# wiedenhoeft/HaMMLET

Hardware: AMD Instinct MI355X
Metric: block-updates/sec (Gibbs sweep) + HBM GB/s, 10^8 pos / 5 states (higher is better)
Workload: dtype f32; 1 GPU; c3_1e8_k5_dynamic; positions=100000000, states=5, block_structure=dynamic, chains=1, parallelism=chain-parallel x1

## Files before the change

hammlet_amd/csrc/hml_capi.hip:

```cpp
#include "hml_capi_shared.hpp"

static thread_local std::string g_err;
int hml_set_err(int code, const std::string& msg) { g_err = msg; return code; }

static const hml_ktab* ktab(int K);
#define HML_KTAB(KV, tab) const hml_ktab* tab = ktab(KV); if (!tab) return set_err(HML_ERR_ARG, "number of states must be in [2,16]")

std::atomic<int> hml_live_ctx[64];
int hml_ctx_bind(hml_ctx* c) { return ctx_bind(c); }
int hml_ctx_fetch_model(hml_ctx* c, hml_model* out) { return fetch_model(c, out); }

HML_KERNEL void hml_k_debug_eval(int fn, const float* __restrict__ a, const float* __restrict__ b, float* __restrict__ out,
                                 uint64_t n, uint64_t seed) {
    if (fn == 24) {
        const uint64_t nw = ((uint64_t)gridDim.x * blockDim.x) >> 6;
        if ((threadIdx.x & 63) != 0) return;
        for (uint64_t i = ((uint64_t)blockIdx.x * blockDim.x + threadIdx.x) >> 6; i < n; i += nw) {
            hml_dev_src src;
            src.s = hml_stream_open(hml_make_key(seed, 0), HML_KIND_THETA, seed, (uint32_t)i);
            out[i] = hml_gamma_f32<hml_devmath>(src, a[i], b[i]);
        }
        return;
    }
    const uint64_t stride = (uint64_t)gridDim.x * blockDim.x;
// ... 615 lines not shown
    layout(c->fwdL_mid, c->lay_mid);
    layout(c->fwdL_many, c->lay_many);
    HIPCHK(hipMalloc(&c->d_em, plane * sizeof(float)));
    HIPCHK(hipMalloc(&c->d_gsc, plane * sizeof(float)));
    HIPCHK(hipMalloc(&c->d_rows, plane * sizeof(float)));
    HIPCHK(hipMalloc(&c->d_entry, maxChunks * K * sizeof(float)));
    HIPCHK(hipMalloc(&c->d_exitA, maxChunks * K * sizeof(float)));
    HIPCHK(hipMalloc(&c->d_fb, maxChunks * sizeof(uint32_t)));
    HIPCHK(hipMalloc(&c->d_smap, (cap + 2) * sizeof(unsigned long long)));
    const uint64_t bchunks = (cap + 15) / 16 + 1;
    HIPCHK(hipMalloc(&c->d_cmap, bchunks * sizeof(unsigned long long)));
    HIPCHK(hipMalloc(&c->d_bentry, bchunks));
    HIPCHK(hipMalloc(&c->d_scmap, bchunks * sizeof(unsigned long long)));
    HIPCHK(hipMalloc(&c->d_super, (bchunks / 64 + 2) * sizeof(unsigned long long)));
    HIPCHK(hipMalloc(&c->d_bentry2, bchunks / 64 + 2));
    HIPCHK(hipMalloc(&c->d_redo, bchunks * sizeof(uint32_t)));
    HIPCHK(hipMemsetAsync(c->d_redo, 0, bchunks * sizeof(uint32_t), c->stream));
    HIPCHK(hipMalloc(&c->d_touched, bchunks * sizeof(uint32_t)));
    HIPCHK(hipMemsetAsync(c->d_touched, 0, bchunks * sizeof(uint32_t), c->stream));
    HIPCHK(hipMalloc(&c->d_redo2, bchunks * sizeof(uint32_t)));
    HIPCHK(hipMalloc(&c->d_tre_bitmap, (bchunks / 32 + 2) * sizeof(uint32_t)));
    HIPCHK(hipMalloc(&c->d_tre_ckpt, (cap / HML_TRE_CKPT_ROWS + 64) * (uint64_t)(K + 1) * sizeof(uint32_t)));
    HIPCHK(hipMalloc(&c->d_q, cap * sizeof(int16_t)));
    const uint64_t n_partial = ((uint64_t)HML_REDUCE_GROUPS + HML_PARAMS_TREE_WGS) * K * 2;
    HIPCHK(hipMalloc(&c->d_partial, n_partial * sizeof(double)));
    HIPCHK(hipMemsetAsync(c->d_partial, 0, n_partial * sizeof(double), c->stream));
    return 0;
}

static int grow_capacity(hml_ctx* c, uint64_t needed) {
    const uint64_t cap = std::min<uint64_t>(c->T, std::max<uint64_t>(needed + needed / 2 + 1024, 2 * c->cap));
    if (c->graph_exec) { hipGraphExecDestroy(c->graph_exec); c->graph_exec = nullptr; }
    void** blocks[] = {(void**)&c->d_starts, (void**)&c->d_bstat};
    for (void** q : blocks) if (*q) { hipFree(*q); *q = nullptr; }
    free_sweep_buffers(c,  true);
    if (c->d_eprobe) { hipFree(c->d_eprobe); c->d_eprobe = nullptr; }
    if (c->d_aprobe) { hipFree(c->d_aprobe); c->d_aprobe = nullptr; }
    c->cap = cap;
    HIPCHK(hipMalloc(&c->d_starts, (cap + 1) * sizeof(uint32_t)));
    HIPCHK(hipMalloc(&c->d_bstat, cap * (uint64_t)c->D * sizeof(float2)));
    if (c->model_set) {
        if (int r = alloc_sweep_buffers(c)) return r;
        if (c->probes) {
            HIPCHK(hipMalloc(&c->d_eprobe, c->cap * c->K * sizeof(float)));
            HIPCHK(hipMalloc(&c->d_aprobe, (c->cap + 1) * c->K * sizeof(float)));
        }
    }
    const uint32_t words[2] = {(uint32_t)cap, 0u};
    static_assert(offsetof(hml_model, halted) == offsetof(hml_model, cap) + sizeof(uint32_t), "cap and halted are written together");
    HIPCHK(hipMemcpyAsync(&c->d_mdl->cap, words, sizeof words, hipMemcpyHostToDevice, c->stream));
    HIPCHK(hipStreamSynchronize(c->stream));
    c->h_B[2] = 0u;
    c->blocks_valid = false;
    c->hint_stale = false;
    c->grown++;
    return 0;
}

static int sweep_dispatch(hml_ctx* c, char method, bool record);

int hml_settle(hml_ctx* c) {
    for (int round = 0; round < 64; ++round) {
        HIPCHK(hipStreamSynchronize(c->stream));
        if (!chain_halted(c)) { c->sweep_log.clear(); c->log_base = c->requested; return 0; }
        const uint64_t needed = c->h_B[2];
        if (c->cap >= c->T) return set_err(HML_ERR_HIP, "internal error: a chain with full block capacity halted");
        std::vector<uint8_t> pending;
        if (c->model_set) {
            hml_model m;
            if (int r = fetch_model(c, &m)) return r;
            const uint64_t ran = m.sweeps >= c->log_base ? m.sweeps - c->log_base : 0;
            if (ran < c->sweep_log.size()) pending.assign(c->sweep_log.begin() + ran, c->sweep_log.end());
            c->log_base = m.sweeps;
        }
        if (int r = grow_capacity(c, needed)) return r;
        c->sweep_log = pending;
        bool halted_again = false;
        for (size_t i = 0; i < pending.size() && !halted_again; ++i) {
            const char method = (pending[i] & 1) ? HML_METHOD_MIXTURE : HML_METHOD_FB;
            const bool record = (pending[i] & 2) != 0;
            if (int r = sweep_dispatch(c, method, record)) return r;
            if (record && c->cb) {
                HIPCHK(hipStreamSynchronize(c->stream));
                halted_again = chain_halted(c);
                if (!halted_again) {
                    if (int r = check_device_error(c)) return r;
                    const unsigned long long ordinal = c->log_base + i;
                    c->cb(c, ordinal >= c->call_base ? (uint64_t)(ordinal - c->call_base) : 0u, c->cb_user);
                }
            }
        }
    }
    return set_err(HML_ERR_HIP, "internal error: the block capacity did not settle");
}

extern "C" {

int hml_set_model(hml_ctx* c, int K, const float nig4[4], float a_off, float a_diag, float pi_alpha, int self_trans) {
    if (!c || !c->loaded) return set_err(HML_ERR_ARG, "no observations loaded");
    if (K < 2) return set_err(HML_ERR_MODEL, "Requested parameters would yield an HMM with less than 2 states!");
    if (K > HML_CAP_K) return set_err(HML_ERR_ARG, "number of states must be in [2,64]");
    if (c->model_set) return set_err(HML_ERR_ARG, "model already set");
    if (c->D > 1 && c->P == 0) {
        for (int pp = 2; pp <= K; ++pp) { long k = 1; for (int d = 0; d < c->D; ++d) k *= pp; if (k == K) { c->P = pp; break; } if (k > K) break; }
        if (c->P == 0) return set_err(HML_ERR_ARG, "number of states must be (number of parameters)^(data dimensions)");
    }
    if (c->P > 0) {
        long k = 1;
        for (int d = 0; d < c->D; ++d) k *= c->P;
        if (k != K) return set_err(HML_ERR_ARG, "number of states must be (number of parameters)^(data dimensions)");
    }
    if (!(nig4[0] > 0)) return set_err(HML_ERR_MODEL, "Alpha (" + std::to_string(nig4[0]) + ") must be positive!");
    if (!(nig4[1] > 0)) return set_err(HML_ERR_MODEL, "Beta (" + std::to_string(nig4[1]) + ") must be positive!");
    if (!(nig4[3] > 0)) return set_err(HML_ERR_MODEL, "Nu (" + std::to_string(nig4[3]) + ")must be positive!");
    const hml_ktab* kt = nullptr;
    c->wide = !c->compat && (K > HML_MAX_K || (getenv("HML_WIDE") && atoi(getenv("HML_WIDE")) != 0));
    if (!c->compat && !c->wide) { kt = ktab(K); if (!kt) return set_err(HML_ERR_ARG, "number of states must be in [2,16]"); }
    if (int r = ctx_bind(c)) return r;
    free_sweep_buffers(c);
    c->K = K;
    if (!getenv("HML_PARAMS_SPREAD")) c->params_spread = K >= 8;
    const uint64_t T = c->T;
    if (int r = alloc_sweep_buffers(c)) return r;

    hml_model m;
    memset(&m, 0, sizeof m);
    m.K = K; m.self_trans = self_trans ? 1 : 0; m.dynamic = 1; m.T = (uint32_t)T;
    m.D = c->D; m.P = c->P > 0 ? c->P : K; m.stat_stride = T;
    m.cap = (uint32_t)c->cap;
    for (int st = 0; st < K; ++st) {
        int nn = st;
        for (int d = 0; d < HML_MAX_D; ++d) { m.map[st][d] = (uint8_t)(d < c->D ? nn % m.P : 0); nn /= m.P; }
    }
    for (int i = 0; i < 4; ++i) m.nig_prior[i] = nig4[i];
    m.a_off = a_off; m.a_diag = a_diag; m.pi_alpha = pi_alpha;
    m.key = hml_make_key(c->seed, c->chain);
    for (int k = 0; k < K; ++k) {
        for (int i = 0; i < 4; ++i) m.nig_post[k][i] = nig4[i];
        m.dirPi[k] = pi_alpha;
        m.pi[k] = 1.0f / K;
        for (int j = 0; j < K; ++j) { m.dirA[k * K + j] = (k == j) ? a_diag : a_off; m.A[k * K + j] = 1.0f / K; }
    }
    m.max_state_recorded = -1;
    m.tre_fused = (c->tre_fused && c->D == 1) ? 1u : 0u;
    m.tre_hi_shift = 17u; m.tre_lo_shift = 20u;
    if (const char* e = getenv("HML_TRE_REFIT_SHIFTS")) { unsigned a = 17, b = 20; if (sscanf(e, "%u,%u", &a, &b) == 2 && a < 32 && b < 32) { m.tre_hi_shift = a; m.tre_lo_shift = b; } }
    m.fwd_W0 = (uint32_t)c->fwdW;
    m.fwd_W = m.fwd_W_burnin = (uint32_t)std::max(c->fwdW, c->fwdW_init);
    if (c->compat || c->wide) { m.fwd_W = 64u; m.fwd_W0 = c->wide ? (uint32_t)c->wide_w0 : 32u; }
    m.wl_bwd_W = 64u; m.wl_bwd_quiet = 0u; m.wl_retry = 0u; m.wl_W_need = 0u; m.wl_need_age = 0u;
    m.fwd_burnin_sweeps = c->fwd_burnin_sweeps;
    m.fwd_quiet_need = c->fwd_quiet_need;
    m.n_spans = c->n_spans;
    HIPCHK(hipMemcpyAsync(c->d_mdl, &m, sizeof m, hipMemcpyHostToDevice, c->stream));
    HIPCHK(hipStreamSynchronize(c->stream));
    c->dynamic = true;
    c->hint_stale = true;
    if (c->compat) {
        hml_mt_state h;
        hml_mt_seed(&h, c->seed + (uint64_t)c->chain);
        HIPCHK(hipMalloc(&c->d_mt, sizeof(hml_mt_state)));
        HIPCHK(hipMemcpyAsync(c->d_mt, &h, sizeof h, hipMemcpyHostToDevice, c->stream));
        HIPCHK(hipStreamSynchronize(c->stream));
        hipLaunchKernelGGL(hml_k_compat_draw, dim3(1), dim3(64), 0, c->stream, c->d_mdl, (hml_mt_state*)c->d_mt, 2);
        KLAUNCH_CHECK();
        c->model_set = true;
        return 0;
    }
    if (c->wide) hipLaunchKernelGGL(hml_k_wide_params, dim3(1), dim3(1024), 0, c->stream, c->d_mdl, c->d_partial, (hml_wide_acc*)c->d_wacc, 2);
    else kt->params(c, 2);
    KLAUNCH_CHECK();
    c->model_set = true;
    return 0;
}

int hml_sample_prior(hml_ctx* c) {
    if (!c || !c->model_set) return set_err(HML_ERR_ARG, "model not set");
    if (int r = ctx_bind(c)) return r;
    if (int r = settle_if_limited(c)) return r;
    if (c->compat) {
        hipLaunchKernelGGL(hml_k_compat_draw, dim3(1), dim3(64), 0, c->stream, c->d_mdl, (hml_mt_state*)c->d_mt, 1);
    } else if (c->wide) {
        hipLaunchKernelGGL(hml_k_wide_params, dim3(1), dim3(1024), 0, c->stream, c->d_mdl, c->d_partial, (hml_wide_acc*)c->d_wacc, 1);
    } else { HML_KTAB(c->K, kt); kt->params(c, 1); }
    KLAUNCH_CHECK();
    if (c->dynamic) c->blocks_valid = false;
    c->hint_stale = true;
    return 0;
}

HML_KERNEL __launch_bounds__(64) void hml_k_set_self_trans(hml_model* mdl, int on) {
    if (threadIdx.x == 0) mdl->self_trans = on;
}

int hml_set_self_transitions(hml_ctx* c, int on) {
    if (!c || !c->model_set) return set_err(HML_ERR_ARG, "model not set");
    if (int r = ctx_bind(c)) return r;
    if (int r = settle_if_limited(c)) return r;
    hipLaunchKernelGGL(hml_k_set_self_trans, dim3(1), dim3(64), 0, c->stream, c->d_mdl, on ? 1 : 0);
    KLAUNCH_CHECK();
    if (c->graph_exec) { hipGraphExecDestroy(c->graph_exec); c->graph_exec = nullptr; }
    return 0;
}

int hml_set_static_blocks(hml_ctx* c) {
    if (!c || !c->model_set) return set_err(HML_ERR_ARG, "model not set");
    if (int r = ctx_bind(c)) return r;
    if (int r = settle_if_limited(c)) return r;
    hipLaunchKernelGGL(hml_k_set_dynamic, dim3(1), dim3(64), 0, c->stream, c->d_mdl, 0, 1);
    KLAUNCH_CHECK();
    c->dynamic = false;
    if (!cap_limited(c)) {
        if (int r = launch_compact(c, false, 0.0f)) return r;
    } else {
        bool fitted = false;
        for (int round = 0; round < 64 && !fitted; ++round) {
            if (int r = launch_compact(c, false, 0.0f)) return r;
            HIPCHK(hipStreamSynchronize(c->stream));
            fitted = !chain_halted(c);
            if (!fitted) { if (int r = grow_capacity(c, c->h_B[2])) return r; }
        }
        if (!fitted) return set_err(HML_ERR_HIP, "internal error: the block capacity did not settle");
        refresh_hint(c);
    }
    c->blocks_valid = true;
    return 0;
}

int hml_set_dynamic(hml_ctx* c, int on) {
    if (!c || !c->model_set) return set_err(HML_ERR_ARG, "model not set");
    if (int r = ctx_bind(c)) return r;
    if (int r = settle_if_limited(c)) return r;
    hipLaunchKernelGGL(hml_k_set_dynamic, dim3(1), dim3(64), 0, c->stream, c->d_mdl, on ? 1 : 0, on ? 1 : 0);
    KLAUNCH_CHECK();
    c->dynamic = on != 0;
    if (on) { c->blocks_valid = false; c->hint_stale = true; }
    return 0;
}

int hml_set_recording(hml_ctx* c, int marginals, hml_record_cb cb, void* user) {
    if (!c) return set_err(HML_ERR_ARG, "null context");
    c->rec_marginals = marginals != 0;
    c->cb = cb; c->cb_user = user;
    return 0;
}

static int set_recorder(hml_ctx* c, int kind, int on) {
    if (!c) return set_err(HML_ERR_ARG, "null context");
    c->rec[kind].on = on != 0;
    if (on) c->rec[kind].asked = true;
    if (c->graph_exec) { if (int r = ctx_bind(c)) return r; hipGraphExecDestroy(c->graph_exec); c->graph_exec = nullptr; }
    return 0;
}
int hml_set_level_recording(hml_ctx* c, int on) { return set_recorder(c, HML_REC_LEVELS, on); }
int hml_set_break_recording(hml_ctx* c, int on) { return set_recorder(c, HML_REC_BREAKS, on); }

int hml_set_level_bands(hml_ctx* c, int n_edges, const float* edges) {
    if (!c) return set_err(HML_ERR_ARG, "null context");
    if (c->graph_exec) { if (int r = ctx_bind(c)) return r; hipGraphExecDestroy(c->graph_exec); c->graph_exec = nullptr; }
    if (n_edges == 0) { c->rec[HML_REC_BANDS].on = false; return 0; }
    if (!edges) return set_err(HML_ERR_ARG, "null argument");
    if (const char* why = band_edges_fault(n_edges, edges)) return set_err(HML_ERR_ARG, why);
    if (c->model_set && (uint64_t)c->D * (uint64_t)(n_edges + 1) > HML_CAP_K)
        return set_err(HML_ERR_ARG, "level bands: the data dimensions times (edges + 1) exceed 64 columns");
    if (!same_band_edges(c, n_edges, edges) && c->rec[HML_REC_BANDS].d_acc) {
        if (int r = ctx_bind(c)) return r;
        if (int r = hml_settle(c)) return r;
        hml_model m; if (int r = fetch_model(c, &m)) return r;
        if (m.n_bands_recorded != 0ull) return set_err(HML_ERR_ARG, "level bands were already recorded under other edges: they cannot be changed any more");
        hml_recorder& rec = c->rec[HML_REC_BANDS];
        HIPCHK(hipFree(rec.d_acc)); rec.d_acc = nullptr;
        HIPCHK(hipFree(rec.d_boundary)); rec.d_boundary = nullptr;
    }
    c->n_band_edges = n_edges;
    memcpy(c->band_edges, edges, (size_t)n_edges * sizeof(float));
    c->rec[HML_REC_BANDS].on = c->rec[HML_REC_BANDS].asked = true;
    return 0;
}

int hml_get_level_bands(hml_ctx* c, int* n_edges, float* edges) {
    if (!c || !n_edges) return set_err(HML_ERR_ARG, "null argument");
    *n_edges = c->n_band_edges;
    if (edges) memcpy(edges, c->band_edges, (size_t)c->n_band_edges * sizeof(float));
    return 0;
}

int hml_enable_probes(hml_ctx* c, int on) {
    if (!c || !c->model_set) return set_err(HML_ERR_ARG, "model not set");
    if (int r = ctx_bind(c)) return r;
    if (int r = settle_if_limited(c)) return r;
    if (on && !c->d_eprobe) {
        HIPCHK(hipMalloc(&c->d_eprobe, c->cap * c->K * sizeof(float)));
        HIPCHK(hipMalloc(&c->d_aprobe, (c->cap + 1) * c->K * sizeof(float)));
    }
    c->probes = on != 0;
    return 0;
}

}

int hml_ctx_ensure_marginal_buffers(hml_ctx* c) { return ensure_marginal_buffers(c); }

static hml_compat_chunks chunk_views(const hml_ctx* c) {
    hml_compat_chunks ch;
    char* base = (char*)c->d_cchunk;
    const uint64_t n = c->wide ? c->wide_chunks_cap : (uint64_t)HML_COMPAT_MAX_CHUNKS;
// ... 208 lines not shown
                int rr = sweep_dispatch(c, method, false);
                const hipError_t ec = hipStreamEndCapture(c->stream, &g);
                if (rr || ec != hipSuccess) {
                    if (g) hipGraphDestroy(g);
                    (void)hipGetLastError();
                    return rr ? rr : set_err(HML_ERR_HIP, std::string("hipStreamEndCapture: ") + hipGetErrorString(ec));
                }
                const hipError_t ei = hipGraphInstantiate(&c->graph_exec, g, nullptr, nullptr, 0);
                hipGraphDestroy(g);
                if (ei != hipSuccess) { c->graph_exec = nullptr; return set_err(HML_ERR_HIP, std::string("hipGraphInstantiate: ") + hipGetErrorString(ei)); }
                c->graph_method = method; c->graph_dynamic = c->dynamic; c->graph_hint = c->B_hint; c->graph_fused = wants_fused;
                c->graph_dense = c->B_hint >= c->dense_min_blocks;
                c->graph_mid = c->B_hint >= c->mid_min_blocks;
            }
            if (c->graph_exec) {
                log_sweep(c, method, false);
                HIPCHK(hipGraphLaunch(c->graph_exec, c->stream));
                if (tre_path) c->tre_dense_sweeps++;
                continue;
            }
        }
        log_sweep(c, method, record);
        if (int r = sweep_dispatch(c, method, record)) return r;
        if (record && c->cb) {
            HIPCHK(hipStreamSynchronize(c->stream));
            if (chain_halted(c)) { if (int r = hml_settle(c)) return r; continue; }
            if (int r = check_device_error(c)) return r;
            c->cb(c, i, c->cb_user);
        }
    }
    return 0;
}

}

extern "C" int hml_iterate_many(hml_ctx* const* cs, int n, char method, uint64_t iterations, uint64_t thinning) {
    if (!cs || n < 1) return set_err(HML_ERR_ARG, "no contexts");
    for (int i = 0; i < n; ++i) if (!cs[i] || !cs[i]->model_set) return set_err(HML_ERR_ARG, "model not set");
    if (method != HML_METHOD_FB && method != HML_METHOD_MIXTURE) return set_err(HML_ERR_ARG, std::string("Unknown sampling type ") + method + "!");
    for (int i = 0; i < n; ++i) cs[i]->call_base = cs[i]->requested;
    uint64_t done = 0;
    while (done < iterations && many_eligible(cs, n, method)) {
        if (int r = ctx_bind(cs[0])) return r;
        for (int i = 0; i < n; ++i) {
            hml_ctx* c = cs[i];
            if (int r = settle_if_limited(c)) return r;
            if (c->hint_stale) { launch_compact_pair(c, 0, 0.0f); KLAUNCH_CHECK(); }
            HIPCHK(hipStreamSynchronize(c->stream));
            c->hint_stale = false;
            if (c->graph_exec) { hipGraphExecDestroy(c->graph_exec); c->graph_exec = nullptr; }
        }
        int r = 0;
        uint64_t reached = done;
        { HML_KTAB(cs[0]->K, kt); r = kt->iterate_many(cs, n, done, iterations, thinning, &reached); }
        if (r) return r;
        hipEvent_t ev = ev_get(cs[0]);
        HIPCHK(hipEventRecord(ev, cs[0]->stream));
        for (int i = 1; i < n; ++i) HIPCHK(hipStreamWaitEvent(cs[i]->stream, ev, 0));
        cs[0]->ev_pool.push_back(ev);
        if (reached == iterations) return 0;
        HIPCHK(hipStreamSynchronize(cs[0]->stream));
        bool halted = false;
        for (int i = 0; i < n; ++i) halted = halted || chain_halted(cs[i]);
        const bool progress = reached > done;
        done = reached;
        if (!halted && !progress) break;
        if (!halted) { bool sparse = true; for (int i = 0; i < n; ++i) sparse = sparse && many_sparse(cs[i]); if (!sparse) break; }
    }
    for (int i = 0; i < n; ++i) if (int r = settle_if_limited(cs[i])) return r;
    for (uint64_t i = done; i < iterations; ++i) {
        const bool record = thinning > 0 && ((i + 1) % thinning == 0);
        for (int k = 0; k < n; ++k) {
            hml_ctx* c = cs[k];
            if (int r = ctx_bind(c)) return r;
            if (record && c->rec_marginals && c->pooled) return set_err(HML_ERR_ARG, "the marginals of a context are pooled (common labels, several chains): further sweeps cannot be recorded into them");
            if (chain_halted(c)) { if (int r = hml_settle(c)) return r; }
            log_sweep(c, method, record);
            if (int r = sweep_dispatch(c, method, record)) return r;
            if (record && c->cb) {
                HIPCHK(hipStreamSynchronize(c->stream));
                if (chain_halted(c)) { if (int r = hml_settle(c)) return r; continue; }
                if (int r = check_device_error(c)) return r;
                c->cb(c, i, c->cb_user);
            }
        }
    }
    return 0;
}

extern "C" {

int hml_set_option(hml_ctx* c, const char* name, int value) {
    if (!c || !name) return set_err(HML_ERR_ARG, "null argument");
    if (std::string(name) == "weight_keys") {
        if (c->loaded) return set_err(HML_ERR_ARG, "weight_keys must be set before the observations are loaded");
        c->use_keys = value != 0;
        c->summary_always = value == 2;
        return 0;
    }
    if (std::string(name) == "max_blocks") {
        if (c->loaded) return set_err(HML_ERR_ARG, "max_blocks must be set before the observations are loaded");
        if (value < 0) return set_err(HML_ERR_ARG, "max_blocks: a number of blocks, or 0 for the default");
        c->cap_opt = (uint64_t)value;
        return 0;
    }
    if (std::string(name) == "fused_blocks") {
        c->fused_blocks = value != 0;
        c->fused_keep = value == 2;
        if (c->graph_exec) { hipGraphExecDestroy(c->graph_exec); c->graph_exec = nullptr; }
        return 0;
    }
    if (std::string(name) == "compat") {
        if (c->model_set) return set_err(HML_ERR_ARG, "compat must be set before the model");
        c->compat = value != 0;
        return 0;
    }
    if (std::string(name) == "trellis_L") {
        if (value < 0 || value > HML_TRE_MAX_L || value % 32) return set_err(HML_ERR_ARG, "trellis_L: 0 or a multiple of 32 up to 1024");
        c->tre_L = (uint32_t)value;
        return 0;
    }
    return set_err(HML_ERR_ARG, std::string("unknown option ") + name);
}

int hml_sync(hml_ctx* c) {
    if (!c) return set_err(HML_ERR_ARG, "null context");
    if (int r = ctx_bind(c)) return r;
    if (int r = hml_settle(c)) return r;
    if (c->d_dbg && getenv("HML_FUSED_DEBUG") && atoi(getenv("HML_FUSED_DEBUG")) == 2) {
        std::vector<unsigned long long> h(4096 * 8);
        hipMemcpy(h.data(), c->d_dbg, h.size() * 8, hipMemcpyDeviceToHost);
        uint32_t n = 0; while (n < 4096 && h[n * 8]) ++n;
        unsigned long long t0 = ~0ull; for (uint32_t i = 0; i < n; ++i) t0 = std::min(t0, h[i * 8]);
        double mx[5] = {0, 0, 0, 0, 0}, av[5] = {0, 0, 0, 0, 0};
        if (n) for (uint32_t i = 0; i < n; ++i) for (int k = 0; k < 5; ++k) { const double d = (double)(h[i * 8 + k] - t0) * 0.01; mx[k] = std::max(mx[k], d); av[k] += d / n; }
        if (n) fprintf(stderr, "[fused-many dbg] n=%u start avg %.2f max %.2f | phaseA avg %.2f max %.2f | requested avg %.2f max %.2f | offsets avg %.2f max %.2f | end avg %.2f max %.2f (us)\n",
                n, av[0], mx[0], av[1], mx[1], av[2], mx[2], av[3], mx[3], av[4], mx[4]);
        if (n) for (uint32_t i : {0u, n / 4, n / 2, n - 1}) if (i < n) fprintf(stderr, "   wg %u: %.2f %.2f %.2f %.2f %.2f | wavefront 0: parameters in LDS %.2f, weights arrived %.2f, its lists done %.2f\n", i, (h[i*8]-t0)*0.01, (h[i*8+1]-t0)*0.01, (h[i*8+2]-t0)*0.01, (h[i*8+3]-t0)*0.01, (h[i*8+4]-t0)*0.01,
                                                                                  (h[i*8+5]-t0)*0.01, (h[i*8+6]-t0)*0.01, (h[i*8+7]-t0)*0.01);
    } else if (c->d_dbg) {
        std::vector<unsigned long long> h(4096 * 4);
        hipMemcpy(h.data(), c->d_dbg, h.size() * 8, hipMemcpyDeviceToHost);
        const uint32_t n = (uint32_t)std::min<uint64_t>(4096, (c->T + HML_FUSED_SUB_POSITIONS - 1) / HML_FUSED_SUB_POSITIONS);
        unsigned long long t0 = ~0ull; for (uint32_t i = 0; i < n; ++i) if (h[i * 4]) t0 = std::min(t0, h[i * 4]);
        double mx[4] = {0, 0, 0, 0}, av[4] = {0, 0, 0, 0};
        for (uint32_t i = 0; i < n; ++i) for (int k = 0; k < 4; ++k) { const double d = (double)(h[i * 4 + k] - t0) * 0.01; mx[k] = std::max(mx[k], d); av[k] += d / n; }
        fprintf(stderr, "[fused dbg] n=%u start avg %.2f max %.2f | phaseA avg %.2f max %.2f | offsets avg %.2f max %.2f | end avg %.2f max %.2f (us)\n", n, av[0], mx[0], av[1], mx[1], av[2], mx[2], av[3], mx[3]);
        { uint32_t late = 0, first_late = n; for (uint32_t i = 0; i < n; ++i) if ((h[i * 4] - t0) * 0.01 > 2.0) { ++late; first_late = std::min(first_late, i); }
          fprintf(stderr, "   late starters: %u, first index %u\n", late, first_late); }
        for (uint32_t i : {0u, n / 4, n / 2, n - 1}) fprintf(stderr, "   wg %u: %.2f %.2f %.2f %.2f\n", i, (h[i*4]-t0)*0.01, (h[i*4+1]-t0)*0.01, (h[i*4+2]-t0)*0.01, (h[i*4+3]-t0)*0.01);
    }
    if (c->model_set && getenv("HML_PARAMS_DEBUG")) {
        hml_model m;
        if (fetch_model(c, &m) == 0) {
            fprintf(stderr, "[params dbg] us since the kernel's start: accumulators read %.2f | tree %.2f | theta drawn %.2f | A gammas %.2f | barrier %.2f | end %.2f\n",
                    (m.dbg_t[1] - m.dbg_t[0]) * 0.01, (m.dbg_t[2] - m.dbg_t[0]) * 0.01, (m.dbg_t[3] - m.dbg_t[0]) * 0.01, (m.dbg_t[4] - m.dbg_t[0]) * 0.01,
                    (m.dbg_t[5] - m.dbg_t[0]) * 0.01, (m.dbg_t[6] - m.dbg_t[0]) * 0.01);
            fprintf(stderr, "[params dbg]   theta's gamma core + normal drawn %.2f | last wavefront's tree %.2f\n", (m.dbg_t[7] - m.dbg_t[0]) * 0.01, (m.dbg_t[8] - m.dbg_t[0]) * 0.01);
        }
    }
    if (c->model_set) return check_device_error(c);
    return 0;
}


static int current_B(hml_ctx* c, uint32_t* B) {
    HIPCHK(hipMemcpyAsync(c->h_B, &c->d_mdl->B, sizeof(uint32_t), hipMemcpyDeviceToHost, c->stream));
    HIPCHK(hipStreamSynchronize(c->stream));
    *B = *c->h_B;
    return 0;
}

int hml_get_num_blocks(hml_ctx* c, uint64_t* B) {
    NEED_LOADED();
    uint32_t b; if (int r = current_B(c, &b)) return r;
    *B = b; return 0;
}
int hml_get_blocks(hml_ctx* c, uint32_t* starts) {
    NEED_LOADED();
    uint32_t b; if (int r = current_B(c, &b)) return r;
    HIPCHK(hipMemcpy(starts, c->d_starts, ((uint64_t)b + 1) * sizeof(uint32_t), hipMemcpyDeviceToHost));
    return 0;
}
int hml_get_block_stats(hml_ctx* c, float* sum, float* sum_sq) {
    NEED_LOADED();
    uint32_t b; if (int r = current_B(c, &b)) return r;
    std::vector<float2> v(b);
    for (int d = 0; d < c->D; ++d) {
        HIPCHK(hipMemcpy(v.data(), c->d_bstat + (uint64_t)d * c->T, (uint64_t)b * sizeof(float2), hipMemcpyDeviceToHost));
        for (uint32_t i = 0; i < b; ++i) { sum[(uint64_t)d * b + i] = v[i].x; sum_sq[(uint64_t)d * b + i] = v[i].y; }
    }
    return 0;
}
int hml_get_states(hml_ctx* c, int16_t* q) {
    NEED_MODEL();
    uint32_t b; if (int r = current_B(c, &b)) return r;
    HIPCHK(hipMemcpy(q, c->d_q, (uint64_t)b * sizeof(int16_t), hipMemcpyDeviceToHost));
    return 0;
}
int hml_get_theta(hml_ctx* c, float* mean_var) {
    NEED_MODEL();
    hml_model m; if (int r = fetch_model(c, &m)) return r;
    for (int k = 0; k < m.P; ++k) { mean_var[2 * k] = m.mu[k]; mean_var[2 * k + 1] = m.var[k]; }
    return 0;
}
int hml_get_dimensions(hml_ctx* c, int* D, int* P) {
    if (!c) return set_err(HML_ERR_ARG, "null context");
    if (D) *D = c->D;
    if (P) *P = c->P > 0 ? c->P : c->K;
    return 0;
}
int hml_get_transitions(hml_ctx* c, float* A, float* pi) {
    NEED_MODEL();
    hml_model m; if (int r = fetch_model(c, &m)) return r;
    if (A) memcpy(A, m.A, (size_t)c->K * c->K * sizeof(float));
    if (pi) memcpy(pi, m.pi, (size_t)c->K * sizeof(float));
    return 0;
}
int hml_set_parameters(hml_ctx* c, const float* mean_var, const float* A, const float* pi) {
    NEED_MODEL();
    hml_model m; if (int r = fetch_model(c, &m)) return r;
    const int K = c->K;
    for (int k = 0; k < m.P; ++k) {
        const float mean = mean_var[2 * k], var = mean_var[2 * k + 1];
        if (!std::isfinite(mean)) return set_err(HML_ERR_MODEL, "Mean (" + std::to_string(mean) + ") must be set to a finite value!");
        if (!std::isfinite(var)) return set_err(HML_ERR_MODEL, "Variance(" + std::to_string(var) + ") must be set to a finite value!");
        if (var <= 0) return set_err(HML_ERR_MODEL, "Variance (" + std::to_string(var) + ") must be positive!");
        m.mu[k] = mean; m.var[k] = var; m.sd[k] = sqrtf(var);
    }
    memcpy(m.A, A, (size_t)K * K * sizeof(float));
    memcpy(m.pi, pi, (size_t)K * sizeof(float));
    HIPCHK(hipMemcpyAsync(c->d_mdl, &m, sizeof m, hipMemcpyHostToDevice, c->stream));
    if (c->compat) hipLaunchKernelGGL(hml_k_compat_derive, dim3(1), dim3(64), 0, c->stream, c->d_mdl);
    else if (c->wide) hipLaunchKernelGGL(hml_k_wide_derive, dim3(1), dim3(64), 0, c->stream, c->d_mdl);
    else { HML_KTAB(K, kt); kt->derive(c); }
    KLAUNCH_CHECK();
    HIPCHK(hipStreamSynchronize(c->stream));
    if (c->dynamic) c->blocks_valid = false;
    return 0;
}
int hml_get_threshold(hml_ctx* c, float* thr) {
    NEED_MODEL();
    hml_model m; if (int r = fetch_model(c, &m)) return r;
    *thr = m.thr; return 0;
}
int hml_get_block_loglik(hml_ctx* c, float* E) {
    NEED_MODEL();
    if (!c->probes) return set_err(HML_ERR_ARG, "probes are not enabled");
    uint32_t b; if (int r = current_B(c, &b)) return r;
    HIPCHK(hipMemcpy(E, c->d_eprobe, (uint64_t)b * c->K * sizeof(float), hipMemcpyDeviceToHost));
    return 0;
}
int hml_get_forward_rows(hml_ctx* c, float* rows) {
    NEED_MODEL();
    if (!c->probes) return set_err(HML_ERR_ARG, "probes are not enabled");
    uint32_t b; if (int r = current_B(c, &b)) return r;
    HIPCHK(hipMemcpy(rows, c->d_aprobe, ((uint64_t)b + 1) * c->K * sizeof(float), hipMemcpyDeviceToHost));
    return 0;
}
int hml_get_counts(hml_ctx* c, uint64_t* trans, uint64_t* occ, float* sum, float* sum_sq, uint64_t* nterms) {
    NEED_MODEL();
    hml_model m; if (int r = fetch_model(c, &m)) return r;
    const int K = c->K;
    for (int i = 0; i < K * K; ++i) trans[i] = m.last_trans[i];
    for (int k = 0; k < K; ++k) { occ[k] = m.last_occ[k]; nterms[k] = m.last_occ[k]; sum[k] = m.last_sum[k]; sum_sq[k] = m.last_sumsq[k]; }
    return 0;
}
int hml_get_weights(hml_ctx* c, float* w) {
    NEED_LOADED();
    HIPCHK(hipStreamSynchronize(c->stream));
    HIPCHK(hipMemcpy(w, c->d_w, c->T * sizeof(float), hipMemcpyDeviceToHost));
    return 0;
}
int hml_get_coefficients(hml_ctx* c, float* cf) {
    NEED_LOADED();
    HIPCHK(hipStreamSynchronize(c->stream));
    HIPCHK(hipMemcpy(cf, c->d_coeff, c->T * sizeof(float), hipMemcpyDeviceToHost));
    return 0;
}
int hml_get_integral_array(hml_ctx* c, float* sum, float* sum_sq) {
    NEED_LOADED();
    HIPCHK(hipStreamSynchronize(c->stream));
    std::vector<float2> v(c->T + 1);
    HIPCHK(hipMemcpy(v.data(), c->d_ia, (c->T + 1) * sizeof(float2), hipMemcpyDeviceToHost));
    for (uint64_t i = 0; i <= c->T; ++i) { sum[i] = v[i].x; sum_sq[i] = v[i].y; }
    return 0;
}

int hml_recorded_sweeps(hml_ctx* c, uint64_t* n) {
    NEED_MODEL();
    hml_model m; if (int r = fetch_model(c, &m)) return r;
    *n = m.n_recorded; return 0;
}

int hml_relabel_permutation(hml_ctx* c, int32_t* perm) {
    NEED_MODEL();
    if (!perm) return set_err(HML_ERR_ARG, "null argument");
    hml_model m; if (int r = fetch_model(c, &m)) return r;
    const int K = c->K, D = m.D;
    std::vector<int32_t> p(K);
    for (int k = 0; k < K; ++k) p[k] = k;
    std::stable_sort(p.begin(), p.end(), [&](int32_t a, int32_t b) {
        for (int d = 0; d < D; ++d) {
            const float ma = m.mu[m.map[a][d]], mb = m.mu[m.map[b][d]];
            if (ma < mb) return true;
            if (mb < ma) return false;
        }
// ... 98 lines not shown
```

hammlet_amd/csrc/hml_common.h:

```cpp
#ifndef HML_COMMON_H
#define HML_COMMON_H

#include <stdint.h>
#include <stddef.h>

#if defined(__HIPCC__)
#include <hip/hip_runtime.h>
#define HML_HD __host__ __device__ __forceinline__
#define HML_HDM __host__ __device__ __forceinline__
#define HML_KERNEL static __global__
#else
#define HML_HD static inline
#define HML_HDM inline
#endif

#define HML_CELLSIZE 65535u

#define HML_MAX_K 16
#define HML_CAP_K 64

HML_HD uint32_t hml_f2u(float f) { return __builtin_bit_cast(uint32_t, f); }
HML_HD float hml_u2f(uint32_t u) { return __builtin_bit_cast(float, u); }
HML_HD uint64_t hml_d2u(double d) { return __builtin_bit_cast(uint64_t, d); }
HML_HD double hml_u2d(uint64_t u) { return __builtin_bit_cast(double, u); }

#define HML_INF_F (hml_u2f(0x7f800000u))

#endif
```

hammlet_amd/csrc/hml_k_backward.h:

```cpp
#ifndef HML_K_BACKWARD_H
#define HML_K_BACKWARD_H

#include <type_traits>

#include "hml_dist.h"
#include "hml_k_forward.h"
#include "hml_philox.h"
#include "hml_state.h"

#define HML_MAP_IDENTITY 0xfedcba9876543210ull

template <int K>
__device__ __forceinline__ unsigned long long hml_map_compose(unsigned long long f, unsigned long long g) {
    unsigned long long r = 0ull;
#pragma unroll
    for (int x = 0; x < K; ++x) {
        const unsigned y = (unsigned)(g >> (4 * x)) & 15u;
        const unsigned long long z = (f >> (4 * y)) & 15ull;
        r |= z << (4 * x);
    }
    return r;
}

__device__ __forceinline__ unsigned long long hml_shfl_down_u64(unsigned long long v, int d) {
    const unsigned lo = (unsigned)v, hi = (unsigned)(v >> 32);
    const unsigned lo2 = __shfl_down(lo, d), hi2 = __shfl_down(hi, d);
    return ((unsigned long long)hi2 << 32) | lo2;
}

template <int K>
__device__ __forceinline__ int hml_categorical_k_literal(const float (&w)[K], double u) {
    double sum = 0.0;
#pragma unroll
    for (int i = 0; i < K; ++i) sum += (double)w[i];
    double cp = 0.0;
    int res = K - 1;
    bool done = false;
#pragma unroll
    for (int i = 0; i < K; ++i) {
        cp += (double)w[i] / sum;
        const double c = (i == K - 1) ? 1.0 : cp;
        if (!done && !(c < u)) { res = i; done = true; }
    }
    return res;
}

template <int K>
__device__ __forceinline__ int hml_categorical_k_fast(const float (&w)[K], double u, bool& unsure_out) {
    double s[K];
    double acc = 0.0;
#pragma unroll
    for (int i = 0; i < K; ++i) { acc += (double)w[i]; s[i] = acc; }
    const double t = u * acc;
    const double margin = acc * 5.684341886080802e-14;
    bool unsure = !(acc > 0.0) || !(acc < 1.7976931348623157e308);
    int res = K - 1;
    bool done = false;
#pragma unroll
    for (int i = 0; i < K - 1; ++i) {
        const double d = s[i] - t;
        unsure = unsure || !(__builtin_fabs(d) > margin);
        if (!done && d >= 0.0) { res = i; done = true; }
    }
    unsure_out = unsure_out || unsure;
    return res;
}

template <int K>
__device__ __forceinline__ int hml_categorical_k_screen(const float (&w)[K], float uf, bool& unsure_out) {
    static_assert(K <= 16, "error bound of the float screen");
    float s[K];
    float acc = 0.0f;
#pragma unroll
    for (int i = 0; i < K; ++i) { acc += w[i]; s[i] = acc; }
    const float t = uf * acc;
    const float margin = acc * 7.62939453125e-06f;
    bool unsure = !(acc > 7.888609052210118e-31f) || !(acc < 3.4028234663852886e38f);
    int res = K - 1;
    bool done = false;
#pragma unroll
    for (int i = 0; i < K - 1; ++i) {
        const float d = s[i] - t;
        unsure = unsure || !(__builtin_fabsf(d) > margin);
        if (!done && d >= 0.0f) { res = i; done = true; }
    }
    unsure_out = unsure;
    return res;
}

template <int K>
__device__ __forceinline__ int hml_categorical_k(const float (&w)[K], double u) {
    bool unsure = false;
    int res = hml_categorical_k_screen<K>(w, (float)u, unsure);
    if (unsure) {
        asm volatile("" ::: "memory");
        unsure = false;
        res = hml_categorical_k_fast<K>(w, u, unsure);
        if (unsure) res = hml_categorical_k_literal<K>(w, u);
    }
    return res;
}

template <int K>
struct hml_bwd_ctx {
    hml_amat<K> A;
    float logA[K];
    bool self;
};
template <int K>
__device__ __forceinline__ void hml_bwd_ctx_load(hml_bwd_ctx<K>& bx, const hml_model* __restrict__ mdl_ro, const float* lds_A) {
    bx.A.attach(mdl_ro, lds_A);
#pragma unroll
    for (int i = 0; i < K; ++i) bx.logA[i] = mdl_ro->logA[i];
    bx.self = mdl_ro->self_trans != 0;
}

template <int K>
__device__ __forceinline__ void hml_bwd_row_load(const float* __restrict__ rows, const hml_layout lay, uint32_t c, int lane,
                                                 uint32_t B, float (&r)[K], const uint32_t* __restrict__ starts,
                                                 const hml_bwd_ctx<K>& bx) {
    const uint32_t t = c * HML_BWD_CHUNK + (uint32_t)lane + 1u;
    uint32_t st = 0u, en = 1u;
    if (starts && t < B) { st = starts[t - 1u]; en = starts[t]; }
#pragma unroll
    for (int i = 0; i < K; ++i) r[i] = (t <= B) ? rows[hml_bk(lay, t - 1u, K, i)] : 0.0f;
    if (starts && t < B && bx.self) {
        const float N = (float)(en - st);
#pragma unroll
        for (int i = 0; i < K; ++i) r[i] = r[i] * hml_expf((N - 1.0f) * bx.logA[i]);
    }
}

template <int K>
__device__ __forceinline__ void hml_bwd_chunk_maps(const float (&r)[K], hml_model* __restrict__ mdl, const hml_bwd_ctx<K>& bx,
                                                   unsigned long long* __restrict__ smap, unsigned long long* __restrict__ cmap,
                                                   uint32_t c, int lane, uint32_t B, unsigned long long epoch, const hml_key key) {
    const uint32_t t = c * HML_BWD_CHUNK + (uint32_t)lane + 1u;
    unsigned long long map = HML_MAP_IDENTITY;
    if (t <= B) {
        const double u = hml_cat_uniform(key, epoch, t);
        map = 0ull;
#pragma unroll
        for (int i = 0; i < K; ++i)
            if (r[i] < 0.0f) hml_raise(mdl, HML_DEVERR_NEG_BACKWARD, r[i]);
        if (t == B) {
            const unsigned long long st = (unsigned long long)hml_categorical_k<K>(r, u);
#pragma unroll
            for (int x = 0; x < K; ++x) map |= st << (4 * x);
        } else {
#pragma unroll
            for (int x = 0; x < K; ++x) {
                float w[K];
#pragma unroll
                for (int i = 0; i < K; ++i) w[i] = r[i] * bx.A[i * K + x];
                map |= (unsigned long long)hml_categorical_k<K>(w, u) << (4 * x);
            }
        }
    }
#pragma unroll
    for (int d = 1; d < 64; d <<= 1) {
        unsigned long long o = hml_shfl_down_u64(map, d);
        if (lane + d >= 64) o = HML_MAP_IDENTITY;
        map = hml_map_compose<K>(map, o);
    }
    if (t <= B) smap[t] = map;
    if (lane == 0) cmap[c] = map;
}

template <int K>
__device__ __forceinline__ void hml_b_backward_maps(const float* __restrict__ rows, hml_model* __restrict__ mdl,
                                                           unsigned long long* __restrict__ smap,
                                                           unsigned long long* __restrict__ cmap, const hml_layout lay,
                                                           const float* __restrict__ entry, const float* __restrict__ exitv,
                                                           uint32_t* __restrict__ fail_list, int L,
                                                           const uint32_t* __restrict__ starts,
                                                           const hml_model* __restrict__ mdl_ro) {
    const uint32_t B = mdl_ro->B;
    const uint32_t nchunks = (B + HML_BWD_CHUNK - 1u) / HML_BWD_CHUNK;
    const int lane = threadIdx.x & 63;
    const uint32_t wave_global = (blockIdx.x * blockDim.x + threadIdx.x) >> 6;
    const uint32_t nwaves = (gridDim.x * blockDim.x) >> 6;
    const unsigned long long epoch = mdl_ro->epoch;
    const hml_key key = mdl_ro->key;
    const int W = (int)mdl_ro->fwd_W;
    __shared__ float sm_A[hml_amat<K>::LDS_FLOATS];
    hml_amat_fill<K>(sm_A, mdl_ro, (int)threadIdx.x, (int)blockDim.x);
    hml_bwd_ctx<K> bx;
    hml_bwd_ctx_load<K>(bx, mdl_ro, sm_A);
    const uint32_t C = (B + (uint32_t)L - 1u) / (uint32_t)L;
    for (uint32_t c = wave_global; c < nchunks; c += nwaves) {
        float r[K];
        hml_bwd_row_load<K>(rows, lay, c, lane, B, r, starts, bx);
        bool ok = true;
        {
            const uint32_t f0 = (c * HML_BWD_CHUNK) / (uint32_t)L;
            const uint32_t f1 = (c * HML_BWD_CHUNK + HML_BWD_CHUNK - 1u) / (uint32_t)L;
            const uint32_t f = f0 + (uint32_t)lane;
            if (f <= f1 && f < C && !hml_fwd_chunk_exact(f, L, W)) {
                uint32_t differ = 0u;
#pragma unroll
                for (int s = 0; s < K; ++s) differ |= hml_f2u(entry[(uint64_t)f * K + s]) ^ hml_f2u(exitv[(uint64_t)(f - 1) * K + s]);
                ok = differ == 0u;
            }
        }
        if (__ballot(!ok) != 0ull) {
            if (lane == 0) fail_list[atomicAdd(&mdl->fwd_mismatch, 1u)] = c;
            continue;
        }
        hml_bwd_chunk_maps<K>(r, mdl, bx, smap, cmap, c, lane, B, epoch, key);
    }
}
template <int K>
HML_KERNEL __launch_bounds__(256) void hml_k_backward_maps(const float* __restrict__ rows, hml_model* __restrict__ mdl,
                                                           unsigned long long* __restrict__ smap,
                                                           unsigned long long* __restrict__ cmap, const hml_layout lay,
                                                           const float* __restrict__ entry, const float* __restrict__ exitv,
                                                           uint32_t* __restrict__ fail_list, int L,
                                                           const uint32_t* __restrict__ starts,
                                                           const hml_model* __restrict__ mdl_ro) {
    hml_b_backward_maps<K>(rows, mdl, smap, cmap, lay, entry, exitv, fail_list, L, starts, mdl_ro);
}


template <int K>
__device__ __forceinline__ unsigned long long hml_bwd_row_map(const float (&r)[K], hml_model* __restrict__ mdl, const hml_bwd_ctx<K>& bx,
                                                              uint32_t t, uint32_t B, double u) {
    if (t > B) return HML_MAP_IDENTITY;
    unsigned long long map = 0ull;
#pragma unroll
    for (int i = 0; i < K; ++i)
        if (r[i] < 0.0f) hml_raise(mdl, HML_DEVERR_NEG_BACKWARD, r[i]);
    if (t == B) {
        const unsigned long long st = (unsigned long long)hml_categorical_k<K>(r, u);
#pragma unroll
        for (int x = 0; x < K; ++x) map |= st << (4 * x);
    } else {
#pragma unroll
        for (int x = 0; x < K; ++x) {
            float w[K];
#pragma unroll
            for (int i = 0; i < K; ++i) w[i] = r[i] * bx.A[i * K + x];
            map |= (unsigned long long)hml_categorical_k<K>(w, u) << (4 * x);
        }
    }
    return map;
}
template <int K>
__device__ __forceinline__ void hml_bwd_row_load_t(const float* __restrict__ rows, const hml_layout lay, uint32_t t, uint32_t B, float (&r)[K],
                                                   const uint32_t* __restrict__ starts, const hml_bwd_ctx<K>& bx) {
    uint32_t st = 0u, en = 1u;
    if (starts && t < B) { st = starts[t - 1u]; en = starts[t]; }
#pragma unroll
    for (int i = 0; i < K; ++i) r[i] = (t <= B) ? rows[hml_bk(lay, t - 1u, K, i)] : 0.0f;
    if (starts && t < B && bx.self) {
        const float N = (float)(en - st);
#pragma unroll
        for (int i = 0; i < K; ++i) r[i] = r[i] * hml_expf((N - 1.0f) * bx.logA[i]);
    }
}
template <int K>
__device__ __forceinline__ void hml_b_backward_maps2(const float* __restrict__ rows, hml_model* __restrict__ mdl,
                                                            unsigned long long* __restrict__ smap,
                                                            unsigned long long* __restrict__ cmap, const hml_layout lay,
                                                            const float* __restrict__ entry, const float* __restrict__ exitv,
                                                            uint32_t* __restrict__ fail_list, int L,
                                                            const uint32_t* __restrict__ starts,
                                                            const hml_model* __restrict__ mdl_ro) {
    const uint32_t B = mdl_ro->B;
    const uint32_t nchunks = (B + HML_BWD_CHUNK - 1u) / HML_BWD_CHUNK;
    const uint32_t npairs = (nchunks + 1u) / 2u;
    const int lane = threadIdx.x & 63, li = lane & 31, half = lane >> 5;
    const uint32_t wave_global = (blockIdx.x * blockDim.x + threadIdx.x) >> 6;
    const uint32_t nwaves = (gridDim.x * blockDim.x) >> 6;
    const unsigned long long epoch = mdl_ro->epoch;
    const hml_key key = mdl_ro->key;
    const int W = (int)mdl_ro->fwd_W;
    __shared__ float sm_A[hml_amat<K>::LDS_FLOATS];
    hml_amat_fill<K>(sm_A, mdl_ro, (int)threadIdx.x, (int)blockDim.x);
    hml_bwd_ctx<K> bx;
    hml_bwd_ctx_load<K>(bx, mdl_ro, sm_A);
    const uint32_t C = (B + (uint32_t)L - 1u) / (uint32_t)L;
    for (uint32_t pw = wave_global; pw < npairs; pw += nwaves) {
        const uint32_t c = 2u * pw + (uint32_t)half;
        const uint32_t t0 = c * HML_BWD_CHUNK + 2u * (uint32_t)li + 1u;
        float r0[K], r1[K];
        hml_bwd_row_load_t<K>(rows, lay, t0, B, r0, starts, bx);
        hml_bwd_row_load_t<K>(rows, lay, t0 + 1u, B, r1, starts, bx);
        bool ok = true;
        if (c < nchunks) {
            const uint32_t f0 = (c * HML_BWD_CHUNK) / (uint32_t)L;
            const uint32_t f1 = (c * HML_BWD_CHUNK + HML_BWD_CHUNK - 1u) / (uint32_t)L;
            for (uint32_t f = f0 + (uint32_t)li; f <= f1 && f < C; f += 32u) {
                if (hml_fwd_chunk_exact(f, L, W)) continue;
                uint32_t differ = 0u;
#pragma unroll
                for (int s = 0; s < K; ++s) differ |= hml_f2u(entry[(uint64_t)f * K + s]) ^ hml_f2u(exitv[(uint64_t)(f - 1) * K + s]);
                ok = ok && differ == 0u;
            }
        }
        const unsigned long long failed = __ballot(!ok);
        const bool my_fail = (half ? (failed >> 32) : (failed & 0xffffffffull)) != 0ull;
        if (my_fail && li == 0 && c < nchunks) fail_list[atomicAdd(&mdl->fwd_mismatch, 1u)] = c;
        if ((failed & 0xffffffffull) != 0ull && (failed >> 32) != 0ull) continue;
        double u0, u1;
        hml_cat_uniform_pair(key, epoch, (t0 - 1u) >> 1, u0, u1);
        const bool live = !my_fail && c < nchunks;
        const unsigned long long m0 = live ? hml_bwd_row_map<K>(r0, mdl, bx, t0, B, u0) : HML_MAP_IDENTITY;
        const unsigned long long m1 = live ? hml_bwd_row_map<K>(r1, mdl, bx, t0 + 1u, B, u1) : HML_MAP_IDENTITY;
        unsigned long long P = hml_map_compose<K>(m0, m1);
#pragma unroll
        for (int d = 1; d < 32; d <<= 1) {
            unsigned long long o = hml_shfl_down_u64(P, d);
            if (li + d >= 32) o = HML_MAP_IDENTITY;
            P = hml_map_compose<K>(P, o);
        }
        unsigned long long later = hml_shfl_down_u64(P, 1);
        if (li == 31) later = HML_MAP_IDENTITY;
        if (live) {
            if (t0 <= B) smap[t0] = P;
            if (t0 + 1u <= B) smap[t0 + 1u] = hml_map_compose<K>(m1, later);
            if (li == 0) cmap[c] = P;
        }
    }
}

template <int K>
__device__ __forceinline__ void hml_b_backward_chain(unsigned long long* __restrict__ cmap, hml_model* __restrict__ mdl,
                                                             uint8_t* __restrict__ entry_state, const float* __restrict__ em,
                                                             const float* __restrict__ gsc, float* __restrict__ rows,
                                                             float* __restrict__ aprobe, float* __restrict__ entry,
                                                             float* __restrict__ exitv, uint32_t* __restrict__ fb_count,
                                                             const uint32_t* __restrict__ fail_list, uint32_t* __restrict__ touched,
                                                             unsigned long long* __restrict__ smap, int L, const hml_layout lay,
                                                             int mode, int super_level, const uint32_t* __restrict__ starts) {
    __shared__ unsigned long long P[1024];
    __shared__ hml_repair_lds sh;
    const uint32_t B = mdl->B;
    const uint32_t NCb = (B + HML_BWD_CHUNK - 1u) / HML_BWD_CHUNK;
    const uint32_t NC = super_level ? (NCb + 63u) / 64u : NCb;
    const int tid = threadIdx.x;
    const uint32_t n_fail = (mode & 1) ? mdl->fwd_mismatch : 0u;
    if (n_fail != 0u) {
        const unsigned long long epoch = mdl->epoch;
        const uint32_t gen = (uint32_t)epoch + 1u;
        const hml_key key = mdl->key;
        __shared__ float sm_A[hml_amat<K>::LDS_FLOATS];
        hml_amat_fill<K>(sm_A, mdl, tid, 1024);
        hml_fwd_repair<K>(em, gsc, mdl, rows, aprobe, entry, exitv, fb_count, fail_list, n_fail, touched, gen, L, lay, sh, sm_A);
        const int lane = tid & 63, wave = tid >> 6;
        hml_bwd_ctx<K> bx;
        hml_bwd_ctx_load<K>(bx, mdl, sm_A);
        auto redo = [&](uint32_t c) {
            float r[K];
            hml_bwd_row_load<K>(rows, lay, c, lane, B, r, starts, bx);
            hml_bwd_chunk_maps<K>(r, mdl, bx, smap, cmap, c, lane, B, epoch, key);
        };
        for (uint32_t i = (uint32_t)wave; i < n_fail; i += 16u) redo(fail_list[i]);
        const uint32_t n_touched = sh.tcount;
        if (n_touched <= (uint32_t)HML_REPAIR_TOUCHED_CAP) {
            for (uint32_t i = (uint32_t)wave; i < n_touched; i += 16u) redo(sh.tlist[i]);
        } else {
            for (uint32_t c0 = (uint32_t)wave * 64u; c0 < NCb; c0 += 16u * 64u) {
                const uint32_t c = c0 + (uint32_t)lane;
                unsigned long long todo = __ballot(c < NCb && hml_ld_u32_coherent(touched + c) == gen);
                while (todo) {
                    const int j = __ffsll((long long)todo) - 1;
                    todo &= todo - 1ull;
                    redo(c0 + (uint32_t)j);
                }
            }
        }
        __threadfence_block();
        __syncthreads();
        if (tid == 0) mdl->fwd_mismatch = 0u;
    }
    if (!(mode & 2)) return;
    const uint32_t per = (NC + 1023u) / 1024u;
    const uint32_t a = (uint32_t)tid * per < NC ? (uint32_t)tid * per : NC;
    const uint32_t b = (a + per < NC) ? a + per : NC;
    const int lane = tid & 63, wave = tid >> 6;
    constexpr int CACHED = 4;
    unsigned long long mine[CACHED];
    unsigned long long prod = HML_MAP_IDENTITY;
    if (per <= (uint32_t)CACHED) {
#pragma unroll
        for (int j = 0; j < CACHED; ++j) mine[j] = (a + (uint32_t)j < b) ? cmap[a + (uint32_t)j] : HML_MAP_IDENTITY;
#pragma unroll
        for (int j = CACHED - 1; j >= 0; --j) prod = hml_map_compose<K>(mine[j], prod);
    } else {
        for (uint32_t c = b; c > a; --c) prod = hml_map_compose<K>(cmap[c - 1], prod);
    }
    unsigned long long S = prod;
#pragma unroll
    for (int d = 1; d < 64; d <<= 1) {
        unsigned long long o = hml_shfl_down_u64(S, d);
        if (lane + d >= 64) o = HML_MAP_IDENTITY;
        S = hml_map_compose<K>(S, o);
    }
    if (lane == 0) P[wave] = S;
    __syncthreads();
    if (tid < 64) {
        unsigned long long w = (tid < 16) ? P[tid] : HML_MAP_IDENTITY;
#pragma unroll
        for (int d = 1; d < 16; d <<= 1) {
            unsigned long long o = hml_shfl_down_u64(w, d);
            if (tid + d >= 16) o = HML_MAP_IDENTITY;
            w = hml_map_compose<K>(w, o);
        }
        if (tid < 16) P[16 + tid] = w;
    }
    __syncthreads();
    const unsigned long long after_wave = (wave < 15) ? P[16 + wave + 1] : HML_MAP_IDENTITY;
    unsigned long long next_S = hml_shfl_down_u64(S, 1);
    const unsigned long long later = (lane < 63) ? hml_map_compose<K>(next_S, after_wave) : after_wave;
    if (a >= b) return;
    unsigned x = (unsigned)(later & 15ull);
    if (per <= (uint32_t)CACHED) {
#pragma unroll
        for (int j = CACHED - 1; j >= 0; --j) {
            if (a + (uint32_t)j < b) {
                entry_state[a + (uint32_t)j] = (uint8_t)x;
                x = (unsigned)(mine[j] >> (4 * x)) & 15u;
            }
        }
    } else {
        for (uint32_t c = b; c > a; --c) {
            entry_state[c - 1] = (uint8_t)x;
            x = (unsigned)(cmap[c - 1] >> (4 * x)) & 15u;
        }
    }
}
template <int K>
HML_KERNEL __launch_bounds__(1024) void hml_k_backward_chain(unsigned long long* __restrict__ cmap, hml_model* __restrict__ mdl,
// ... 405 lines not shown
```

hammlet_amd/csrc/hml_k_blocks_fused.h:

```cpp
#ifndef HML_K_BLOCKS_FUSED_H
#define HML_K_BLOCKS_FUSED_H

#include "hml_k_blocks.h"
#include "hml_k_forward.h"

#define HML_FUSED_WAVES 8
#define HML_FUSED_WAVE_BATCH (HML_SUM_SPANS * HML_SPAN)
#define HML_FUSED_SUB_POSITIONS (HML_FUSED_WAVES * HML_FUSED_WAVE_BATCH)
#define HML_FUSED_MAX_SUB 4
#define HML_FUSED_POS_BITS 19
#define HML_FUSED_GEN_MASK ((1u << (64 - 2 * HML_FUSED_POS_BITS - 1)) - 1u)
#define HML_FUSED_WAVE_LIST 256
__device__ __forceinline__ unsigned long long hml_group_word(uint32_t gen, uint32_t total, uint32_t last_rel) {
    return ((unsigned long long)(gen & HML_FUSED_GEN_MASK) << (2 * HML_FUSED_POS_BITS + 1)) |
           ((unsigned long long)total << HML_FUSED_POS_BITS) | (unsigned long long)last_rel;
}
__device__ __forceinline__ uint32_t hml_fused_generation(const hml_model* mdl) { return ((uint32_t)mdl->epoch + 1u) & HML_FUSED_GEN_MASK; }

__device__ __forceinline__ unsigned long long hml_fused_tile_word(const uint8_t* __restrict__ summary, const float* __restrict__ w, uint32_t T,
                                                               float thr, int32_t base, uint32_t tile, uint32_t n_sub, uint32_t gen) {
    const uint32_t n_spans = (uint32_t)(((uint64_t)T + HML_SPAN - 1) / HML_SPAN);
    const uint32_t kthr = (thr != thr) ? 0u : hml_weight_key(thr, base);
    const uint32_t first_span = tile * (uint32_t)HML_FUSED_WAVES * n_sub * HML_SUM_SPANS;
    const uint32_t spans = (uint32_t)HML_FUSED_WAVES * n_sub * HML_SUM_SPANS;
    uint32_t total = 0u, last1 = 0u;
    for (uint32_t s = 0; s < spans && first_span + s < n_spans; ++s) {
        const uint32_t span = first_span + s;
        for (uint32_t g = 0; g < 256u; ++g) {
            const uint32_t key = summary[(uint64_t)span * 256u + (uint64_t)(g & 63u) * 4u + (g >> 6)];
            const bool origin = (span == 0u && g == 0u);
            if (key < kthr && !origin) continue;
            uint32_t m16 = hml_group_mask16(w, (uint64_t)span * HML_SPAN + (uint64_t)g * 16u, T, thr);
            if (origin) m16 |= 1u;
            if (m16) {
                total += (uint32_t)__popc(m16);
                last1 = s * HML_SPAN + g * 16u + (31u - (uint32_t)__clz((int)m16)) + 1u;
            }
        }
    }
    return hml_group_word(gen, total, last1 ? last1 - 1u : 0u);
}

template <int K>
HML_KERNEL __launch_bounds__(HML_FUSED_WAVES * 64, 6) void hml_k_blocks_fused(const uint8_t* __restrict__ summary, const float* __restrict__ w,
                                                          const float2* __restrict__ ia, uint32_t T,
                                                          hml_model* __restrict__ mdl, int32_t base,
                                                          unsigned long long* __restrict__ group_word,
                                                          uint16_t* __restrict__ stage, uint32_t* __restrict__ starts,
                                                          float2* __restrict__ bstat, float* __restrict__ em,
                                                          float* __restrict__ gsc, float* __restrict__ eprobe, int mixture,
                                                          const hml_layout lay, uint32_t* __restrict__ host_words,
                                                          uint32_t n_sub, uint32_t spin_limit, unsigned long long* __restrict__ dbg,
                                                          const hml_model* __restrict__ mdl_ro) {
    if (dbg && threadIdx.x == 0) dbg[blockIdx.x * 4 + 0] = wall_clock64();
    static_assert(HML_FUSED_MAX_SUB * HML_FUSED_SUB_POSITIONS == (1 << HML_FUSED_POS_BITS), "tile geometry (bit fields of hml_group_word)");
    static_assert(HML_FUSED_MAX_SUB * HML_FUSED_WAVE_BATCH <= 65536, "16-bit offsets into a wavefront's eighth");
    constexpr int NW = HML_FUSED_WAVES;
    constexpr uint32_t NT = NW * 64;
    __shared__ uint16_t listed_all[NW][HML_SUM_SPANS * 256];
    __shared__ uint16_t mask_all[NW][HML_SUM_SPANS * 256];
    __shared__ uint16_t wave_list[NW][HML_FUSED_WAVE_LIST];
    __shared__ uint32_t wave_total[NW], wave_last[NW];
    __shared__ unsigned long long red_sum[NW], red_near[NW];
    __shared__ uint64_t sm_exp_tab[32];
    if (threadIdx.x < 32u) sm_exp_tab[threadIdx.x] = HML_EXP2F_TAB[threadIdx.x];
    constexpr bool LOOPED = K > 6;
    __shared__ hml_emit_lds<LOOPED ? K : 1> sm_emit;
    if (LOOPED) hml_emit_lds_fill<LOOPED ? K : 1>(sm_emit, mdl_ro, (int)threadIdx.x);

    const int lane = threadIdx.x & 63, wave = threadIdx.x >> 6;
    const uint32_t g = blockIdx.x;
    const uint32_t n_spans = (uint32_t)(((uint64_t)T + HML_SPAN - 1) / HML_SPAN);
    const uint32_t eighth = n_sub * (uint32_t)HML_FUSED_WAVE_BATCH;
    const uint32_t tile_positions = eighth * (uint32_t)NW;
    const uint64_t wave_base = ((uint64_t)g * NW + (uint32_t)wave) * eighth;
    const uint32_t gen = hml_fused_generation(mdl_ro);
    uint16_t* listed = listed_all[wave];
    uint16_t* masks = mask_all[wave];
    const float thr = mdl_ro->thr;
    const uint32_t cap = mdl_ro->cap;

    uint32_t total = 0u, last1 = 0u;
    uint32_t placed = 0u;
    uint32_t n_listed = 0u, last_batch = 0u;
    auto expand = [&](uint32_t j, uint32_t n_l) {
        for (uint32_t i0 = 0; i0 < n_l; i0 += 64u) {
            const uint32_t i = i0 + (uint32_t)lane;
            uint32_t m16 = 0u, in_eighth = 0u;
            if (i < n_l) {
                const uint32_t sg = listed[i];
                m16 = masks[i];
                in_eighth = j * (uint32_t)HML_FUSED_WAVE_BATCH + (sg >> 8) * HML_SPAN + (sg & 255u) * 16u;
            }
            const uint32_t c = (uint32_t)__popc(m16);
            uint32_t r, sum;
            const unsigned long long some = __ballot(c != 0u);
            if (__ballot(c > 1u) == 0ull) {
                r = placed + hml_mbcnt(some);
                sum = (uint32_t)__popcll(some);
            } else {
                uint32_t incl = c;
#pragma unroll
                for (int d = 1; d < 64; d <<= 1) {
                    const uint32_t o = __shfl_up(incl, d);
                    if (lane >= d) incl += o;
                }
                r = placed + incl - c;
                sum = __shfl(incl, 63);
            }
            while (m16) {
                const int bit = __ffs(m16) - 1;
                m16 &= m16 - 1u;
                const uint16_t off = (uint16_t)(in_eighth + (uint32_t)bit);
                if (r < (uint32_t)HML_FUSED_WAVE_LIST) wave_list[wave][r] = off;
                else stage[wave_base + r] = off;
                ++r;
            }
            placed += sum;
        }
    };
    {
        const uint32_t kthr = (thr != thr) ? 0u : hml_weight_key(thr, base);
        const hml_swar_ge sw_ge = hml_swar_ge_make(kthr);
        auto load_batch = [&](uint32_t j, uint32_t (&gw)[HML_SUM_SPANS]) {
            const uint32_t span0 = (uint32_t)(wave_base / HML_SPAN) + j * HML_SUM_SPANS;
#pragma unroll
            for (int s = 0; s < HML_SUM_SPANS; ++s)
                gw[s] = (j < n_sub && span0 + s < n_spans)
                            ? __builtin_nontemporal_load(reinterpret_cast<const uint32_t*>(summary) + (uint64_t)(span0 + s) * 64u + lane)
                            : 0u;
        };
        uint32_t gw[HML_SUM_SPANS];
        load_batch(0u, gw);
        for (uint32_t j = 0; j < n_sub; ++j) {
            const uint32_t span0 = (uint32_t)(wave_base / HML_SPAN) + j * HML_SUM_SPANS;
            if (span0 >= n_spans) break;
            if (j > 0u) expand(j - 1u, n_listed);
            n_listed = 0u;
            last_batch = j;
#pragma unroll
            for (int s = 0; s < HML_SUM_SPANS; ++s) {
                const uint32_t fl = (span0 + s < n_spans) ? hml_swar_ge_apply(sw_ge, gw[s]) : 0u;
#pragma unroll
                for (int q = 0; q < 4; ++q) {
                    const bool open = ((fl >> (8 * q + 7)) & 1u) || (span0 + s == 0u && q == 0 && lane == 0);
                    const unsigned long long m = __ballot(open);
                    if (open) listed[n_listed + hml_mbcnt(m)] = (uint16_t)((s << 8) | (64 * q + lane));
                    n_listed += (uint32_t)__popcll(m);
                }
            }
            load_batch(j + 1u, gw);
            for (uint32_t i0 = 0; i0 < n_listed; i0 += 64u) {
                const uint32_t i = i0 + (uint32_t)lane;
                uint32_t m16 = 0u;
                if (i < n_listed) {
                    const uint32_t sg = listed[i];
                    const uint32_t in_batch = (sg >> 8) * HML_SPAN + (sg & 255u) * 16u;
                    m16 = hml_group_mask16(w, (uint64_t)span0 * HML_SPAN + in_batch, T, thr);
                    if (span0 == 0u && i == 0u) m16 |= 1u;
                    masks[i] = (uint16_t)m16;
                    if (m16) last1 = (uint32_t)wave * eighth + j * (uint32_t)HML_FUSED_WAVE_BATCH + in_batch + (31u - (uint32_t)__clz((int)m16)) + 1u;
                }
                total += (uint32_t)__popc(m16);
            }
        }
        total = hml_wave_sum_u32(total);
#pragma unroll
        for (int m = 1; m < 64; m <<= 1) { const uint32_t o = __shfl_xor(last1, m); last1 = o > last1 ? o : last1; }
    }
    if (lane == 0) { wave_total[wave] = total; wave_last[wave] = last1; }
    __syncthreads();
    if (dbg && threadIdx.x == 0) dbg[blockIdx.x * 4 + 1] = wall_clock64();
    uint32_t wg_total = 0u, wg_last1 = 0u;
#pragma unroll
    for (int k = 0; k < NW; ++k) {
        wg_total += wave_total[k];
        wg_last1 = wave_last[k] > wg_last1 ? wave_last[k] : wg_last1;
    }
    if (threadIdx.x == 0) {
        const uint32_t l1 = wg_last1;
        __hip_atomic_store(&group_word[g], hml_group_word(gen, wg_total, l1 ? l1 - 1u : 0u), __ATOMIC_RELAXED, __HIP_MEMORY_SCOPE_AGENT);
    }
    if ((uint32_t)(wave_base / HML_SPAN) < n_spans) expand(last_batch, n_listed);
    __syncthreads();

    auto start_at = [&](uint32_t k) -> uint32_t {
        uint32_t wv = 0u, first = 0u, run = 0u;
#pragma unroll
        for (int q = 0; q < NW - 1; ++q) {
            run += wave_total[q];
            if (k >= run) { wv = (uint32_t)q + 1u; first = run; }
        }
        const uint32_t idx = k - first;
        const uint64_t wb = ((uint64_t)g * NW + wv) * eighth;
        const uint32_t off = (idx < (uint32_t)HML_FUSED_WAVE_LIST) ? (uint32_t)wave_list[wv][idx] : (uint32_t)stage[wb + idx];
        return (uint32_t)(wb + off);
    };
    const bool last_wg = (g == gridDim.x - 1u);
    const uint32_t n_items = wg_total + (last_wg ? 1u : 0u);

    const uint32_t k_first = threadIdx.x;
    bool have_first = false;
    uint32_t first_t = 0u, first_n = 0u;
    float first_sx = 0.0f, first_sq = 0.0f;
    if (k_first > 0u && k_first < n_items) {
        first_t = (k_first < wg_total) ? start_at(k_first) : T;
        const uint32_t prev_t = start_at(k_first - 1u);
        first_n = first_t - prev_t;
        hml_block_stats_one(ia, prev_t, first_t, first_sx, first_sq);
        have_first = true;
    }

    unsigned long long acc = 0ull, near = 0ull;
    {
        for (uint32_t i = threadIdx.x; i < g; i += NT) {
            unsigned long long d = spin_limit ? __hip_atomic_load(&group_word[i], __ATOMIC_RELAXED, __HIP_MEMORY_SCOPE_AGENT)
                                              : hml_group_word(gen + 1u, 0u, 0u);
            uint32_t tries = 0u;
            while ((uint32_t)(d >> (2 * HML_FUSED_POS_BITS + 1)) != gen) {
                if (tries++ >= spin_limit) {
                    d = hml_fused_tile_word(summary, w, T, thr, base, i, n_sub, gen);
                    __hip_atomic_store(&group_word[i], d, __ATOMIC_RELAXED, __HIP_MEMORY_SCOPE_AGENT);
                    if (host_words) __hip_atomic_store(host_words + 1, 1u, __ATOMIC_RELAXED, __HIP_MEMORY_SCOPE_SYSTEM);
                    atomicAdd(&mdl->fused_fallbacks, 1ull);
                    break;
                }
                __builtin_amdgcn_s_sleep(1);
                d = __hip_atomic_load(&group_word[i], __ATOMIC_RELAXED, __HIP_MEMORY_SCOPE_AGENT);
            }
            const uint32_t tot = (uint32_t)(d >> HML_FUSED_POS_BITS) & ((2u << HML_FUSED_POS_BITS) - 1u);
            acc += tot;
            if (tot) near = ((unsigned long long)(i + 1u) << HML_FUSED_POS_BITS) | (d & ((1ull << HML_FUSED_POS_BITS) - 1ull));
        }
    }
#pragma unroll
    for (int m = 1; m < 64; m <<= 1) {
        acc += __shfl_xor(acc, m);
        const unsigned long long o = __shfl_xor(near, m);
        near = o > near ? o : near;
    }
    if (lane == 0) { red_sum[wave] = acc; red_near[wave] = near; }
    __syncthreads();
    if (dbg && threadIdx.x == 0) dbg[blockIdx.x * 4 + 2] = wall_clock64();
    unsigned long long sum_all = 0ull, nr = 0ull;
#pragma unroll
    for (int k = 0; k < NW; ++k) { sum_all += red_sum[k]; nr = red_near[k] > nr ? red_near[k] : nr; }
    const uint32_t before_group = (uint32_t)sum_all;
    const uint32_t prev_group_start =
        nr ? (uint32_t)(((nr >> HML_FUSED_POS_BITS) - 1ull) * tile_positions + (nr & ((1ull << HML_FUSED_POS_BITS) - 1ull))) : 0u;

    hml_emit_params<LOOPED ? 1 : K> p;
    if (!LOOPED) hml_emit_load<LOOPED ? 1 : K>(p, mdl_ro, mixture);
    const bool self_trans = mdl_ro->self_trans != 0;
    {
        uint32_t t = first_t, n = first_n;
        float sx = first_sx, sq = first_sq;
        bool gathered = have_first;
        for (uint32_t k = threadIdx.x; k < n_items; k += NT) {
            const uint32_t b = before_group + k;
            if (!gathered) {
                t = (k < wg_total) ? start_at(k) : T;
                if (t != 0u) {
                    const uint32_t prev_t = (k > 0u) ? start_at(k - 1u) : prev_group_start;
                    n = t - prev_t;
                    hml_block_stats_one(ia, prev_t, t, sx, sq);
                }
            }
            gathered = false;
            if (b > cap) continue;
            starts[b] = t;
            if (t == 0u) continue;
            bstat[b - 1u] = make_float2(sx, sq);
            if constexpr (LOOPED)
                hml_emit_block_looped<K>(reinterpret_cast<const hml_emit_lds<K>&>(sm_emit), mdl, self_trans, b - 1u, sx, sq, (float)n, em, gsc, eprobe, mixture, lay, sm_exp_tab);
            else
                hml_emit_block<LOOPED ? 1 : K, true>(p, mdl, b - 1u, sx, sq, (float)n, em, gsc, eprobe, mixture, lay, sm_exp_tab);
        }
    }
    if (dbg) { __syncthreads(); if (threadIdx.x == 0) dbg[blockIdx.x * 4 + 3] = wall_clock64(); }
    if (last_wg && threadIdx.x == 0) {
        const uint32_t Bn = before_group + wg_total;
        if (Bn > cap) { hml_halt(mdl, Bn, host_words); return; }
        mdl->B = Bn;
        hml_warmup_for_many_blocks(mdl, Bn);
        if (host_words) __hip_atomic_store(host_words, Bn, __ATOMIC_RELAXED, __HIP_MEMORY_SCOPE_SYSTEM);
    }
}

#endif
```

hammlet_amd/csrc/hml_k_forward.h:

```cpp
#ifndef HML_K_FORWARD_H
#define HML_K_FORWARD_H

#include "hml_k_blocks.h"
#include "hml_math.h"
#include "hml_state.h"

__device__ __forceinline__ void hml_raise(hml_model* mdl, uint32_t code, float value) {
    if (atomicCAS(&mdl->err_code, 0u, code) == 0u) mdl->err_value = value;
    atomicAdd(&mdl->err_count, 1ull);
}

__device__ __forceinline__ bool hml_isfinite(float x) { return (hml_f2u(x) & 0x7f800000u) != 0x7f800000u; }

template <int K>
struct hml_emit_params {
    float mu[K], var[K], logN[K], logA[K];
    double rvar[K];
    bool self;
};

__device__ __forceinline__ float hml_inner_product(float mu, float var, double rvar, float sx, float sq) {
    const double num = 2.0 * (double)mu * (double)sx - (double)sq;
    double ipd = num * rvar;
    const uint64_t bits = hml_d2u(ipd);
// ... 154 lines not shown
    if (threadIdx.x < (unsigned)K) {
        s_logNs[threadIdx.x] = mdl->logNs[threadIdx.x]; s_logA[threadIdx.x] = mdl->logA[threadIdx.x];
        for (int d = 0; d < HML_MAX_D; ++d) s_map[threadIdx.x][d] = mdl->map[threadIdx.x][d];
    }
    if (threadIdx.x >= 64 && threadIdx.x < 96) s_tab[threadIdx.x - 64] = HML_EXP2F_TAB[threadIdx.x - 64];
    __syncthreads();
    const uint32_t stride = gridDim.x * blockDim.x;
    for (uint32_t b = blockIdx.x * blockDim.x + threadIdx.x; b < B; b += stride) {
        const uint32_t st = starts[b], en = starts[b + 1];
        float sx[HML_MAX_D], sq[HML_MAX_D];
        for (int d = 0; d < D; ++d) {
            if (STATS) {
                hml_block_stats_one(ia + (uint64_t)d * (T + 1u), st, en, sx[d], sq[d]);
                bstat[(uint64_t)d * T + b] = make_float2(sx[d], sq[d]);
            } else {
                const float2 v = bstat[(uint64_t)d * T + b];
                sx[d] = v.x; sq[d] = v.y;
            }
        }
        const float N = (float)(en - st);
        float E[K];
        float maxE = -3.40282346638528859812e+38f;
#pragma unroll
        for (int s = 0; s < K; ++s) {
            float r = 0.0f;
            for (int d = 0; d < D; ++d) {
                const int pp = s_map[s][d];
                const float ip = hml_inner_product(s_mu[pp], s_var[pp], s_rvar[pp], sx[d], sq[d]);
                if (!hml_isfinite(ip)) hml_raise(mdl, HML_DEVERR_IP_NOT_FINITE, ip);
                r += ip;
            }
            float e = r - N * s_logNs[s];
            if (self) e += (N - 1.0f) * s_logA[s];
            E[s] = e;
            maxE = (e < maxE) ? maxE : e;
        }
#pragma unroll
        for (int s = 0; s < K; ++s) {
            if (eprobe) eprobe[(uint64_t)b * K + s] = E[s];
            em[hml_bk(lay, b, K, s)] = hml_expf_tab(E[s] - maxE, s_tab);
            if (!mixture && gsc) gsc[hml_bk(lay, b, K, s)] = self ? hml_expf_tab((N - 1.0f) * s_logA[s], s_tab) : 1.0f;
        }
    }
}

template <int K>
struct hml_emit_tile {
    static constexpr int BLOCKS = (K <= 8) ? 512 : 256;
    static constexpr int MAXL = 64;
    static constexpr int GTAB = 64;
};

template <int K>
__device__ __forceinline__ void hml_emit_values_fast(const hml_emit_params<K>& p, const double (&rvar)[K], const float* __restrict__ gtab,
                                                     hml_model* mdl, uint32_t b, float sx, float sq, uint32_t n,
                                                     float* __restrict__ eprobe, int mixture, float (&ev)[K], float (&gv)[K]) {
    const float N = (float)n;
    float E[K];
    float maxE = -3.40282346638528859812e+38f;
#pragma unroll
    for (int s = 0; s < K; ++s) {
        const float ip = hml_inner_product(p.mu[s], p.var[s], rvar[s], sx, sq);
        if (!hml_isfinite(ip)) hml_raise(mdl, HML_DEVERR_IP_NOT_FINITE, ip);
        float e = (0.0f + ip) - N * p.logN[s];
        if (p.self) e += (N - 1.0f) * p.logA[s];
        E[s] = e;
        maxE = (e < maxE) ? maxE : e;
    }
#pragma unroll
    for (int s = 0; s < K; ++s) {
        if (eprobe) eprobe[(uint64_t)b * K + s] = E[s];
        ev[s] = hml_expf(E[s] - maxE);
        gv[s] = 1.0f;
        if (!mixture && p.self) gv[s] = (n <= (uint32_t)hml_emit_tile<K>::GTAB) ? gtab[(n - 1u) * K + s] : hml_expf((N - 1.0f) * p.logA[s]);
    }
}

template <int K, bool STATS>
HML_KERNEL __launch_bounds__(256) void hml_k_emission_tiled(const float2* __restrict__ ia, const uint32_t* __restrict__ starts,
                                                            hml_model* __restrict__ mdl, float2* __restrict__ bstat,
                                                            float* __restrict__ em, float* __restrict__ gsc,
                                                            float* __restrict__ eprobe, int mixture, const hml_layout lay) {
    constexpr int TB = hml_emit_tile<K>::BLOCKS;
    constexpr int GT = hml_emit_tile<K>::GTAB;
    __shared__ float sm_e[K * TB + K * 64 + 64];
    __shared__ float sm_g[K * TB + K * 64 + 64];
    __shared__ float gtab[GT * K];
    const uint32_t B = mdl->B;
    hml_emit_params<K> p;
    hml_emit_load<K>(p, mdl, mixture);
    double rvar[K];
#pragma unroll
    for (int s = 0; s < K; ++s) rvar[s] = p.rvar[s];
    for (int i = threadIdx.x; i < GT * K; i += 256) {
        const int n1 = i / K, s = i % K;
        gtab[i] = hml_expf((float)n1 * mdl->logA[s]);
    }
    const uint32_t Lr = 1u << lay.lshift;
    if (Lr > (uint32_t)hml_emit_tile<K>::MAXL) return;
    const uint32_t cpt = (uint32_t)TB >> lay.lshift;
    const uint32_t pitch = cpt + 1u;
    const uint32_t n_tiles = (B + TB - 1u) / TB;
    __syncthreads();
    for (uint32_t tile = blockIdx.x; tile < n_tiles; tile += gridDim.x) {
        const uint32_t b0 = tile * TB;
#pragma unroll
        for (int j = 0; j < TB / 256; ++j) {
            const uint32_t bl = (uint32_t)j * 256u + threadIdx.x;
            const uint32_t b = b0 + bl;
            if (b < B) {
                const uint32_t st = starts[b], en = starts[b + 1];
                float sx, sq;
                if (STATS) { hml_block_stats_one(ia, st, en, sx, sq); bstat[b] = make_float2(sx, sq); }
                else { const float2 v = bstat[b]; sx = v.x; sq = v.y; }
                float ev[K], gv[K];
                hml_emit_values_fast<K>(p, rvar, gtab, mdl, b, sx, sq, en - st, eprobe, mixture, ev, gv);
                const uint32_t r = bl & (Lr - 1u), cl = bl >> lay.lshift;
#pragma unroll
                for (int s = 0; s < K; ++s) {
                    sm_e[((uint32_t)s * Lr + r) * pitch + cl] = ev[s];
                    sm_g[((uint32_t)s * Lr + r) * pitch + cl] = gv[s];
                }
            }
        }
        __syncthreads();
        const uint32_t c0 = b0 >> lay.lshift;
        const uint32_t nrs = Lr * (uint32_t)K;
        for (uint32_t e = threadIdx.x; e < nrs * cpt; e += 256u) {
            const uint32_t cl = e % cpt, rs = e / cpt;
            const uint32_t r = rs / (uint32_t)K, s = rs % (uint32_t)K;
            const uint32_t b = b0 + (cl << lay.lshift) + r;
            if (b < B) {
                const uint64_t g = ((uint64_t)r * (uint32_t)K + s) * lay.cstride + c0 + cl;
                em[g] = sm_e[(s * Lr + r) * pitch + cl];
                if (!mixture) gsc[g] = sm_g[(s * Lr + r) * pitch + cl];
            }
        }
        __syncthreads();
    }
}

#define HML_A_REGISTERS_MAX_K 7
template <int K, bool REG = (K <= HML_A_REGISTERS_MAX_K)>
struct hml_amat;
template <int K>
struct hml_amat<K, true> {
    static constexpr int LDS_FLOATS = 1;
    float v[K * K];
    __device__ __forceinline__ void attach(const hml_model* mdl, const float*) {
#pragma unroll
        for (int i = 0; i < K * K; ++i) v[i] = mdl->A[i];
    }
    __device__ __forceinline__ float operator[](int i) const { return v[i]; }
};
template <int K>
struct hml_amat<K, false> {
    static constexpr int LDS_FLOATS = K * K;
    const float* p;
    __device__ __forceinline__ void attach(const hml_model*, const float* lds) { p = lds; }
    __device__ __forceinline__ float operator[](int i) const { return p[i]; }
};
template <int K>
__device__ __forceinline__ void hml_amat_fill(float* lds, const hml_model* mdl, int tid, int nthreads) {
    if (K > HML_A_REGISTERS_MAX_K) {
        for (int i = tid; i < K * K; i += nthreads) lds[i] = mdl->A[i];
        __syncthreads();
    }
}

template <int K>
struct hml_fwd_ctx {
    hml_amat<K> A;
    float invK;
    bool self;
    uint32_t B;
};

template <int K>
__device__ __forceinline__ void hml_fwd_ctx_load(hml_fwd_ctx<K>& cx, const hml_model* mdl, const float* lds_A) {
    cx.A.attach(mdl, lds_A);
    cx.invK = (float)(1.0 / (double)(float)K);
    cx.self = mdl->self_trans != 0;
    cx.B = mdl->B;
}

__device__ __forceinline__ double hml_tr2_reciprocal(double Zd) {
    double r = __builtin_amdgcn_rcp(Zd);
    const double e = __builtin_fma(-Zd, r, 1.0);
    return __builtin_fma(r, e, r);
}
__device__ __forceinline__ float hml_tr2_quotient(float f, double Zd, double r) {
    const double fd = (double)f;
    const double q1 = fd * r;
    const double rho = __builtin_fma(-q1, Zd, fd);
    return (float)__builtin_fma(rho, r, q1);
}

template <int K>
__device__ __forceinline__ bool hml_fwd_step(const hml_fwd_ctx<K>& cx, float (&alpha)[K], const float (&e)[K]) {
    float f[K];
#pragma unroll
    for (int j = 0; j < K; ++j) {
        float tt = 0.0f;
#pragma unroll
        for (int i = 0; i < K; ++i) tt += alpha[i] * cx.A[i * K + j];
        f[j] = e[j] * tt;
    }
    float Z = 0.0f;
#pragma unroll
    for (int j = 0; j < K; ++j) Z += f[j];
    if (__builtin_expect(!(Z > 0.0f) || !(Z < 3.4028234663852886e38f), 0)) {
        const bool ok = (Z != 0.0f);
#pragma unroll
        for (int j = 0; j < K; ++j) alpha[j] = ok ? f[j] / Z : cx.invK;
        return !ok;
    }
    const double Zd = (double)Z;
    const double r = hml_tr2_reciprocal(Zd);
#pragma unroll
    for (int j = 0; j < K; ++j) alpha[j] = hml_tr2_quotient(f[j], Zd, r);
    return false;
}

template <int K, bool STORE>
__device__ __forceinline__ void hml_fwd_run(const hml_fwd_ctx<K>& cx, float (&alpha)[K], const float* __restrict__ em,
                                            const float* __restrict__ gsc, float* __restrict__ rows,
                                            float* __restrict__ aprobe, uint32_t b0, uint32_t b1, uint32_t& nfb,
                                            const hml_layout lay) {
    constexpr int BATCH = (K <= 6) ? 4 : 2;
    for (uint32_t b = b0; b < b1; b += BATCH) {
        float e[BATCH][K], g[BATCH][K];
#pragma unroll
        for (int i = 0; i < BATCH; ++i) {
            const uint32_t bi = b + (uint32_t)i;
            const bool ok = bi < b1;
#pragma unroll
            for (int s = 0; s < K; ++s) {
                e[i][s] = ok ? em[hml_bk(lay, bi, K, s)] : 0.0f;
                g[i][s] = (STORE && ok && cx.self && gsc) ? gsc[hml_bk(lay, bi, K, s)] : 1.0f;
            }
        }
#pragma unroll
        for (int i = 0; i < BATCH; ++i) {
            const uint32_t bi = b + (uint32_t)i;
            if (bi < b1) {
                const bool fb = hml_fwd_step<K>(cx, alpha, e[i]);
                if (STORE) {
                    if (fb) nfb++;
                    const uint32_t t = bi + 1u;
#pragma unroll
                    for (int s = 0; s < K; ++s) {
                        rows[hml_bk(lay, bi, K, s)] = (cx.self && t < cx.B) ? alpha[s] * g[i][s] : alpha[s];
                        if (aprobe) aprobe[(uint64_t)t * K + s] = alpha[s];
                    }
                }
            }
        }
    }
}

template <int K>
__device__ __forceinline__ void hml_b_forward(const float* __restrict__ em, const float* __restrict__ gsc,
                                                     hml_model* __restrict__ mdl, float* __restrict__ rows,
                                                     float* __restrict__ aprobe, float* __restrict__ entry,
                                                     float* __restrict__ exitv, uint32_t* __restrict__ fb_count, int L,
                                                     const hml_layout lay) {
    __shared__ float sm_A[hml_amat<K>::LDS_FLOATS];
    hml_amat_fill<K>(sm_A, mdl, (int)threadIdx.x, (int)blockDim.x);
    hml_fwd_ctx<K> cx;
    hml_fwd_ctx_load<K>(cx, mdl, sm_A);
    const uint32_t B = cx.B;
    const int W = (int)mdl->fwd_W;
    const uint32_t C = (B + (uint32_t)L - 1u) / (uint32_t)L;
    const uint32_t gid = blockIdx.x * blockDim.x + threadIdx.x;
    const uint32_t nthreads = gridDim.x * blockDim.x;
    if (gid < (uint32_t)K && aprobe) aprobe[gid] = mdl->pi[gid];
    for (uint32_t c = gid; c < C; c += nthreads) {
        const uint32_t first = c * (uint32_t)L;
        const uint32_t last = (first + (uint32_t)L < B) ? first + (uint32_t)L : B;
        const uint32_t ws = (first >= (uint32_t)W) ? first - (uint32_t)W : 0u;
        const bool exact = (ws == 0u);
        float alpha[K];
        uint32_t nfb = 0;
#pragma unroll
        for (int s = 0; s < K; ++s) alpha[s] = exact ? mdl->pi[s] : cx.invK;
        hml_fwd_run<K, false>(cx, alpha, em, gsc, rows, aprobe, ws, first, nfb, lay);
#pragma unroll
        for (int s = 0; s < K; ++s) entry[(uint64_t)c * K + s] = alpha[s];
        hml_fwd_run<K, true>(cx, alpha, em, gsc, rows, aprobe, first, last, nfb, lay);
#pragma unroll
        for (int s = 0; s < K; ++s) exitv[(uint64_t)c * K + s] = alpha[s];
        fb_count[c] = nfb;
        if (nfb) atomicAdd(&mdl->uniform_fallbacks, (unsigned long long)nfb);
    }
}
template <int K>
HML_KERNEL __launch_bounds__(256) void hml_k_forward(const float* __restrict__ em, const float* __restrict__ gsc,
                                                     hml_model* __restrict__ mdl, float* __restrict__ rows,
                                                     float* __restrict__ aprobe, float* __restrict__ entry,
                                                     float* __restrict__ exitv, uint32_t* __restrict__ fb_count, int L,
                                                     const hml_layout lay) {
    hml_b_forward<K>(em, gsc, mdl, rows, aprobe, entry, exitv, fb_count, L, lay);
}


__device__ __forceinline__ bool hml_fwd_chunk_exact(uint32_t c, int L, int W) { return c == 0u || c * (uint32_t)L <= (uint32_t)W; }

__device__ __forceinline__ uint32_t hml_ld_u32_coherent(const uint32_t* p) {
    return __hip_atomic_load(p, __ATOMIC_RELAXED, __HIP_MEMORY_SCOPE_AGENT);
}
__device__ __forceinline__ uint32_t hml_ld_bits_coherent(const float* p) {
    return hml_ld_u32_coherent(reinterpret_cast<const uint32_t*>(p));
}

template <int K>
__device__ __forceinline__ bool hml_fwd_chunk_consistent(const float* __restrict__ entry, const float* __restrict__ exitv, uint32_t c) {
    bool same = true;
#pragma unroll
    for (int s = 0; s < K; ++s)
        same = same && (hml_ld_bits_coherent(entry + (uint64_t)c * K + s) == hml_ld_bits_coherent(exitv + (uint64_t)(c - 1) * K + s));
    return same;
}

#define HML_REPAIR_WINDOW_WORDS 4096
#define HML_REPAIR_TOUCHED_CAP 2048
struct hml_repair_lds {
    uint32_t bad[HML_REPAIR_WINDOW_WORDS];
    uint32_t bad2[HML_REPAIR_WINDOW_WORDS];
    uint32_t tlist[HML_REPAIR_TOUCHED_CAP];
    uint32_t tcount;
    uint32_t next_first_bad;
    uint32_t any_bad;
    uint32_t any_marked, carry;
};

template <int K>
__device__ void hml_fwd_repair(const float* __restrict__ em, const float* __restrict__ gsc, hml_model* __restrict__ mdl,
                               float* __restrict__ rows, float* __restrict__ aprobe, float* __restrict__ entry,
                               float* __restrict__ exitv, uint32_t* __restrict__ fb_count,
                               const uint32_t* __restrict__ fail_list, uint32_t n_fail, uint32_t* __restrict__ touched,
                               uint32_t gen, int L, const hml_layout lay, hml_repair_lds& sh, const float* lds_A) {
    hml_fwd_ctx<K> cx;
    hml_fwd_ctx_load<K>(cx, mdl, lds_A);
    const uint32_t B = cx.B;
    const int W = (int)mdl->fwd_W;
    const uint32_t C = (B + (uint32_t)L - 1u) / (uint32_t)L;
    const int tid = threadIdx.x, nthr = blockDim.x;
    const uint32_t win = HML_REPAIR_WINDOW_WORDS * 32u;
    const uint32_t nfper = HML_BWD_CHUNK / (uint32_t)L + 1u;
    auto account = [&](uint32_t c, uint32_t nfb) {
        const uint32_t old = fb_count[c];
        fb_count[c] = nfb;
        if (nfb != old) atomicAdd(&mdl->uniform_fallbacks, (unsigned long long)(long long)((int)nfb - (int)old));
        for (uint32_t b = c * (uint32_t)L; b < (c + 1u) * (uint32_t)L && b < B; b += HML_BWD_CHUNK) {
            const uint32_t bc = b / HML_BWD_CHUNK;
            touched[bc] = gen;
            const uint32_t k = atomicAdd(&sh.tcount, 1u);
            if (k < (uint32_t)HML_REPAIR_TOUCHED_CAP) sh.tlist[k] = bc;
        }
    };
    if (tid == 0) { mdl->fwd_serial_ran = 1u; sh.tcount = 0u; sh.next_first_bad = 0u; }
    __syncthreads();
    for (uint32_t w0 = 0; w0 < C; w0 += win) {
        const uint32_t w1 = (w0 + win < C) ? w0 + win : C;
        for (int i = tid; i < HML_REPAIR_WINDOW_WORDS; i += nthr) { sh.bad[i] = 0u; sh.bad2[i] = 0u; }
        if (tid == 0) { sh.any_marked = 0u; sh.carry = 0u; sh.any_bad = 0u; }
        __syncthreads();
        if (tid == 0 && sh.next_first_bad) { sh.bad2[0] = 1u; sh.next_first_bad = 0u; sh.carry = 1u; }
        for (uint64_t i = (uint64_t)tid; i < (uint64_t)n_fail * nfper; i += (uint64_t)nthr) {
            const uint32_t cb = fail_list[i / nfper];
            const uint32_t f = (cb * HML_BWD_CHUNK) / (uint32_t)L + (uint32_t)(i % nfper);
            if (f > (cb * HML_BWD_CHUNK + HML_BWD_CHUNK - 1u) / (uint32_t)L || f >= C || f < w0 || f >= w1) continue;
            if ((uint32_t)(((uint64_t)f * (uint32_t)L) / HML_BWD_CHUNK) != cb) continue;
            if (hml_fwd_chunk_exact(f, L, W)) continue;
            bool same = true;
#pragma unroll
            for (int s = 0; s < K; ++s) same = same && (hml_f2u(entry[(uint64_t)f * K + s]) == hml_f2u(exitv[(uint64_t)(f - 1) * K + s]));
            if (!same) { atomicOr(&sh.bad[(f - w0) >> 5], 1u << ((f - w0) & 31u)); sh.any_marked = 1u; }
        }
        __syncthreads();
        if (sh.any_marked == 0u && sh.carry == 0u) continue;
        for (uint32_t factor = 2u; factor <= 16u; factor *= 2u) {
            for (uint32_t c = w0 + (uint32_t)tid; c < w1; c += (uint32_t)nthr) {
                if (((sh.bad[(c - w0) >> 5] >> ((c - w0) & 31u)) & 1u) == 0u) continue;
                if (hml_fwd_chunk_exact(c, L, W)) continue;
                const uint32_t first = c * (uint32_t)L;
                const uint32_t last = (first + (uint32_t)L < B) ? first + (uint32_t)L : B;
                const uint32_t Wl = (uint32_t)W * factor;
                const uint32_t ws = (first >= Wl) ? first - Wl : 0u;
                float alpha[K];
                uint32_t nfb = 0;
#pragma unroll
                for (int s = 0; s < K; ++s) alpha[s] = (ws == 0u) ? mdl->pi[s] : cx.invK;
                hml_fwd_run<K, false>(cx, alpha, em, gsc, rows, aprobe, ws, first, nfb, lay);
#pragma unroll
                for (int s = 0; s < K; ++s) entry[(uint64_t)c * K + s] = alpha[s];
                hml_fwd_run<K, true>(cx, alpha, em, gsc, rows, aprobe, first, last, nfb, lay);
#pragma unroll
                for (int s = 0; s < K; ++s) exitv[(uint64_t)c * K + s] = alpha[s];
                account(c, nfb);
                atomicAdd(&mdl->forward_refits, 1ull);
            }
            __threadfence_block();
            __syncthreads();
            if (tid == 0) sh.any_bad = 0u;
            __syncthreads();
            for (uint32_t c = w0 + (uint32_t)tid; c < w1; c += (uint32_t)nthr) {
                if (((sh.bad[(c - w0) >> 5] >> ((c - w0) & 31u)) & 1u) == 0u) continue;
                for (uint32_t cc = c; cc <= c + 1u && cc < C; ++cc) {
                    if (hml_fwd_chunk_exact(cc, L, W) || hml_fwd_chunk_consistent<K>(entry, exitv, cc)) continue;
                    if (cc < w1) { atomicOr(&sh.bad2[(cc - w0) >> 5], 1u << ((cc - w0) & 31u)); sh.any_bad = 1u; }
                    else sh.next_first_bad = 1u;
                }
            }
            __syncthreads();
            if (sh.any_bad == 0u || factor == 16u) break;
            for (int i = tid; i < HML_REPAIR_WINDOW_WORDS; i += nthr) { sh.bad[i] = sh.bad2[i]; sh.bad2[i] = 0u; }
            __syncthreads();
        }
        if (tid == 0 && (sh.any_bad != 0u || sh.carry != 0u)) {
            for (uint32_t wi = 0; wi < (w1 - w0 + 31u) / 32u; ++wi) {
                uint32_t bits = sh.bad2[wi];
                while (bits) {
                    const int bit = __ffs(bits) - 1;
                    bits &= bits - 1u;
                    float alpha[K];
                    bool have_alpha = false;
                    for (uint32_t c = w0 + wi * 32u + (uint32_t)bit; c < C; ++c) {
                        bool same = true;
#pragma unroll
                        for (int s = 0; s < K; ++s) {
                            if (!have_alpha) alpha[s] = hml_u2f(hml_ld_bits_coherent(exitv + (uint64_t)(c - 1) * K + s));
                            same = same && (hml_f2u(alpha[s]) == hml_ld_bits_coherent(entry + (uint64_t)c * K + s));
                        }
                        if (same) break;
                        const uint32_t first = c * (uint32_t)L;
                        const uint32_t last = (first + (uint32_t)L < B) ? first + (uint32_t)L : B;
#pragma unroll
                        for (int s = 0; s < K; ++s) entry[(uint64_t)c * K + s] = alpha[s];
                        uint32_t nfb = 0;
                        hml_fwd_run<K, true>(cx, alpha, em, gsc, rows, aprobe, first, last, nfb, lay);
#pragma unroll
                        for (int s = 0; s < K; ++s) exitv[(uint64_t)c * K + s] = alpha[s];
                        have_alpha = true;
                        account(c, nfb);
                        atomicAdd(&mdl->forward_serial, 1ull);
                    }
                }
            }
        }
// ... 7 lines not shown
```

hammlet_amd/csrc/hml_k_many.h:

```cpp
#ifndef HML_K_MANY_H
#define HML_K_MANY_H

#include "hml_k_backward.h"
#include "hml_k_blocks.h"
#include "hml_k_forward.h"
#include "hml_k_params.h"

struct hml_chain_dev {
    const uint8_t* summary;
    const float* w;
    const float2* ia;
    int32_t key_base;
    uint32_t n_spans;
    uint16_t* stage;
    uint32_t *span_count, *coarse1, *starts, *host_B;
    float2* bstat;
    hml_model* mdl;
    float *em, *gsc, *rows, *entry, *exitv;
    uint32_t *fb, *redo, *touched;
    unsigned long long *smap, *cmap;
    uint8_t* bentry;
    int16_t* q;
    double* partial;
    int32_t* diff;
    uint32_t* boundary;
    hml_layout lay;
};

#define HML_MANY_ARG_CHAINS 16
struct hml_many_args { hml_chain_dev c[HML_MANY_ARG_CHAINS]; };
static_assert(sizeof(hml_many_args) + 64 <= 4096, "kernel arguments of the batched kernels");

HML_KERNEL __launch_bounds__(256) void hml_m_compact_scan_summary(const hml_chain_dev* __restrict__ cs, uint32_t T) {
    const hml_chain_dev& c = cs[blockIdx.y];
    hml_b_compact_scan_summary(c.summary, c.w, T, c.mdl, 0.0f, 0, c.key_base, c.stage, c.span_count, c.coarse1);
}
HML_KERNEL __launch_bounds__(256) void hml_m_compact_scatter(const hml_chain_dev* __restrict__ cs, uint32_t T) {
    const hml_chain_dev& c = cs[blockIdx.y];
    hml_b_compact_scatter(c.stage, c.span_count, c.coarse1, c.n_spans, T, c.mdl, c.starts, c.host_B);
}
template <int K>
HML_KERNEL __launch_bounds__(256) void hml_m_stats_emission(const hml_chain_dev* __restrict__ cs, int with_gsc) {
    const hml_chain_dev& c = cs[blockIdx.y];
    hml_b_stats_emission<K>(c.ia, c.starts, c.mdl, c.bstat, c.em, with_gsc ? c.gsc : nullptr, nullptr, 0, c.lay);
}
template <int K>
HML_KERNEL __launch_bounds__(256) void hml_m_forward(const hml_many_args a, int with_gsc, int L) {
    const hml_chain_dev& c = a.c[blockIdx.y];
    hml_b_forward<K>(c.em, with_gsc ? c.gsc : nullptr, c.mdl, c.rows, nullptr, c.entry, c.exitv, c.fb, L, c.lay);
}
template <int K>
HML_KERNEL __launch_bounds__(256) void hml_m_backward_maps(const hml_many_args a, int with_gsc, int L) {
    const hml_chain_dev& c = a.c[blockIdx.y];
    hml_b_backward_maps2<K>(c.rows, c.mdl, c.smap, c.cmap, c.lay, c.entry, c.exitv, c.redo, L, with_gsc ? nullptr : c.starts, c.mdl);
}
template <int K>
HML_KERNEL __launch_bounds__(1024) void hml_m_backward_chain(const hml_many_args a, int with_gsc, int L) {
    const hml_chain_dev& c = a.c[blockIdx.y];
    hml_b_backward_chain<K>(c.cmap, c.mdl, c.bentry, c.em, with_gsc ? c.gsc : nullptr, c.rows, nullptr, c.entry, c.exitv, c.fb, c.redo, c.touched,
                            c.smap, L, c.lay, 3, 0, with_gsc ? nullptr : c.starts);
}
template <int K>
HML_KERNEL __launch_bounds__(256) void hml_m_counts(const hml_many_args a) {
    const hml_chain_dev& c = a.c[blockIdx.y];
    hml_b_counts<K, true, false>(c.q, c.starts, c.bstat, c.mdl, c.partial, c.smap, c.bentry);
}
HML_KERNEL __launch_bounds__(256) void hml_m_record(const hml_many_args a, unsigned long long chains_recording) {
    if (!((chains_recording >> blockIdx.y) & 1ull)) return;
    const hml_chain_dev& c = a.c[blockIdx.y];
    hml_b_record(c.q, c.starts, c.mdl, c.diff, c.boundary);
}
template <int K>
HML_KERNEL __launch_bounds__(1024) void hml_m_params(const hml_many_args a) {
    const hml_chain_dev& c = a.c[blockIdx.y];
    hml_b_params<K, true, true>(c.mdl, c.partial, 0, (int)blockIdx.x, (int)gridDim.x);
}

#endif
```

hammlet_amd/csrc/hml_k_params.h:

```cpp
#ifndef HML_K_PARAMS_H
#define HML_K_PARAMS_H

#include <type_traits>

#include "hml_dist.h"
#include "hml_k_backward.h"
#include "hml_state.h"

struct hml_dev_src {
    hml_stream s;
    __device__ __forceinline__ uint32_t next() { return hml_stream_next(&s); }
};

template <int K>
__device__ __forceinline__ void hml_derive(hml_model* mdl, int tid) {
    const int P = mdl->P, D = mdl->D;
    if (tid < P) {
        const float m = mdl->mu[tid], v = mdl->var[tid], sd = mdl->sd[tid];
        mdl->logN[tid] = hml_logf(sd) + m * m / (2 * v);
        mdl->rvar2[tid] = 1.0 / (2.0 * (double)v);
    }
    if (tid < K) {
        float r = 0.0f;
        for (int d = 0; d < D; ++d) {
            const int pp = mdl->map[tid][d];
            const float m = mdl->mu[pp], v = mdl->var[pp], sd = mdl->sd[pp];
            r += hml_logf(sd) + m * m / (2 * v);
        }
        mdl->logNs[tid] = r;
        mdl->logA[tid] = hml_logf(mdl->A[tid * K + tid]);
    }
    if (tid == 0) {
        float mv = HML_INF_F;
        for (int k = 0; k < P; ++k) { const float v = mdl->var[k]; mv = (v < mv) ? v : mv; }
        const float l = hml_logf((float)mdl->T);
        const float arg = 2 * l * mv;
        const float t = HML_SQRTF(arg);
        mdl->thr_theta = t;
        if (mdl->dynamic) mdl->thr = t;
    }
}

template <int K>
HML_KERNEL __launch_bounds__(64) void hml_k_derive(hml_model* mdl) { hml_derive<K>(mdl, threadIdx.x); }

HML_KERNEL __launch_bounds__(64) void hml_k_set_dynamic(hml_model* mdl, int on, int take_threshold) {
    if (threadIdx.x == 0) {
        mdl->dynamic = on;
        if (take_threshold) mdl->thr = mdl->thr_theta;
    }
}

template <int K, bool SPREAD, bool MANY = false>
__device__ __forceinline__ void hml_b_params(hml_model* __restrict__ mdl, typename std::conditional<SPREAD, double, const double>::type* __restrict__ partial,
                                                     int mode, int leaf, int nleaf) {
    __shared__ double wp[16][K][2];
    __shared__ uint32_t s_last;
    __shared__ float fin[K][2];
    __shared__ float graw[K * K];
    __shared__ float praw[K];
    __shared__ unsigned long long s_trans[K * K];
    __shared__ unsigned long long s_occ[K];
    const int tid = threadIdx.x, lane = tid & 63, wave = tid >> 6;
    if (mode == 0 && mdl->halted != 0u) return;
    if (tid == 0) mdl->dbg_t[0] = wall_clock64();
    __shared__ float s_var[K], s_logN[K];
    const int P = mdl->P, D = mdl->D;
    const unsigned long long epoch = mdl->epoch;
    const hml_key key = mdl->key;
    float hyp0 = 0.0f, hyp1 = 0.0f, hyp2 = 0.0f, hyp3 = 0.0f;
    if (wave == 0 && lane < P) { hyp0 = mdl->nig_post[lane][0]; hyp1 = mdl->nig_post[lane][1]; hyp2 = mdl->nig_post[lane][2]; hyp3 = mdl->nig_post[lane][3]; }
    if (wave == 1 && lane < K) hyp0 = mdl->dirPi[lane];
    if (tid >= 128 && tid < 128 + K * K) hyp0 = mdl->dirA[tid - 128];
    unsigned long long acc_total = 0ull;
    if (tid >= 128 && tid < 128 + K * K) {
        const int e = tid - 128;
        unsigned long long v[HML_CNT_SPLIT];
#pragma unroll
        for (int sp = 0; sp < HML_CNT_SPLIT; ++sp) v[sp] = mdl->trans[sp][e];
        unsigned long long t = 0ull;
#pragma unroll
        for (int sp = 0; sp < HML_CNT_SPLIT; ++sp) { t += v[sp]; if (!SPREAD) mdl->trans[sp][e] = 0ull; }
        s_trans[e] = t;
        if (!SPREAD) mdl->last_trans[e] = t;
        acc_total = t;
    }
    if (tid >= 512 && tid < 512 + K) {
        const int k = tid - 512;
        unsigned long long v[HML_CNT_SPLIT];
#pragma unroll
        for (int sp = 0; sp < HML_CNT_SPLIT; ++sp) v[sp] = mdl->occ[sp][k];
        unsigned long long t = 0ull;
#pragma unroll
        for (int sp = 0; sp < HML_CNT_SPLIT; ++sp) { t += v[sp]; if (!SPREAD) mdl->occ[sp][k] = 0ull; }
        s_occ[k] = t;
        if (!SPREAD) mdl->last_occ[k] = t;
        acc_total = t;
    }
    typename std::conditional<SPREAD, double, const double>::type* const level1 = partial + (uint64_t)HML_REDUCE_GROUPS * 2 * K;
    if constexpr (SPREAD) {
        for (int idx = wave; idx < 2 * K; idx += 16) {
            const double r = hml_wave_tree_f64(partial[(uint64_t)idx * HML_REDUCE_GROUPS + 64u * (uint32_t)leaf + (uint32_t)lane]);
            if (lane == 0) __hip_atomic_store(reinterpret_cast<unsigned long long*>(level1) + leaf * 2 * K + idx, hml_d2u(r), __ATOMIC_RELAXED, __HIP_MEMORY_SCOPE_AGENT);
        }
    }
    constexpr int NDRAW = 2 + (K * K + 63) / 64;
    static_assert(2 * NDRAW <= 16, "wavefronts of the parameter kernel");
    const bool draws = wave < NDRAW;
    const int mirror = wave - (16 - NDRAW);
    double part_s[K], part_q[K], part2_s[K], part2_q[K];
#pragma unroll
    for (int s = 0; s < K; ++s) {
        part_s[s] = (!SPREAD && mode == 0 && !draws) ? partial[(uint64_t)(s * 2 + 0) * HML_REDUCE_GROUPS + tid] : 0.0;
        part_q[s] = (!SPREAD && mode == 0 && !draws) ? partial[(uint64_t)(s * 2 + 1) * HML_REDUCE_GROUPS + tid] : 0.0;
        part2_s[s] = (!SPREAD && mode == 0 && mirror >= 0) ? partial[(uint64_t)(s * 2 + 0) * HML_REDUCE_GROUPS + (mirror * 64 + lane)] : 0.0;
        part2_q[s] = (!SPREAD && mode == 0 && mirror >= 0) ? partial[(uint64_t)(s * 2 + 1) * HML_REDUCE_GROUPS + (mirror * 64 + lane)] : 0.0;
    }

    if (SPREAD) __syncthreads();
    else asm volatile("s_waitcnt lgkmcnt(0)\n\ts_barrier" ::: "memory");
    if (tid == 0) mdl->dbg_t[1] = wall_clock64();
    if constexpr (SPREAD) {
        static_assert(NDRAW <= 8, "wavefronts 8 (occupancies) and 15 (ticket) draw nothing");
        if (wave == 15) {
            uint32_t last = 0u;
            if (lane == 0) {
                __threadfence();
                const uint32_t t = atomicAdd(&mdl->params_ticket, 1u);
                last = ((t + 1u) % (uint32_t)nleaf == 0u) ? 1u : 0u;
                s_last = last;
            }
            last = (uint32_t)__builtin_amdgcn_readfirstlane((int)last);
            if (last != 0u) {
                __threadfence();
                if (lane < 2 * K) {
                    unsigned long long raw[16];
#pragma unroll
                    for (int i = 0; i < 16; ++i) raw[i] = __hip_atomic_load(reinterpret_cast<unsigned long long*>(level1) + i * 2 * K + lane, __ATOMIC_RELAXED, __HIP_MEMORY_SCOPE_AGENT);
#pragma unroll
                    for (int i = 0; i < 16; ++i) wp[i][lane >> 1][lane & 1] = hml_u2d(raw[i]);
                }
            }
        }
    }

    unsigned long long cnt = 0ull;
    float th_alpha = hyp0, th_gcore = 0.0f, th_z = 0.0f;
    if (wave == 0 && lane < P) {
        const int k = lane;
        if (mode == 0) {
            if (D == 1) cnt = s_occ[k];
            else for (int st = 0; st < K; ++st) for (int d = 0; d < D; ++d) if (mdl->map[st][d] == k) cnt += s_occ[st];
        }
        if (cnt > 0ull) th_alpha = (float)((double)hyp0 + (double)cnt / 2.0);
        hml_dev_src src;
        src.s = hml_stream_open(key, HML_KIND_THETA, epoch, (uint32_t)k);
        th_gcore = hml_gamma_core_f32<hml_devmath>(src, th_alpha);
        hml_normal_f32<hml_devmath> nd;
        th_z = nd.draw_std(src);
        if (tid == 0) mdl->dbg_t[7] = wall_clock64();
    }
    if (mode != 2) {
        if (wave == 1 && lane < K) {
            const int k = lane;
            const float al = hyp0 + (float)s_occ[k];
            hml_dev_src src;
            src.s = hml_stream_open(key, HML_KIND_PI, epoch, (uint32_t)k);
            praw[k] = hml_gamma_f32<hml_devmath>(src, al, 1.0f);
        }
        if (tid >= 128 && tid < 128 + K * K) {
            const int e = tid - 128;
            const float al = hyp0 + (float)s_trans[e];
            hml_dev_src src;
            src.s = hml_stream_open(key, HML_KIND_TRANS, epoch, (uint32_t)e);
            graw[e] = hml_gamma_f32<hml_devmath>(src, al, 1.0f);
        }
    }
    if (tid == 128) mdl->dbg_t[4] = wall_clock64();

    if constexpr (SPREAD) {
        __syncthreads();
        if (s_last == 0u) return;
        if (tid >= 128 && tid < 128 + K * K) {
            const int e = tid - 128;
#pragma unroll
            for (int sp = 0; sp < HML_CNT_SPLIT; ++sp) mdl->trans[sp][e] = 0ull;
            mdl->last_trans[e] = acc_total;
        }
        if (tid >= 512 && tid < 512 + K) {
            const int k = tid - 512;
#pragma unroll
            for (int sp = 0; sp < HML_CNT_SPLIT; ++sp) mdl->occ[sp][k] = 0ull;
            mdl->last_occ[k] = acc_total;
        }
    }
    if (mode == 0) {
        if (!SPREAD && !draws) {
#pragma unroll
            for (int s = 0; s < K; ++s) {
                const double a = hml_wave_tree_f64(part_s[s]), d = hml_wave_tree_f64(part_q[s]);
                if (lane == 0) { wp[wave][s][0] = a; wp[wave][s][1] = d; }
            }
        }
        if (!SPREAD && mirror >= 0) {
#pragma unroll
            for (int s = 0; s < K; ++s) {
                const double a = hml_wave_tree_f64(part2_s[s]), d = hml_wave_tree_f64(part2_q[s]);
                if (lane == 0) { wp[mirror][s][0] = a; wp[mirror][s][1] = d; }
            }
        }
        if (tid == 1023) mdl->dbg_t[8] = wall_clock64();
        __syncthreads();
        if (tid < 2 * K) {
            const int s = tid >> 1, c = tid & 1;
            double v[16];
#pragma unroll
            for (int i = 0; i < 16; ++i) v[i] = wp[i][s][c];
#pragma unroll
            for (int st = 1; st < 16; st <<= 1)
#pragma unroll
                for (int i = 0; i < 16; i += 2 * st) v[i] = v[i] + v[i + st];
            fin[s][c] = (float)v[0];
        }
        __syncthreads();
        if (tid == 0) mdl->dbg_t[2] = wall_clock64();
    }

    if (wave == 0 && lane < P) {
        const int k = lane;
        float alpha = hyp0, beta = hyp1, mu0 = hyp2, nu = hyp3;
        if (mode == 0) { mdl->last_sum[k] = fin[k][0]; mdl->last_sumsq[k] = fin[k][1]; }
        if (cnt > 0ull) {
            const float sum = fin[k][0], sumSq = fin[k][1];
            if (sumSq < 0.0f) hml_raise(mdl, HML_DEVERR_NEG_SUMSQ, sumSq);
            const double N = (double)cnt;
            const float xbar = (float)((double)sum / N);
            float ssN = (float)((double)(sum * sum) / N);
            if (ssN > sumSq) ssN = sumSq;
            const float na = th_alpha;
            const float dxm = (xbar - mu0) * (xbar - mu0);
            const float nb = (float)((double)beta +
                                     (((double)sumSq + (N * (double)nu / (N + (double)nu)) * (double)dxm) - (double)ssN) / 2.0);
            const float nm = (float)((double)(nu * mu0 + sum) / ((double)nu + N));
            const float nn = (float)((double)nu + N);
            if (na <= 0.0f) hml_raise(mdl, HML_DEVERR_NIG_ALPHA, na);
            if (nb <= 0.0f) hml_raise(mdl, HML_DEVERR_NIG_BETA, nb);
            if (nn <= 0.0f) hml_raise(mdl, HML_DEVERR_NIG_NU, nn);
            if (!hml_isfinite(nm)) hml_raise(mdl, HML_DEVERR_NIG_MU0, nm);
            alpha = na; beta = nb; mu0 = nm; nu = nn;
        }
        (void)alpha;
        const float g = th_gcore * (float)(1.0 / (double)beta);
        const float v = (float)(1.0 / (double)g);
        const float m = th_z * HML_SQRTF(v / nu) + mu0;
        if (!hml_isfinite(m)) hml_raise(mdl, HML_DEVERR_MEAN_NOT_FINITE, m);
        if (!hml_isfinite(v)) hml_raise(mdl, HML_DEVERR_VAR_NOT_FINITE, v);
        else if (v <= 0.0f) hml_raise(mdl, HML_DEVERR_VAR_NOT_POSITIVE, v);
        const float sd = HML_SQRTF(v);
        mdl->mu[k] = m; mdl->var[k] = v; mdl->sd[k] = sd;
        mdl->rvar2[k] = 1.0 / (2.0 * (double)v);
        if (mode == 0) {
            const float ln = hml_logf(sd) + m * m / (2 * v);
            mdl->logN[k] = ln;
            s_logN[k] = ln;
            s_var[k] = v;
        }
#pragma unroll
        for (int i = 0; i < 4; ++i) mdl->nig_post[k][i] = mdl->nig_prior[i];
        if (tid == 0) mdl->dbg_t[3] = wall_clock64();
    }
    __syncthreads();
    if (tid == 0) mdl->dbg_t[5] = wall_clock64();
    if (mode != 2) {
        if (tid < K) {
            float sum = 0.0f;
#pragma unroll
            for (int d = 0; d < K; ++d) sum += graw[tid * K + d];
#pragma unroll
            for (int d = 0; d < K; ++d) mdl->A[tid * K + d] = graw[tid * K + d] / sum;
            if (mode == 0) {
                mdl->logA[tid] = hml_logf(graw[tid * K + tid] / sum);
                float r = 0.0f;
                for (int d = 0; d < D; ++d) r += s_logN[mdl->map[tid][d]];
                mdl->logNs[tid] = r;
            }
        }
        if (mode == 0 && tid == 65) {
            float mv = HML_INF_F;
#pragma unroll
            for (int k = 0; k < P; ++k) { const float v = s_var[k]; mv = (v < mv) ? v : mv; }
            const float l = hml_logf((float)mdl->T);
            const float arg = 2 * l * mv;
            const float t = HML_SQRTF(arg);
            mdl->thr_theta = t;
            if (mdl->dynamic) mdl->thr = t;
        }
        if (tid == 64) {
            float sum = 0.0f;
#pragma unroll
            for (int d = 0; d < K; ++d) sum += praw[d];
#pragma unroll
            for (int d = 0; d < K; ++d) mdl->pi[d] = praw[d] / sum;
        }
        if (tid >= 128 && tid < 128 + K * K) {
            const int e = tid - 128;
            mdl->dirA[e] = (e / K == e % K) ? mdl->a_diag : mdl->a_off;
        }
        if (tid >= 512 && tid < 512 + K) {
            const int k = tid - 512;
            mdl->dirPi[k] = mdl->pi_alpha;
        }
    }
    if (mode != 0) {
        __threadfence_block();
        __syncthreads();
        hml_derive<K>(mdl, tid);
    }
    if (tid == 1023) {
        if (mode == 0) {
            uint32_t W = mdl->fwd_W;
            const unsigned long long refits = mdl->forward_refits - mdl->fwd_refits_seen;
            const unsigned long long serial = mdl->forward_serial - mdl->fwd_serial_seen;
            const unsigned long long handful = (mdl->B >> 22) ? (((unsigned long long)(mdl->B >> 16) > 16ull) ? (unsigned long long)(mdl->B >> 16) : 16ull) : 0ull;
            if (mdl->tre_fused && (mdl->B >> 22)) {
                const unsigned long long hi = (unsigned long long)(mdl->B >> mdl->tre_hi_shift) + 16ull, lo = (unsigned long long)(mdl->B >> mdl->tre_lo_shift) + 2ull;
                if (serial != 0ull || refits > hi) {
                    W = (W + 8u < (uint32_t)HML_TRE_HALO_MAX) ? W + 8u : (uint32_t)HML_TRE_HALO_MAX;
                    mdl->tre_W_floor = W;
                    mdl->tre_floor_age = 0u;
                } else {
                    if (++mdl->tre_floor_age >= 256u) { mdl->tre_floor_age = 0u; mdl->tre_W_floor = (mdl->tre_W_floor > 8u) ? mdl->tre_W_floor - 8u : 0u; }
                    const uint32_t lowest = (mdl->tre_W_floor > 8u) ? mdl->tre_W_floor : 8u;
                    if (refits < lo && W >= lowest + 8u) W -= 8u;
                }
                if (W > (uint32_t)HML_TRE_HALO_MAX) W = (uint32_t)HML_TRE_HALO_MAX;
            } else
            {
            if (mdl->wl_W_need != 0u && ++mdl->wl_need_age > 128u) mdl->wl_W_need = 0u;
            if (serial != 0ull || refits > handful) {
                if (mdl->sweeps >= (unsigned long long)mdl->fwd_burnin_sweeps && (serial != 0ull || refits >= 16ull) && !MANY) { mdl->wl_W_need = W; mdl->wl_need_age = 0u; }
                W = (2u * W < 1024u) ? 2u * W : 1024u; mdl->fwd_quiet = 0u;
            } else if (refits == 0ull) {
                uint32_t floorW = (mdl->sweeps < (unsigned long long)mdl->fwd_burnin_sweeps) ? mdl->fwd_W_burnin : mdl->fwd_W0;
                if (mdl->wl_W_need != 0u) { const uint32_t keep = ((mdl->wl_W_need + 8u) & ~7u) < 1024u ? ((mdl->wl_W_need + 8u) & ~7u) : 1024u; floorW = keep > floorW ? keep : floorW; }
                if (++mdl->fwd_quiet >= mdl->fwd_quiet_need) {
                    const uint32_t w2 = W - W / 4u;
                    const uint32_t lower = (w2 > floorW) ? ((w2 & ~7u) > floorW ? (w2 & ~7u) : floorW) : floorW;
                    W = lower < W ? lower : W;
                    mdl->fwd_quiet = 0u;
                }
            } else mdl->fwd_quiet = 0u;
            }
            mdl->fwd_W = W;
            mdl->fwd_refits_seen = mdl->forward_refits;
            mdl->fwd_serial_seen = mdl->forward_serial;
            mdl->fwd_serial_ran = 0u;
        }
        mdl->dbg_t[6] = wall_clock64();
        mdl->fwd_mismatch = 0u;
        mdl->fwd_mismatch2 = 0u;
        mdl->epoch = epoch + 1ull;
        if (mode == 0) { mdl->sweeps += 1ull; mdl->block_updates += (unsigned long long)mdl->B; }
    }
}
template <int K>
HML_KERNEL __launch_bounds__(1024) void hml_k_params(hml_model* __restrict__ mdl, const double* __restrict__ partial,
                                                     int mode) {
    hml_b_params<K, false>(mdl, partial, mode, 0, 1);
}
#define HML_PARAMS_TREE_WGS 16
template <int K>
HML_KERNEL __launch_bounds__(1024) void hml_k_params_spread(hml_model* __restrict__ mdl, double* __restrict__ partial) {
    hml_b_params<K, true>(mdl, partial, 0, (int)blockIdx.x, (int)gridDim.x);
}


#endif
```

hammlet_amd/csrc/hml_state.h:

```cpp
#ifndef HML_STATE_H
#define HML_STATE_H

#include "hml_common.h"
#include "hml_philox.h"

#define HML_TRE_HALO_MAX 128
#define HML_SPAN 4096
#define HML_GROUP_SPANS 16
#define HML_REDUCE_CHUNK 256
#define HML_REDUCE_GROUPS 1024
#define HML_BWD_CHUNK 64
#define HML_FWD_GROUP 16
struct hml_layout {
    uint32_t lshift;
    uint32_t cstride;
};
HML_HD uint64_t hml_bk(const hml_layout lay, uint32_t b, int K, int s) {
    const uint32_t r = b & ((1u << lay.lshift) - 1u), c = b >> lay.lshift;
    return ((uint64_t)r * (uint32_t)K + (uint32_t)s) * lay.cstride + c;
}

#define HML_CNT_SPLIT 16

enum {
    HML_DEVERR_NONE = 0,
    HML_DEVERR_IP_NOT_FINITE = 1,
    HML_DEVERR_NEG_BACKWARD = 2,
    HML_DEVERR_NEG_SUMSQ = 3,
    HML_DEVERR_NIG_ALPHA = 4,
    HML_DEVERR_NIG_BETA = 5,
    HML_DEVERR_NIG_NU = 6,
    HML_DEVERR_NIG_MU0 = 7,
    HML_DEVERR_MEAN_NOT_FINITE = 8,
    HML_DEVERR_VAR_NOT_FINITE = 9,
    HML_DEVERR_VAR_NOT_POSITIVE = 10,
    HML_DEVERR_TOO_MANY_RECORDS = 11,
    HML_DEVERR_LAUNCH_GEOMETRY = 12
};

#define HML_MAX_D 4

struct hml_model {
    int32_t K;
    int32_t D, P;
    uint8_t map[HML_CAP_K][HML_MAX_D];
    float logNs[HML_CAP_K];
    uint64_t stat_stride;
    int32_t self_trans;
    int32_t dynamic;
    uint32_t T;
    float nig_prior[4];
    float a_off, a_diag, pi_alpha;
    hml_key key;
    float mu[HML_CAP_K], var[HML_CAP_K], sd[HML_CAP_K];
    double rvar2[HML_CAP_K];
    float logN[HML_CAP_K];
    float logA[HML_CAP_K];
    float A[HML_CAP_K * HML_CAP_K];
    float pi[HML_CAP_K];
    float thr;
    float thr_theta;
    float nig_post[HML_CAP_K][4];
    float dirA[HML_CAP_K * HML_CAP_K];
    float dirPi[HML_CAP_K];
    uint32_t B;
    uint32_t n_spans;
    uint32_t cap;
    uint32_t halted;
    unsigned long long trans[HML_CNT_SPLIT][HML_MAX_K * HML_MAX_K];
    unsigned long long occ[HML_CNT_SPLIT][HML_MAX_K];
    unsigned long long last_trans[HML_CAP_K * HML_CAP_K];
    unsigned long long last_occ[HML_CAP_K];
    float last_sum[HML_CAP_K], last_sumsq[HML_CAP_K];
    unsigned long long epoch;
    unsigned long long sweeps, block_updates, uniform_fallbacks, forward_refits, forward_serial;
    unsigned long long fused_fallbacks;
    unsigned long long n_recorded;
    int32_t max_state_recorded;
    uint32_t err_code;
    float err_value;
    unsigned long long err_count;
    uint32_t fwd_mismatch;
    uint32_t fwd_mismatch2;
    uint32_t fwd_W, fwd_W0, fwd_serial_ran, fwd_quiet;
    uint32_t fwd_W_burnin;
    uint32_t fwd_burnin_sweeps;
    uint32_t fwd_quiet_need;
    uint32_t tre_fused;
    uint32_t tre_hi_shift, tre_lo_shift;
    uint32_t tre_W_floor, tre_floor_age;
    unsigned long long fwd_refits_seen, fwd_serial_seen;
    uint32_t params_ticket;
    unsigned long long dbg_t[12];
    uint32_t wl_lshift, wl_cstride;
    uint32_t wl_bwd_W, wl_bwd_quiet;
    uint32_t wl_W_need, wl_need_age;
    uint32_t wl_retry;
    unsigned long long n_levels_recorded;
    unsigned long long n_breaks_recorded;
    unsigned long long n_bands_recorded;
};

#if defined(__HIPCC__)
__device__ __forceinline__ void hml_halt(hml_model* mdl, uint32_t found, uint32_t* host_words) {
    mdl->B = 0u;
    mdl->halted = found;
    if (host_words) {
        __hip_atomic_store(host_words, found, __ATOMIC_RELAXED, __HIP_MEMORY_SCOPE_SYSTEM);
        __hip_atomic_store(host_words + 2, found, __ATOMIC_RELAXED, __HIP_MEMORY_SCOPE_SYSTEM);
    }
}
__device__ __forceinline__ void hml_warmup_for_many_blocks(hml_model* mdl, uint32_t B) {
    if (B >= (1u << 22) && !mdl->tre_fused && mdl->sweeps < 4ull && mdl->fwd_W < 4u * mdl->fwd_W_burnin) mdl->fwd_W = 4u * mdl->fwd_W_burnin;
    if (B >= (1u << 22) && mdl->tre_fused && mdl->sweeps < 4ull && mdl->fwd_W < 64u) mdl->fwd_W = 64u;
}
#endif

#endif
```

hammlet_amd/csrc/hml_sweep.hip:

```cpp
#include "hml_capi_shared.hpp"

template <int KK>
static bool fused_geometry(hml_ctx* c, uint32_t* n_sub, uint32_t* n_wg) {
    if (c->fused_slots == 0) {
        int per_cu = 0, cus = 0;
        if (hipOccupancyMaxActiveBlocksPerMultiprocessor(&per_cu, hml_k_blocks_fused<KK>, HML_FUSED_WAVES * 64, 0) != hipSuccess ||
            hipDeviceGetAttribute(&cus, hipDeviceAttributeMultiprocessorCount, c->device) != hipSuccess || per_cu <= 0 || cus <= 0) {
            (void)hipGetLastError();
            c->fused_slots = -1;
        } else {
            c->fused_slots = per_cu * cus;
        }
        if (const char* e = getenv("HML_FUSED_SLOTS")) c->fused_slots = atoi(e);
    }
    if (c->fused_slots <= 0) return false;
    const uint64_t batches = (c->T + HML_FUSED_SUB_POSITIONS - 1) / HML_FUSED_SUB_POSITIONS;
    const uint64_t m = (batches + (uint64_t)c->fused_slots - 1) / (uint64_t)c->fused_slots;
    if (m > HML_FUSED_MAX_SUB) return false;
    *n_sub = (uint32_t)m;
    *n_wg = (uint32_t)((c->T + m * HML_FUSED_SUB_POSITIONS - 1) / (m * HML_FUSED_SUB_POSITIONS));
    return true;
}


template <int KK>
static int sweep_k(hml_ctx* c, char method, bool record) {
    hipStream_t s = c->stream;
    const bool mix = (method == HML_METHOD_MIXTURE);
    const uint32_t T = (uint32_t)c->T;
    bool emitted = false, fused = false;
    if (c->hint_stale && (c->dynamic || !c->blocks_valid)) {
        hipStreamCaptureStatus cap = hipStreamCaptureStatusNone;
        if (hipStreamIsCapturing(s, &cap) == hipSuccess && cap == hipStreamCaptureStatusNone) {
            launch_compact_pair(c, 0, 0.0f);
            KLAUNCH_CHECK();
            HIPCHK(hipStreamSynchronize(s));
        }
    }
    c->hint_stale = false;
    refresh_hint(c);
    const bool dense_geo = c->B_hint >= c->dense_min_blocks;
    const bool trellis = dense_geo && !mix && c->D == 1 && c->tre_fused;
    const bool mid_geo = !dense_geo && c->fwdL_mid > c->fwdL && c->B_hint >= c->mid_min_blocks;
    const int L = dense_geo ? c->fwdL_dense : mid_geo ? c->fwdL_mid : c->fwdL;
    const hml_layout lay = dense_geo ? c->lay_dense : mid_geo ? c->lay_mid : c->lay;
    float* const gsc_plane = (!dense_geo && c->late_rescale) ? nullptr : c->d_gsc;
    const uint32_t* const starts_for_maps = gsc_plane ? nullptr : c->d_starts;
    if (c->dynamic || !c->blocks_valid) {
        uint32_t n_sub = 0u, n_wg = 0u;
        if (c->h_B[1] && !c->fused_keep) c->fused_blocks = false;
        if (c->D == 1 && c->use_keys && c->fused_blocks && !shares_device(c) &&
            !(!c->summary_always && c->B_hint && (uint64_t)c->B_hint * 24u > c->T) && fused_geometry<KK>(c, &n_sub, &n_wg)) {
            ProfScope ps(c, "blocks_compact", 1);
            hipLaunchKernelGGL(HIP_KERNEL_NAME(hml_k_blocks_fused<KK>), dim3(n_wg), dim3(HML_FUSED_WAVES * 64), 0, s, c->d_summary, c->d_w, c->d_ia,
                               T, c->d_mdl, c->key_base, c->d_group_word, c->d_stage, c->d_starts, c->d_bstat, c->d_em,
                               gsc_plane, c->probes ? c->d_eprobe : nullptr, mix ? 1 : 0, lay, c->d_hB, n_sub, c->fused_spin_limit, c->d_dbg, c->d_mdl);
            fused = true;
        } else {
            launch_compact_pair(c, 0, 0.0f);
        }
        if (!fused && !trellis) {
            refresh_hint(c);
            const uint32_t h0 = c->B_hint ? c->B_hint : (uint32_t)std::min<uint64_t>(c->T, 1u << 20);
            ProfScope ps(c, "stats_emission");
            if (c->D > 1)
                hipLaunchKernelGGL(HIP_KERNEL_NAME(hml_k_emission_mv<KK, true>), dim3(grid_for(h0, 256, 64, 16384)), dim3(256), 0, s,
                                   c->d_ia, c->d_starts, c->d_mdl, c->d_bstat, c->d_em, gsc_plane, c->probes ? c->d_eprobe : nullptr,
                                   mix ? 1 : 0, lay);
            else if (dense_geo && L <= hml_emit_tile<KK>::MAXL)
                hipLaunchKernelGGL(HIP_KERNEL_NAME(hml_k_emission_tiled<KK, true>), dim3(grid_for(h0, hml_emit_tile<KK>::BLOCKS, 64, 65536)),
                                   dim3(256), 0, s, c->d_ia, c->d_starts, c->d_mdl, c->d_bstat, c->d_em, gsc_plane,
                                   c->probes ? c->d_eprobe : nullptr, mix ? 1 : 0, lay);
            else
            hipLaunchKernelGGL(HIP_KERNEL_NAME(hml_k_stats_emission<KK>), dim3(grid_for(h0, 256, 64, 16384)), dim3(256), 0, s,
                               c->d_ia, c->d_starts, c->d_mdl, c->d_bstat, c->d_em, gsc_plane, c->probes ? c->d_eprobe : nullptr,
                               mix ? 1 : 0, lay);
        }
        KLAUNCH_CHECK();
        emitted = true;
        if (!c->dynamic) c->blocks_valid = true;
    }
    refresh_hint(c);
    const uint32_t hint = c->B_hint ? c->B_hint : (uint32_t)std::min<uint64_t>(c->T, 1u << 20);
    const int gB = grid_for(hint, 256, 64, 16384);
    if (!emitted && !trellis) {
        ProfScope ps(c, "emission");
        if (c->D > 1)
            hipLaunchKernelGGL(HIP_KERNEL_NAME(hml_k_emission_mv<KK, false>), dim3(gB), dim3(256), 0, s, c->d_ia, c->d_starts, c->d_mdl,
                               c->d_bstat, c->d_em, gsc_plane, c->probes ? c->d_eprobe : nullptr, mix ? 1 : 0, lay);
        else if (dense_geo && L <= hml_emit_tile<KK>::MAXL)
            hipLaunchKernelGGL(HIP_KERNEL_NAME(hml_k_emission_tiled<KK, false>), dim3(grid_for(hint, hml_emit_tile<KK>::BLOCKS, 64, 65536)),
                               dim3(256), 0, s, c->d_ia, c->d_starts, c->d_mdl, c->d_bstat, c->d_em, gsc_plane,
                               c->probes ? c->d_eprobe : nullptr, mix ? 1 : 0, lay);
        else
        hipLaunchKernelGGL(HIP_KERNEL_NAME(hml_k_emission<KK>), dim3(gB), dim3(256), 0, s, c->d_bstat, c->d_starts, c->d_mdl,
                           c->d_em, gsc_plane, c->probes ? c->d_eprobe : nullptr, mix ? 1 : 0, lay);
    }
    if (trellis) {
        hipStreamCaptureStatus capst = hipStreamCaptureStatusNone;
        (void)hipStreamIsCapturing(s, &capst);
        bool measure = false;
        if (c->tre_rows && c->tre_slots == 0) {
            int per_cu = 0, cus = 0;
            if (hipOccupancyMaxActiveBlocksPerMultiprocessor(&per_cu, hml_k_trellis_rows<KK, false>, 64 * HML_TR2_WAVES, 0) == hipSuccess &&
                hipDeviceGetAttribute(&cus, hipDeviceAttributeMultiprocessorCount, c->device) == hipSuccess && per_cu > 0 && cus > 0)
                c->tre_slots = per_cu * cus * HML_TR2_WAVES;
            else { (void)hipGetLastError(); c->tre_slots = -1; }
            if (const char* e = getenv("HML_TRELLIS_SLOTS")) c->tre_slots = atoi(e);
        }
        const uint32_t TL = tre_pick_L(c, hint, capst != hipStreamCaptureStatusNone, &measure);
        hipEvent_t tev0 = nullptr, tev1 = nullptr;
        if (measure) { tev0 = ev_get(c); tev1 = ev_get(c); hipEventRecord(tev0, s); }
        if (c->graph_tre_L != TL && getenv("HML_TRELLIS_TUNE_DEBUG")) fprintf(stderr, "[trellis] chunk length %u for %u blocks (%d wavefront slots)\n", TL, hint, c->tre_slots);
        c->graph_tre_L = TL;
        const uint64_t tchunks = ((uint64_t)hint + TL - 1) / TL;
        const uint64_t tgroups = (tchunks + HML_TRE_NCH - 1) / HML_TRE_NCH;
        float* ep = c->probes ? c->d_eprobe : nullptr;
        float* ap = c->probes ? c->d_aprobe : nullptr;
        {
            ProfScope ps(c, "trellis", 1);
            if (c->tre_rows && hint > 1024u && ((uint64_t)hint - 1024u) * 8u >= c->T * 9u)
                hipLaunchKernelGGL(HIP_KERNEL_NAME(hml_k_trellis_rows<KK, true>), dim3(grid_for(tgroups, HML_TR2_WAVES, 4, 1 << 20)), dim3(64 * HML_TR2_WAVES), 0, s,
                                   c->d_ia, c->d_starts, c->d_mdl, c->d_mdl, c->d_bstat, c->d_smap, c->d_cmap, c->d_entry, c->d_exitA, c->d_fb, ep, ap, c->d_tre_ckpt, TL);
            else if (c->tre_rows)
                hipLaunchKernelGGL(HIP_KERNEL_NAME(hml_k_trellis_rows<KK, false>), dim3(grid_for(tgroups, HML_TR2_WAVES, 4, 1 << 20)), dim3(64 * HML_TR2_WAVES), 0, s,
                                   c->d_ia, c->d_starts, c->d_mdl, c->d_mdl, c->d_bstat, c->d_smap, c->d_cmap, c->d_entry, c->d_exitA, c->d_fb, ep, ap, c->d_tre_ckpt, TL);
            else
            hipLaunchKernelGGL(HIP_KERNEL_NAME(hml_k_trellis_tile<KK>), dim3(grid_for(tgroups, 1, 16, 1 << 20)), dim3(64), 0, s,
                               c->d_ia, c->d_starts, c->d_mdl, c->d_mdl, c->d_bstat, c->d_smap, c->d_cmap, c->d_entry, c->d_exitA, c->d_fb, ep, ap, TL);
        }
        {
            ProfScope ps(c, "trellis_repair");
            hipLaunchKernelGGL(HIP_KERNEL_NAME(hml_k_trellis_verify<KK>), dim3(grid_for(tchunks, 256, 16, 1 << 14)), dim3(256), 0, s, c->d_mdl,
                               c->d_entry, c->d_exitA, c->d_redo, TL);
            int in_a = 1;
            for (uint32_t round = 0; round < c->tre_refit_rounds; ++round, in_a ^= 1) {
                uint32_t* lin = in_a ? c->d_redo : c->d_redo2;
                uint32_t* lout = in_a ? c->d_redo2 : c->d_redo;
                hipLaunchKernelGGL(HIP_KERNEL_NAME(hml_k_trellis_refit<KK>), dim3(4096), dim3(64), 0, s, c->d_ia, c->d_starts, c->d_mdl, c->d_smap,
                                   c->d_cmap, c->d_entry, c->d_exitA, c->d_fb, ep, ap, lin, in_a, (c->tre_rows && c->tre_ckpt) ? c->d_tre_ckpt : nullptr, TL);
                hipLaunchKernelGGL(HIP_KERNEL_NAME(hml_k_trellis_verify_list<KK>), dim3(64), dim3(256), 0, s, c->d_mdl, c->d_entry, c->d_exitA,
                                   lin, lout, c->d_touched, in_a, round, TL);
            }
            hipLaunchKernelGGL(HIP_KERNEL_NAME(hml_k_trellis_serial<KK>), dim3(1), dim3(256), 0, s, c->d_ia, c->d_starts, c->d_mdl, c->d_smap,
                               c->d_cmap, c->d_entry, c->d_exitA, c->d_fb, ep, ap, in_a ? c->d_redo : c->d_redo2, in_a, c->d_tre_bitmap, TL);
        }
        {
            ProfScope ps(c, "backward_chain");
            const uint64_t supers = (tchunks + 63) / 64;
            hipLaunchKernelGGL(HIP_KERNEL_NAME(hml_k_trellis_super<KK>), dim3(grid_for(supers * 64, 256, 16, 1 << 16)), dim3(256), 0, s, c->d_cmap,
                               c->d_mdl, c->d_scmap, c->d_super, TL);
            hipLaunchKernelGGL(HIP_KERNEL_NAME(hml_k_trellis_chain<KK>), dim3(1), dim3(1024), 0, s, c->d_super, c->d_mdl, c->d_bentry2, TL);
            hipLaunchKernelGGL(HIP_KERNEL_NAME(hml_k_trellis_states<KK>), dim3(grid_for(tgroups, 1, 16, 1 << 20)), dim3(64), 0, s, c->d_smap,
                               c->d_scmap, c->d_bentry2, c->d_mdl, c->d_q, TL);
        }
        if (measure) {
            hipEventRecord(tev1, s);
            float ms = 0.0f;
            const bool ok = hipEventSynchronize(tev1) == hipSuccess && hipEventElapsedTime(&ms, tev0, tev1) == hipSuccess;
            c->ev_pool.push_back(tev0);
            c->ev_pool.push_back(tev1);
            if (ok) tre_tune_report(c, hint, ms); else { (void)hipGetLastError(); c->tre_autotune = false; }
        }
        c->tre_dense_sweeps++;
        {
            ProfScope ps(c, "counts");
            hipLaunchKernelGGL(HIP_KERNEL_NAME(hml_k_counts_dense<KK, false>), dim3(HML_REDUCE_GROUPS), dim3(256), 0, s, c->d_q,
                               c->d_starts, c->d_bstat, c->d_mdl, c->d_partial, (const unsigned long long*)nullptr, (const uint8_t*)nullptr);
        }
    } else if (!mix) {
        const uint64_t chunks = ((uint64_t)hint + L - 1) / L;
        const int gF = grid_for(chunks, 256, 16, 1 << 20);
        {
            ProfScope ps(c, "forward");
            hipLaunchKernelGGL(HIP_KERNEL_NAME(hml_k_forward<KK>), dim3(gF), dim3(256), 0, s, c->d_em, gsc_plane, c->d_mdl, c->d_rows,
                               c->probes ? c->d_aprobe : nullptr, c->d_entry, c->d_exitA, c->d_fb, L, lay);
        }
        {
            const uint64_t bch = ((uint64_t)hint + HML_BWD_CHUNK - 1) / HML_BWD_CHUNK;
            {
                ProfScope ps(c, "backward_maps");
                hipLaunchKernelGGL(HIP_KERNEL_NAME(hml_k_backward_maps<KK>), dim3(grid_for(bch * 64, 256, 16, 1 << 18)), dim3(256), 0,
                                   s, c->d_rows, c->d_mdl, c->d_smap, c->d_cmap, lay, c->d_entry, c->d_exitA, c->d_redo, L, starts_for_maps, c->d_mdl);
            }
            ProfScope ps(c, "backward_chain");
            if (!dense_geo) {
                hipLaunchKernelGGL(HIP_KERNEL_NAME(hml_k_backward_chain<KK>), dim3(1), dim3(1024), 0, s, c->d_cmap, c->d_mdl,
                                   c->d_bentry, c->d_em, gsc_plane, c->d_rows, c->probes ? c->d_aprobe : nullptr, c->d_entry,
                                   c->d_exitA, c->d_fb, c->d_redo, c->d_touched, c->d_smap, L, lay, 3, 0, starts_for_maps);
            } else {
                hipLaunchKernelGGL(HIP_KERNEL_NAME(hml_k_backward_chain<KK>), dim3(1), dim3(1024), 0, s, c->d_cmap, c->d_mdl,
                                   c->d_bentry, c->d_em, gsc_plane, c->d_rows, c->probes ? c->d_aprobe : nullptr, c->d_entry,
                                   c->d_exitA, c->d_fb, c->d_redo, c->d_touched, c->d_smap, L, lay, 1, 0, starts_for_maps);
                hipLaunchKernelGGL(HIP_KERNEL_NAME(hml_k_backward_super<KK>), dim3(grid_for(bch, 256, 16, 1 << 16)), dim3(256), 0, s,
                                   c->d_cmap, c->d_mdl, c->d_scmap, c->d_super);
                hipLaunchKernelGGL(HIP_KERNEL_NAME(hml_k_backward_chain<KK>), dim3(1), dim3(1024), 0, s, c->d_super, c->d_mdl,
                                   c->d_bentry2, c->d_em, gsc_plane, c->d_rows, c->probes ? c->d_aprobe : nullptr, c->d_entry,
                                   c->d_exitA, c->d_fb, c->d_redo, c->d_touched, c->d_smap, L, lay, 2, 1, starts_for_maps);
                hipLaunchKernelGGL(hml_k_backward_entries, dim3(grid_for(bch, 256, 16, 1 << 16)), dim3(256), 0, s, c->d_scmap,
                                   c->d_bentry2, c->d_mdl, c->d_bentry);
            }
        }
        {
            ProfScope ps(c, "counts");
            if (c->D > 1)
                hipLaunchKernelGGL(HIP_KERNEL_NAME(hml_k_counts<KK, true, true>), dim3(HML_REDUCE_GROUPS), dim3(256), 0, s, c->d_q,
                                   c->d_starts, c->d_bstat, c->d_mdl, c->d_partial, c->d_smap, c->d_bentry);
            else if (dense_geo)
                hipLaunchKernelGGL(HIP_KERNEL_NAME(hml_k_counts_dense<KK, true>), dim3(HML_REDUCE_GROUPS), dim3(256), 0, s, c->d_q,
                                   c->d_starts, c->d_bstat, c->d_mdl, c->d_partial, c->d_smap, c->d_bentry);
            else
            hipLaunchKernelGGL(HIP_KERNEL_NAME(hml_k_counts<KK, true>), dim3(HML_REDUCE_GROUPS), dim3(256), 0, s, c->d_q,
                               c->d_starts, c->d_bstat, c->d_mdl, c->d_partial, c->d_smap, c->d_bentry);
        }
    } else {
        {
            ProfScope ps(c, "mixture");
            hipLaunchKernelGGL(HIP_KERNEL_NAME(hml_k_mixture<KK>), dim3(gB), dim3(256), 0, s, c->d_em, c->d_mdl, c->d_q, lay);
        }
        {
            ProfScope ps(c, "counts");
            if (c->D > 1)
                hipLaunchKernelGGL(HIP_KERNEL_NAME(hml_k_counts<KK, false, true>), dim3(HML_REDUCE_GROUPS), dim3(256), 0, s, c->d_q,
                                   c->d_starts, c->d_bstat, c->d_mdl, c->d_partial, (const unsigned long long*)nullptr,
                                   (const uint8_t*)nullptr);
            else if (dense_geo)
                hipLaunchKernelGGL(HIP_KERNEL_NAME(hml_k_counts_dense<KK, false>), dim3(HML_REDUCE_GROUPS), dim3(256), 0, s, c->d_q,
                                   c->d_starts, c->d_bstat, c->d_mdl, c->d_partial, (const unsigned long long*)nullptr,
                                   (const uint8_t*)nullptr);
            else
            hipLaunchKernelGGL(HIP_KERNEL_NAME(hml_k_counts<KK, false>), dim3(HML_REDUCE_GROUPS), dim3(256), 0, s, c->d_q,
                               c->d_starts, c->d_bstat, c->d_mdl, c->d_partial, (const unsigned long long*)nullptr,
                               (const uint8_t*)nullptr);
        }
    }
    if (record && c->rec_marginals) {
        if (c->pooled) return set_err(HML_ERR_ARG, "the marginals of this context are pooled (common labels, several chains): further sweeps cannot be recorded into them");
        if (int r = ensure_marginal_buffers(c)) return r;
        ProfScope ps(c, "marginals");
        hipLaunchKernelGGL(hml_k_record, dim3(gB), dim3(256), 0, s, c->d_q, c->d_starts, c->d_mdl, c->d_diff, c->d_boundary);
    }
    {
        ProfScope ps(c, "params");
        if (c->params_spread) hipLaunchKernelGGL(HIP_KERNEL_NAME(hml_k_params_spread<KK>), dim3(HML_PARAMS_TREE_WGS), dim3(1024), 0, s, c->d_mdl, c->d_partial);
        else hipLaunchKernelGGL(HIP_KERNEL_NAME(hml_k_params<KK>), dim3(1), dim3(1024), 0, s, c->d_mdl, c->d_partial, 0);
    }
    if (record) { if (int r = launch_recorders(c, s, hint)) return r; }
    KLAUNCH_CHECK();
    return 0;
}


template <int KK>
static int iterate_many_k(hml_ctx* const* cs, int n, uint64_t first, uint64_t iterations, uint64_t thinning, uint64_t* done) {
    hml_ctx* c0 = cs[0];
    hipStream_t s = c0->stream;
    const uint32_t T = (uint32_t)c0->T;
    const int L = c0->fwdL_many;
    const int with_gsc = c0->late_rescale ? 0 : 1;
    const uint32_t n_groups = (c0->n_spans + HML_GROUP_SPANS - 1) / HML_GROUP_SPANS;
    const bool records = thinning > 0 && thinning <= iterations;
    unsigned long long rec_mask = 0ull;
    for (int i = 0; i < n; ++i) {
        if (records) { if (int r = ensure_recorders(cs[i])) return r; }
        if (records && cs[i]->rec_marginals) {
            if (cs[i]->pooled) return set_err(HML_ERR_ARG, "the marginals of a context are pooled (common labels, several chains): further sweeps cannot be recorded into them");
            if (int r = ensure_marginal_buffers(cs[i])) return r;
            rec_mask |= 1ull << i;
        }
    }
    std::vector<hml_chain_dev> h(n);
    for (int i = 0; i < n; ++i) {
        hml_ctx* c = cs[i];
        hml_chain_dev& d = h[i];
        d.summary = c->d_summary; d.w = c->d_w; d.ia = c->d_ia; d.key_base = c->key_base; d.n_spans = c->n_spans;
        d.stage = c->d_stage; d.span_count = c->d_span_count; d.coarse1 = c->d_coarse1; d.starts = c->d_starts; d.host_B = c->d_hB;
        d.bstat = c->d_bstat; d.mdl = c->d_mdl; d.em = c->d_em; d.gsc = c->d_gsc; d.rows = c->d_rows; d.entry = c->d_entry; d.exitv = c->d_exitA;
        d.fb = c->d_fb; d.redo = c->d_redo; d.touched = c->d_touched; d.smap = c->d_smap; d.cmap = c->d_cmap; d.bentry = c->d_bentry;
        d.q = c->d_q; d.partial = c->d_partial; d.diff = c->d_diff; d.boundary = c->d_boundary; d.lay = c->lay_many;
    }
    if (c0->many_cap < n) {
        if (c0->d_many) HIPCHK(hipFree(c0->d_many));
        c0->d_many = nullptr; c0->many_cap = 0;
        HIPCHK(hipMalloc(&c0->d_many, n * sizeof(hml_chain_dev)));
        c0->many_cap = n;
    }
    HIPCHK(hipMemcpyAsync(c0->d_many, h.data(), n * sizeof(hml_chain_dev), hipMemcpyHostToDevice, s));
    HIPCHK(hipStreamSynchronize(s));
    const hml_chain_dev* d_cs = (const hml_chain_dev*)c0->d_many;
    int G = n >= 2 ? 2 : 1;
    if (const char* e = getenv("HML_MANY_GROUPS")) G = std::max(1, std::min(std::min(atoi(e), 4), n));
    struct Grp { int first, count; hipStream_t s; };
    std::vector<Grp> grp(G);
    for (int g = 0; g < G; ++g) { grp[g].first = (int)((int64_t)g * n / G); grp[g].count = (int)((int64_t)(g + 1) * n / G) - grp[g].first; grp[g].s = cs[grp[g].first]->stream; }
    bool fm = c0->trace != nullptr && c0->fused_blocks;
    for (int k = 0; k < n; ++k) fm = fm && cs[k]->trace == c0->trace && cs[k]->fused_blocks && cs[k]->key_base == c0->key_base;
    uint32_t fm_sub = 0u, fm_wg = 0u;
    bool fm_split = true;
    if (const char* e = getenv("HML_FM_SPLIT")) fm_split = atoi(e) != 0;
    uint32_t fs_sub = 1u, fs_wg = 0u;
    const uint64_t fs_tiles1 = (c0->T + HML_FUSED_SUB_POSITIONS - 1) / HML_FUSED_SUB_POSITIONS;
    {
        const uint64_t batches = (c0->T + HML_FUSED_SUB_POSITIONS - 1) / HML_FUSED_SUB_POSITIONS;
        fs_sub = (uint32_t)std::max<uint64_t>(1, (batches + 4095) / 4096);
        if (const char* e = getenv("HML_FM_SPLIT_SUB")) fs_sub = (uint32_t)std::max(1, atoi(e));
        if (fs_sub > HML_FUSED_MAX_SUB) fm_split = false;
        fs_wg = (uint32_t)((c0->T + (uint64_t)fs_sub * HML_FUSED_SUB_POSITIONS - 1) / ((uint64_t)fs_sub * HML_FUSED_SUB_POSITIONS));
    }
    if (fm && !fm_split) {
        if (c0->fm_slots == 0) {
            int per_cu = 0, cus = 0;
            if (hipOccupancyMaxActiveBlocksPerMultiprocessor(&per_cu, hml_m_blocks_fused<KK>, HML_FUSED_WAVES * 64, 0) != hipSuccess ||
                hipDeviceGetAttribute(&cus, hipDeviceAttributeMultiprocessorCount, c0->device) != hipSuccess || per_cu <= 0 || cus <= 0) {
                (void)hipGetLastError();
                c0->fm_slots = -1;
            } else c0->fm_slots = per_cu * cus;
            if (const char* e = getenv("HML_FUSED_MANY_SLOTS")) c0->fm_slots = atoi(e);
        }
        const uint64_t batches = (c0->T + HML_FUSED_SUB_POSITIONS - 1) / HML_FUSED_SUB_POSITIONS;
        const int live = c0->device < 64 ? g_live_ctx[c0->device].load() : n;
        const int sharers = G * std::max(1, (live + n - 1) / n);
        const int64_t slots = c0->fm_slots > 0 ? std::max<int64_t>(1, c0->fm_slots / sharers) : 0;
        const uint64_t m = slots > 0 ? (batches + (uint64_t)slots - 1) / (uint64_t)slots : HML_FUSED_MAX_SUB + 1;
        if (m > HML_FUSED_MAX_SUB) fm = false;
        else { fm_sub = (uint32_t)m; fm_wg = (uint32_t)((c0->T + m * HML_FUSED_SUB_POSITIONS - 1) / (m * HML_FUSED_SUB_POSITIONS)); }
    }
    auto join = [&](bool wait) -> int {
        for (int g = 0; g < G; ++g) {
            if (wait) { HIPCHK(hipStreamSynchronize(grp[g].s)); continue; }
            hipEvent_t ev = ev_get(c0);
            HIPCHK(hipEventRecord(ev, grp[g].s));
            for (int k = grp[g].first; k < grp[g].first + grp[g].count; ++k) if (cs[k]->stream != grp[g].s) HIPCHK(hipStreamWaitEvent(cs[k]->stream, ev, 0));
            c0->ev_pool.push_back(ev);
        }
        return 0;
    };
    for (uint64_t i = first; i < iterations; ++i) {
        for (int k = 0; k < n; ++k) if (!many_sparse(cs[k]) || chain_halted(cs[k])) { *done = i; return join(true); }
        const bool record = thinning > 0 && ((i + 1) % thinning == 0);
        for (int k = 0; k < n; ++k) log_sweep(cs[k], HML_METHOD_FB, record);
        if (fm) for (int k = 0; k < n; ++k) if (cs[k]->h_B[1] && !cs[k]->fused_keep) fm = false;
        for (int g = 0; g < G; ++g) {
            const int g0 = grp[g].first, gn = grp[g].count;
            hipStream_t s = grp[g].s;
            const hml_chain_dev* d_g = d_cs + g0;
            uint32_t hint = 0;
            for (int k = g0; k < g0 + gn; ++k) hint = std::max(hint, cs[k]->B_hint ? cs[k]->B_hint : (uint32_t)std::min<uint64_t>(T, 1u << 20));
            const unsigned ny = (unsigned)gn;
            const unsigned gB = (unsigned)grid_for(hint, 256, 64, 16384);
            if (fm && fm_split) {
                for (int k0 = g0; k0 < g0 + gn; k0 += HML_FS_MAX_CHAINS) {
                    const int nk = std::min(g0 + gn - k0, (int)HML_FS_MAX_CHAINS);
                    hml_fs_args fa;
                    memset(&fa, 0, sizeof fa);
                    for (int k = 0; k < nk; ++k) {
                        hml_ctx* c = cs[k0 + k];
                        hml_fs_chain& f = fa.c[k];
                        f.mdl = c->d_mdl; f.group_word = c->d_group_word; f.wave_total = c->d_wave_total; f.stage = c->d_stage; f.starts = c->d_starts;
                        f.tile_before = c->d_wave_total + (fs_tiles1 + 1) * HML_FUSED_WAVES; f.tile_prev = f.tile_before + (fs_tiles1 + 1);
                        f.bstat = c->d_bstat; f.em = c->d_em; f.gsc = with_gsc ? c->d_gsc : nullptr; f.host_words = c->d_hB; f.lay = c->lay_many;
                    }
                    hipLaunchKernelGGL(hml_m_blocks_list, dim3(fs_wg), dim3(HML_FUSED_WAVES * 64), 0, s, c0->d_summary, c0->d_w, T, c0->key_base, fa, nk, fs_sub);
                    hipLaunchKernelGGL(hml_m_blocks_offsets, dim3(1, (unsigned)nk), dim3(1024), 0, s, fa, fs_wg, fs_sub);
                    hipLaunchKernelGGL(HIP_KERNEL_NAME(hml_m_blocks_emit<KK>), dim3(fs_wg), dim3(HML_FUSED_WAVES * 64), 0, s, c0->d_ia, T, fa, nk, fs_sub);
                }
            } else if (fm) {
                for (int k0 = g0; k0 < g0 + gn; k0 += HML_FM_MAX_CHAINS) {
                    const int nk = std::min(g0 + gn - k0, (int)HML_FM_MAX_CHAINS);
                    hml_fm_args fa;
                    memset(&fa, 0, sizeof fa);
                    for (int k = 0; k < nk; ++k) {
                        hml_ctx* c = cs[k0 + k];
                        hml_fm_chain& f = fa.c[k];
                        f.mdl = c->d_mdl; f.group_word = c->d_group_word; f.stage = c->d_stage; f.starts = c->d_starts; f.bstat = c->d_bstat;
                        f.em = c->d_em; f.gsc = with_gsc ? c->d_gsc : nullptr; f.host_words = c->d_hB; f.lay = c->lay_many;
                    }
                    hipLaunchKernelGGL(HIP_KERNEL_NAME(hml_m_blocks_fused<KK>), dim3(fm_wg), dim3(HML_FUSED_WAVES * 64), 0, s, c0->d_summary, c0->d_w, c0->d_ia,
                                       T, c0->key_base, fa, nk, fm_sub, c0->fused_spin_limit, g == 0 ? c0->d_dbg : nullptr);
                }
            } else {
                hipLaunchKernelGGL(hml_m_compact_scan_summary, dim3(n_groups, ny), dim3(256), 0, s, d_g, T);
                hipLaunchKernelGGL(hml_m_compact_scatter, dim3(n_groups, ny), dim3(256), 0, s, d_g, T);
                hipLaunchKernelGGL(HIP_KERNEL_NAME(hml_m_stats_emission<KK>), dim3(gB, ny), dim3(256), 0, s, d_g, with_gsc);
            }
            const uint64_t chunks = ((uint64_t)hint + L - 1) / L;
            const uint64_t bch = ((uint64_t)hint + HML_BWD_CHUNK - 1) / HML_BWD_CHUNK;
            for (int k0 = g0; k0 < g0 + gn; k0 += HML_MANY_ARG_CHAINS) {
                const int nk = std::min(g0 + gn - k0, (int)HML_MANY_ARG_CHAINS);
                hml_many_args ma;
                memset(&ma, 0, sizeof ma);
                for (int k = 0; k < nk; ++k) ma.c[k] = h[k0 + k];
                const unsigned nyk = (unsigned)nk;
                hipLaunchKernelGGL(HIP_KERNEL_NAME(hml_m_forward<KK>), dim3((unsigned)grid_for(chunks, 256, 16, 1 << 20), nyk), dim3(256), 0, s, ma, with_gsc, L);
                hipLaunchKernelGGL(HIP_KERNEL_NAME(hml_m_backward_maps<KK>), dim3((unsigned)grid_for((bch + 1) / 2 * 64, 256, 16, 1 << 18), nyk), dim3(256), 0, s, ma, with_gsc, L);
                hipLaunchKernelGGL(HIP_KERNEL_NAME(hml_m_backward_chain<KK>), dim3(1, nyk), dim3(1024), 0, s, ma, with_gsc, L);
                hipLaunchKernelGGL(HIP_KERNEL_NAME(hml_m_counts<KK>), dim3(HML_REDUCE_GROUPS, nyk), dim3(256), 0, s, ma);
                if (record && (rec_mask >> k0)) hipLaunchKernelGGL(hml_m_record, dim3(gB, nyk), dim3(256), 0, s, ma, rec_mask >> k0);
                hipLaunchKernelGGL(HIP_KERNEL_NAME(hml_m_params<KK>), dim3(HML_PARAMS_TREE_WGS, nyk), dim3(1024), 0, s, ma);
            }
            if (record) for (int kind = 0; kind < HML_REC_KINDS; ++kind)
                for (int k = g0; k < g0 + gn; ++k) if (cs[k]->rec[kind].on) launch_record_kernel(cs[k], kind, s, dim3(gB));
        }
        KLAUNCH_CHECK();
        if (record) {
            bool any_cb = false;
            for (int k = 0; k < n; ++k) any_cb = any_cb || cs[k]->cb;
            if (any_cb) {
                if (int r = join(true)) return r;
                for (int k = 0; k < n; ++k) {
                    if (int r = check_device_error(cs[k])) return r;
                    if (cs[k]->cb && !chain_halted(cs[k])) cs[k]->cb(cs[k], i, cs[k]->cb_user);
                }
            }
        }
    }
    if (int r = join(false)) return r;
    *done = iterations;
    return 0;
}



#define HML_DEFINE_KTAB(KK)                                                                                                        \
    static void hml_kt_params_##KK(hml_ctx* c, int mode) {                                                                         \
        hipLaunchKernelGGL(HIP_KERNEL_NAME(hml_k_params<KK>), dim3(1), dim3(1024), 0, c->stream, c->d_mdl, c->d_partial, mode);    \
    }                                                                                                                              \
    static void hml_kt_derive_##KK(hml_ctx* c) {                                                                                   \
        hipLaunchKernelGGL(HIP_KERNEL_NAME(hml_k_derive<KK>), dim3(1), dim3(64), 0, c->stream, c->d_mdl);                          \
    }                                                                                                                              \
    extern hml_ktab hml_ktab_##KK;                                                                                                 \
    hml_ktab hml_ktab_##KK = {&sweep_k<KK>, &iterate_many_k<KK>, &hml_kt_params_##KK, &hml_kt_derive_##KK};
#if defined(HML_TU_K)
#define HML_DEFINE_KTAB_(K) HML_DEFINE_KTAB(K)
HML_DEFINE_KTAB_(HML_TU_K)
#elif defined(HML_ONLY_K)
#define HML_DEFINE_KTAB_(K) HML_DEFINE_KTAB(K)
HML_DEFINE_KTAB_(HML_ONLY_K)
#else
HML_DEFINE_KTAB(2) HML_DEFINE_KTAB(3) HML_DEFINE_KTAB(4) HML_DEFINE_KTAB(5) HML_DEFINE_KTAB(6) HML_DEFINE_KTAB(7) HML_DEFINE_KTAB(8) HML_DEFINE_KTAB(9)
HML_DEFINE_KTAB(10) HML_DEFINE_KTAB(11) HML_DEFINE_KTAB(12) HML_DEFINE_KTAB(13) HML_DEFINE_KTAB(14) HML_DEFINE_KTAB(15) HML_DEFINE_KTAB(16)
#endif
```

Measured before the change: 3.094 billion block-updates/s.

## Hoist model-parameter loads ahead of LDS fills and pin them in scalar registers

Several kernels (forward, backward maps, fused blocks, params) now issue their model-struct and first summary loads before the LDS fill work, then pin those values in scalar registers with empty inline asm. This lets the global-memory latency overlap the fill, and the thread counts become compile-time constants. The params kernel appears to work on a local copy of the adaptive state and gate its debug timestamps behind a flag. The risk is higher SGPR pressure and compiler constraints from the asm pins, for a small gain on short kernels.

```diff
diff --git a/hammlet_amd/csrc/hml_capi.hip b/hammlet_amd/csrc/hml_capi.hip
--- a/hammlet_amd/csrc/hml_capi.hip
+++ b/hammlet_amd/csrc/hml_capi.hip
@@ -791,6 +791,7 @@
     m.fwd_burnin_sweeps = c->fwd_burnin_sweeps;
     m.fwd_quiet_need = c->fwd_quiet_need;
     m.n_spans = c->n_spans;
+    m.dbg_t[HML_PARAMS_DBG_FLAG] = getenv("HML_PARAMS_DEBUG") ? 1ull : 0ull;
     HIPCHK(hipMemcpyAsync(c->d_mdl, &m, sizeof m, hipMemcpyHostToDevice, c->stream));
     HIPCHK(hipStreamSynchronize(c->stream));
     c->dynamic = true;
@@ -1305,7 +1306,9 @@
     }
     if (c->model_set && getenv("HML_PARAMS_DEBUG")) {
         hml_model m;
-        if (fetch_model(c, &m) == 0) {
+        if (fetch_model(c, &m) == 0 && m.dbg_t[HML_PARAMS_DBG_FLAG] == 0ull) {
+            fprintf(stderr, "[params dbg] no stamps: HML_PARAMS_DEBUG was not set when the model was set up\n");
+        } else if (fetch_model(c, &m) == 0) {
             fprintf(stderr, "[params dbg] us since the kernel's start: accumulators read %.2f | tree %.2f | theta drawn %.2f | A gammas %.2f | barrier %.2f | end %.2f\n",
                     (m.dbg_t[1] - m.dbg_t[0]) * 0.01, (m.dbg_t[2] - m.dbg_t[0]) * 0.01, (m.dbg_t[3] - m.dbg_t[0]) * 0.01, (m.dbg_t[4] - m.dbg_t[0]) * 0.01,
                     (m.dbg_t[5] - m.dbg_t[0]) * 0.01, (m.dbg_t[6] - m.dbg_t[0]) * 0.01);
diff --git a/hammlet_amd/csrc/hml_common.h b/hammlet_amd/csrc/hml_common.h
--- a/hammlet_amd/csrc/hml_common.h
+++ b/hammlet_amd/csrc/hml_common.h
@@ -26,4 +26,17 @@
 
 #define HML_INF_F (hml_u2f(0x7f800000u))
 
+#if defined(__HIPCC__)
+template <typename T>
+__device__ __forceinline__ void hml_pin(T& x) {
+    static_assert(sizeof(T) == 4 || sizeof(T) == 8, "a 32-bit or a 64-bit value");
+    asm volatile("" : "+s"(x));
+}
+template <typename T, int N>
+__device__ __forceinline__ void hml_pin(T (&x)[N]) {
+#pragma unroll
+    for (int i = 0; i < N; ++i) hml_pin(x[i]);
+}
 #endif
+
+#endif
diff --git a/hammlet_amd/csrc/hml_k_backward.h b/hammlet_amd/csrc/hml_k_backward.h
--- a/hammlet_amd/csrc/hml_k_backward.h
+++ b/hammlet_amd/csrc/hml_k_backward.h
@@ -106,13 +106,16 @@
     hml_amat<K> A;
     float logA[K];
     bool self;
+    int32_t self_word;
+    __device__ __forceinline__ void pin() { A.pin(); hml_pin(logA); hml_pin(self_word); self = self_word != 0; }
 };
 template <int K>
 __device__ __forceinline__ void hml_bwd_ctx_load(hml_bwd_ctx<K>& bx, const hml_model* __restrict__ mdl_ro, const float* lds_A) {
     bx.A.attach(mdl_ro, lds_A);
 #pragma unroll
     for (int i = 0; i < K; ++i) bx.logA[i] = mdl_ro->logA[i];
-    bx.self = mdl_ro->self_trans != 0;
+    bx.self_word = mdl_ro->self_trans;
+    bx.self = bx.self_word != 0;
 }
 
 template <int K>
@@ -167,6 +170,7 @@
     if (lane == 0) cmap[c] = map;
 }
 
+#define HML_BWD_MAPS_THREADS 256
 template <int K>
 __device__ __forceinline__ void hml_b_backward_maps(const float* __restrict__ rows, hml_model* __restrict__ mdl,
                                                            unsigned long long* __restrict__ smap,
@@ -175,18 +179,20 @@
                                                            uint32_t* __restrict__ fail_list, int L,
                                                            const uint32_t* __restrict__ starts,
                                                            const hml_model* __restrict__ mdl_ro) {
-    const uint32_t B = mdl_ro->B;
+    uint32_t B = mdl_ro->B;
+    unsigned long long epoch = mdl_ro->epoch;
+    hml_key key = mdl_ro->key;
+    uint32_t fwd_W = mdl_ro->fwd_W;
+    __shared__ float sm_A[hml_amat<K>::LDS_FLOATS];
+    hml_bwd_ctx<K> bx;
+    hml_bwd_ctx_load<K>(bx, mdl_ro, sm_A);
+    hml_amat_fill<K>(sm_A, mdl_ro, (int)threadIdx.x, HML_BWD_MAPS_THREADS);
+    hml_pin(B); hml_pin(epoch); hml_pin(key.k0); hml_pin(key.k1); hml_pin(fwd_W); bx.pin();
+    const int W = (int)fwd_W;
     const uint32_t nchunks = (B + HML_BWD_CHUNK - 1u) / HML_BWD_CHUNK;
     const int lane = threadIdx.x & 63;
-    const uint32_t wave_global = (blockIdx.x * blockDim.x + threadIdx.x) >> 6;
-    const uint32_t nwaves = (gridDim.x * blockDim.x) >> 6;
-    const unsigned long long epoch = mdl_ro->epoch;
-    const hml_key key = mdl_ro->key;
-    const int W = (int)mdl_ro->fwd_W;
-    __shared__ float sm_A[hml_amat<K>::LDS_FLOATS];
-    hml_amat_fill<K>(sm_A, mdl_ro, (int)threadIdx.x, (int)blockDim.x);
-    hml_bwd_ctx<K> bx;
-    hml_bwd_ctx_load<K>(bx, mdl_ro, sm_A);
+    const uint32_t wave_global = (blockIdx.x * HML_BWD_MAPS_THREADS + threadIdx.x) >> 6;
+    const uint32_t nwaves = (gridDim.x * HML_BWD_MAPS_THREADS) >> 6;
     const uint32_t C = (B + (uint32_t)L - 1u) / (uint32_t)L;
     for (uint32_t c = wave_global; c < nchunks; c += nwaves) {
         float r[K];
@@ -211,7 +217,7 @@
     }
 }
 template <int K>
-HML_KERNEL __launch_bounds__(256) void hml_k_backward_maps(const float* __restrict__ rows, hml_model* __restrict__ mdl,
+HML_KERNEL __launch_bounds__(HML_BWD_MAPS_THREADS) void hml_k_backward_maps(const float* __restrict__ rows, hml_model* __restrict__ mdl,
                                                            unsigned long long* __restrict__ smap,
                                                            unsigned long long* __restrict__ cmap, const hml_layout lay,
                                                            const float* __restrict__ entry, const float* __restrict__ exitv,
@@ -266,19 +272,21 @@
                                                             uint32_t* __restrict__ fail_list, int L,
                                                             const uint32_t* __restrict__ starts,
                                                             const hml_model* __restrict__ mdl_ro) {
-    const uint32_t B = mdl_ro->B;
+    uint32_t B = mdl_ro->B;
+    unsigned long long epoch = mdl_ro->epoch;
+    hml_key key = mdl_ro->key;
+    uint32_t fwd_W = mdl_ro->fwd_W;
+    __shared__ float sm_A[hml_amat<K>::LDS_FLOATS];
+    hml_bwd_ctx<K> bx;
+    hml_bwd_ctx_load<K>(bx, mdl_ro, sm_A);
+    hml_amat_fill<K>(sm_A, mdl_ro, (int)threadIdx.x, HML_BWD_MAPS_THREADS);
+    hml_pin(B); hml_pin(epoch); hml_pin(key.k0); hml_pin(key.k1); hml_pin(fwd_W); bx.pin();
+    const int W = (int)fwd_W;
     const uint32_t nchunks = (B + HML_BWD_CHUNK - 1u) / HML_BWD_CHUNK;
     const uint32_t npairs = (nchunks + 1u) / 2u;
     const int lane = threadIdx.x & 63, li = lane & 31, half = lane >> 5;
-    const uint32_t wave_global = (blockIdx.x * blockDim.x + threadIdx.x) >> 6;
-    const uint32_t nwaves = (gridDim.x * blockDim.x) >> 6;
-    const unsigned long long epoch = mdl_ro->epoch;
-    const hml_key key = mdl_ro->key;
-    const int W = (int)mdl_ro->fwd_W;
-    __shared__ float sm_A[hml_amat<K>::LDS_FLOATS];
-    hml_amat_fill<K>(sm_A, mdl_ro, (int)threadIdx.x, (int)blockDim.x);
-    hml_bwd_ctx<K> bx;
-    hml_bwd_ctx_load<K>(bx, mdl_ro, sm_A);
+    const uint32_t wave_global = (blockIdx.x * HML_BWD_MAPS_THREADS + threadIdx.x) >> 6;
+    const uint32_t nwaves = (gridDim.x * HML_BWD_MAPS_THREADS) >> 6;
     const uint32_t C = (B + (uint32_t)L - 1u) / (uint32_t)L;
     for (uint32_t pw = wave_global; pw < npairs; pw += nwaves) {
         const uint32_t c = 2u * pw + (uint32_t)half;
diff --git a/hammlet_amd/csrc/hml_k_blocks_fused.h b/hammlet_amd/csrc/hml_k_blocks_fused.h
--- a/hammlet_amd/csrc/hml_k_blocks_fused.h
+++ b/hammlet_amd/csrc/hml_k_blocks_fused.h
@@ -15,7 +15,8 @@
     return ((unsigned long long)(gen & HML_FUSED_GEN_MASK) << (2 * HML_FUSED_POS_BITS + 1)) |
            ((unsigned long long)total << HML_FUSED_POS_BITS) | (unsigned long long)last_rel;
 }
-__device__ __forceinline__ uint32_t hml_fused_generation(const hml_model* mdl) { return ((uint32_t)mdl->epoch + 1u) & HML_FUSED_GEN_MASK; }
+__device__ __forceinline__ uint32_t hml_fused_generation(unsigned long long epoch) { return ((uint32_t)epoch + 1u) & HML_FUSED_GEN_MASK; }
+__device__ __forceinline__ uint32_t hml_fused_generation(const hml_model* mdl) { return hml_fused_generation(mdl->epoch); }
 
 __device__ __forceinline__ unsigned long long hml_fused_tile_word(const uint8_t* __restrict__ summary, const float* __restrict__ w, uint32_t T,
                                                                float thr, int32_t base, uint32_t tile, uint32_t n_sub, uint32_t gen) {
@@ -52,6 +53,7 @@
                                                           const hml_layout lay, uint32_t* __restrict__ host_words,
                                                           uint32_t n_sub, uint32_t spin_limit, unsigned long long* __restrict__ dbg,
                                                           const hml_model* __restrict__ mdl_ro) {
+    { uint32_t a0 = T, a1 = n_sub; hml_pin(a0); hml_pin(a1); }
     if (dbg && threadIdx.x == 0) dbg[blockIdx.x * 4 + 0] = wall_clock64();
     static_assert(HML_FUSED_MAX_SUB * HML_FUSED_SUB_POSITIONS == (1 << HML_FUSED_POS_BITS), "tile geometry (bit fields of hml_group_word)");
     static_assert(HML_FUSED_MAX_SUB * HML_FUSED_WAVE_BATCH <= 65536, "16-bit offsets into a wavefront's eighth");
@@ -63,10 +65,8 @@
     __shared__ uint32_t wave_total[NW], wave_last[NW];
     __shared__ unsigned long long red_sum[NW], red_near[NW];
     __shared__ uint64_t sm_exp_tab[32];
-    if (threadIdx.x < 32u) sm_exp_tab[threadIdx.x] = HML_EXP2F_TAB[threadIdx.x];
     constexpr bool LOOPED = K > 6;
     __shared__ hml_emit_lds<LOOPED ? K : 1> sm_emit;
-    if (LOOPED) hml_emit_lds_fill<LOOPED ? K : 1>(sm_emit, mdl_ro, (int)threadIdx.x);
 
     const int lane = threadIdx.x & 63, wave = threadIdx.x >> 6;
     const uint32_t g = blockIdx.x;
@@ -74,11 +74,27 @@
     const uint32_t eighth = n_sub * (uint32_t)HML_FUSED_WAVE_BATCH;
     const uint32_t tile_positions = eighth * (uint32_t)NW;
     const uint64_t wave_base = ((uint64_t)g * NW + (uint32_t)wave) * eighth;
-    const uint32_t gen = hml_fused_generation(mdl_ro);
+    auto load_batch = [&](uint32_t j, uint32_t (&gw)[HML_SUM_SPANS]) {
+        const uint32_t span0 = (uint32_t)(wave_base / HML_SPAN) + j * HML_SUM_SPANS;
+#pragma unroll
+        for (int s = 0; s < HML_SUM_SPANS; ++s)
+            gw[s] = (j < n_sub && span0 + s < n_spans)
+                        ? __builtin_nontemporal_load(reinterpret_cast<const uint32_t*>(summary) + (uint64_t)(span0 + s) * 64u + lane)
+                        : 0u;
+    };
+    uint32_t gw[HML_SUM_SPANS];
+    load_batch(0u, gw);
+    float thr = mdl_ro->thr;
+    unsigned long long epoch = mdl_ro->epoch;
+    uint32_t cap = mdl_ro->cap;
+    int32_t self_word = mdl_ro->self_trans;
+    uint64_t exp_tab_word = 0ull;
+    if (threadIdx.x < 32u) exp_tab_word = HML_EXP2F_TAB[threadIdx.x];
+    if (LOOPED) hml_emit_lds_fill<LOOPED ? K : 1>(sm_emit, mdl_ro, (int)threadIdx.x);
+    hml_pin(thr); hml_pin(epoch); hml_pin(cap); hml_pin(self_word);
+    const uint32_t gen = hml_fused_generation(epoch);
     uint16_t* listed = listed_all[wave];
     uint16_t* masks = mask_all[wave];
-    const float thr = mdl_ro->thr;
-    const uint32_t cap = mdl_ro->cap;
 
     uint32_t total = 0u, last1 = 0u;
     uint32_t placed = 0u;
@@ -122,16 +138,6 @@
     {
         const uint32_t kthr = (thr != thr) ? 0u : hml_weight_key(thr, base);
         const hml_swar_ge sw_ge = hml_swar_ge_make(kthr);
-        auto load_batch = [&](uint32_t j, uint32_t (&gw)[HML_SUM_SPANS]) {
-            const uint32_t span0 = (uint32_t)(wave_base / HML_SPAN) + j * HML_SUM_SPANS;
-#pragma unroll
-            for (int s = 0; s < HML_SUM_SPANS; ++s)
-                gw[s] = (j < n_sub && span0 + s < n_spans)
-                            ? __builtin_nontemporal_load(reinterpret_cast<const uint32_t*>(summary) + (uint64_t)(span0 + s) * 64u + lane)
-                            : 0u;
-        };
-        uint32_t gw[HML_SUM_SPANS];
-        load_batch(0u, gw);
         for (uint32_t j = 0; j < n_sub; ++j) {
             const uint32_t span0 = (uint32_t)(wave_base / HML_SPAN) + j * HML_SUM_SPANS;
             if (span0 >= n_spans) break;
@@ -169,6 +175,7 @@
         for (int m = 1; m < 64; m <<= 1) { const uint32_t o = __shfl_xor(last1, m); last1 = o > last1 ? o : last1; }
     }
     if (lane == 0) { wave_total[wave] = total; wave_last[wave] = last1; }
+    if (threadIdx.x < 32u) sm_exp_tab[threadIdx.x] = exp_tab_word;
     __syncthreads();
     if (dbg && threadIdx.x == 0) dbg[blockIdx.x * 4 + 1] = wall_clock64();
     uint32_t wg_total = 0u, wg_last1 = 0u;
@@ -251,7 +258,7 @@
 
     hml_emit_params<LOOPED ? 1 : K> p;
     if (!LOOPED) hml_emit_load<LOOPED ? 1 : K>(p, mdl_ro, mixture);
-    const bool self_trans = mdl_ro->self_trans != 0;
+    const bool self_trans = self_word != 0;
     {
         uint32_t t = first_t, n = first_n;
         float sx = first_sx, sq = first_sq;
diff --git a/hammlet_amd/csrc/hml_k_forward.h b/hammlet_amd/csrc/hml_k_forward.h
--- a/hammlet_amd/csrc/hml_k_forward.h
+++ b/hammlet_amd/csrc/hml_k_forward.h
@@ -330,6 +330,7 @@
         for (int i = 0; i < K * K; ++i) v[i] = mdl->A[i];
     }
     __device__ __forceinline__ float operator[](int i) const { return v[i]; }
+    __device__ __forceinline__ void pin() { hml_pin(v); }
 };
 template <int K>
 struct hml_amat<K, false> {
@@ -337,6 +338,7 @@
     const float* p;
     __device__ __forceinline__ void attach(const hml_model*, const float* lds) { p = lds; }
     __device__ __forceinline__ float operator[](int i) const { return p[i]; }
+    __device__ __forceinline__ void pin() {}
 };
 template <int K>
 __device__ __forceinline__ void hml_amat_fill(float* lds, const hml_model* mdl, int tid, int nthreads) {
@@ -351,6 +353,7 @@
     hml_amat<K> A;
     float invK;
     bool self;
+    int32_t self_word;
     uint32_t B;
 };
 
@@ -358,7 +361,8 @@
 __device__ __forceinline__ void hml_fwd_ctx_load(hml_fwd_ctx<K>& cx, const hml_model* mdl, const float* lds_A) {
     cx.A.attach(mdl, lds_A);
     cx.invK = (float)(1.0 / (double)(float)K);
-    cx.self = mdl->self_trans != 0;
+    cx.self_word = mdl->self_trans;
+    cx.self = cx.self_word != 0;
     cx.B = mdl->B;
 }
 
@@ -437,6 +441,7 @@
     }
 }
 
+#define HML_FWD_THREADS 256
 template <int K>
 __device__ __forceinline__ void hml_b_forward(const float* __restrict__ em, const float* __restrict__ gsc,
                                                      hml_model* __restrict__ mdl, float* __restrict__ rows,
@@ -444,14 +449,24 @@
                                                      float* __restrict__ exitv, uint32_t* __restrict__ fb_count, int L,
                                                      const hml_layout lay) {
     __shared__ float sm_A[hml_amat<K>::LDS_FLOATS];
-    hml_amat_fill<K>(sm_A, mdl, (int)threadIdx.x, (int)blockDim.x);
     hml_fwd_ctx<K> cx;
     hml_fwd_ctx_load<K>(cx, mdl, sm_A);
+    uint32_t fwd_W = mdl->fwd_W;
+    constexpr bool PI_HEAD = K <= HML_A_REGISTERS_MAX_K;
+    float pi[PI_HEAD ? K : 1];
+    if constexpr (PI_HEAD) {
+#pragma unroll
+        for (int s = 0; s < K; ++s) pi[s] = mdl->pi[s];
+    }
+    hml_amat_fill<K>(sm_A, mdl, (int)threadIdx.x, HML_FWD_THREADS);
+    cx.A.pin(); hml_pin(cx.B); hml_pin(cx.self_word); hml_pin(fwd_W);
+    if constexpr (PI_HEAD) hml_pin(pi);
+    cx.self = cx.self_word != 0;
     const uint32_t B = cx.B;
-    const int W = (int)mdl->fwd_W;
+    const int W = (int)fwd_W;
     const uint32_t C = (B + (uint32_t)L - 1u) / (uint32_t)L;
-    const uint32_t gid = blockIdx.x * blockDim.x + threadIdx.x;
-    const uint32_t nthreads = gridDim.x * blockDim.x;
+    const uint32_t gid = blockIdx.x * HML_FWD_THREADS + threadIdx.x;
+    const uint32_t nthreads = gridDim.x * HML_FWD_THREADS;
     if (gid < (uint32_t)K && aprobe) aprobe[gid] = mdl->pi[gid];
     for (uint32_t c = gid; c < C; c += nthreads) {
         const uint32_t first = c * (uint32_t)L;
@@ -461,7 +476,7 @@
         float alpha[K];
         uint32_t nfb = 0;
 #pragma unroll
-        for (int s = 0; s < K; ++s) alpha[s] = exact ? mdl->pi[s] : cx.invK;
+        for (int s = 0; s < K; ++s) alpha[s] = exact ? (PI_HEAD ? pi[PI_HEAD ? s : 0] : mdl->pi[s]) : cx.invK;
         hml_fwd_run<K, false>(cx, alpha, em, gsc, rows, aprobe, ws, first, nfb, lay);
 #pragma unroll
         for (int s = 0; s < K; ++s) entry[(uint64_t)c * K + s] = alpha[s];
@@ -473,7 +488,7 @@
     }
 }
 template <int K>
-HML_KERNEL __launch_bounds__(256) void hml_k_forward(const float* __restrict__ em, const float* __restrict__ gsc,
+HML_KERNEL __launch_bounds__(HML_FWD_THREADS) void hml_k_forward(const float* __restrict__ em, const float* __restrict__ gsc,
                                                      hml_model* __restrict__ mdl, float* __restrict__ rows,
                                                      float* __restrict__ aprobe, float* __restrict__ entry,
                                                      float* __restrict__ exitv, uint32_t* __restrict__ fb_count, int L,
diff --git a/hammlet_amd/csrc/hml_k_many.h b/hammlet_amd/csrc/hml_k_many.h
--- a/hammlet_amd/csrc/hml_k_many.h
+++ b/hammlet_amd/csrc/hml_k_many.h
@@ -45,12 +45,12 @@
     hml_b_stats_emission<K>(c.ia, c.starts, c.mdl, c.bstat, c.em, with_gsc ? c.gsc : nullptr, nullptr, 0, c.lay);
 }
 template <int K>
-HML_KERNEL __launch_bounds__(256) void hml_m_forward(const hml_many_args a, int with_gsc, int L) {
+HML_KERNEL __launch_bounds__(HML_FWD_THREADS) void hml_m_forward(const hml_many_args a, int with_gsc, int L) {
     const hml_chain_dev& c = a.c[blockIdx.y];
     hml_b_forward<K>(c.em, with_gsc ? c.gsc : nullptr, c.mdl, c.rows, nullptr, c.entry, c.exitv, c.fb, L, c.lay);
 }
 template <int K>
-HML_KERNEL __launch_bounds__(256) void hml_m_backward_maps(const hml_many_args a, int with_gsc, int L) {
+HML_KERNEL __launch_bounds__(HML_BWD_MAPS_THREADS) void hml_m_backward_maps(const hml_many_args a, int with_gsc, int L) {
     const hml_chain_dev& c = a.c[blockIdx.y];
     hml_b_backward_maps2<K>(c.rows, c.mdl, c.smap, c.cmap, c.lay, c.entry, c.exitv, c.redo, L, with_gsc ? nullptr : c.starts, c.mdl);
 }
diff --git a/hammlet_amd/csrc/hml_k_params.h b/hammlet_amd/csrc/hml_k_params.h
--- a/hammlet_amd/csrc/hml_k_params.h
+++ b/hammlet_amd/csrc/hml_k_params.h
@@ -6,6 +6,38 @@
 #include "hml_dist.h"
 #include "hml_k_backward.h"
 #include "hml_state.h"
+
+struct hml_warmup_state {
+    uint32_t fwd_W, fwd_W0, fwd_quiet, fwd_W_burnin, fwd_burnin_sweeps, fwd_quiet_need;
+    uint32_t tre_fused, tre_hi_shift, tre_lo_shift, tre_W_floor, tre_floor_age;
+    uint32_t wl_W_need, wl_need_age;
+    uint32_t B;
+    unsigned long long forward_refits, forward_serial, fwd_refits_seen, fwd_serial_seen, sweeps, block_updates;
+    __device__ __forceinline__ void load(const hml_model* mdl) {
+        fwd_W = mdl->fwd_W; fwd_W0 = mdl->fwd_W0; fwd_quiet = mdl->fwd_quiet; fwd_W_burnin = mdl->fwd_W_burnin;
+        fwd_burnin_sweeps = mdl->fwd_burnin_sweeps; fwd_quiet_need = mdl->fwd_quiet_need;
+        tre_fused = mdl->tre_fused; tre_hi_shift = mdl->tre_hi_shift; tre_lo_shift = mdl->tre_lo_shift;
+        tre_W_floor = mdl->tre_W_floor; tre_floor_age = mdl->tre_floor_age;
+        wl_W_need = mdl->wl_W_need; wl_need_age = mdl->wl_need_age;
+        B = mdl->B;
+        forward_refits = mdl->forward_refits; forward_serial = mdl->forward_serial;
+        fwd_refits_seen = mdl->fwd_refits_seen; fwd_serial_seen = mdl->fwd_serial_seen;
+        sweeps = mdl->sweeps; block_updates = mdl->block_updates;
+    }
+    __device__ __forceinline__ void pin() {
+        hml_pin(fwd_W); hml_pin(fwd_W0); hml_pin(fwd_quiet); hml_pin(fwd_W_burnin); hml_pin(fwd_burnin_sweeps); hml_pin(fwd_quiet_need);
+        hml_pin(tre_fused); hml_pin(tre_hi_shift); hml_pin(tre_lo_shift); hml_pin(tre_W_floor); hml_pin(tre_floor_age);
+        hml_pin(wl_W_need); hml_pin(wl_need_age); hml_pin(B);
+        hml_pin(forward_refits); hml_pin(forward_serial); hml_pin(fwd_refits_seen); hml_pin(fwd_serial_seen);
+        hml_pin(sweeps); hml_pin(block_updates);
+    }
+    __device__ __forceinline__ void store_adapted(hml_model* mdl) const {
+        mdl->fwd_W = fwd_W; mdl->fwd_quiet = fwd_quiet;
+        mdl->tre_W_floor = tre_W_floor; mdl->tre_floor_age = tre_floor_age;
+        mdl->wl_W_need = wl_W_need; mdl->wl_need_age = wl_need_age;
+        mdl->fwd_refits_seen = fwd_refits_seen; mdl->fwd_serial_seen = fwd_serial_seen;
+    }
+};
 
 struct hml_dev_src {
     hml_stream s;
@@ -62,37 +94,53 @@
     __shared__ unsigned long long s_trans[K * K];
     __shared__ unsigned long long s_occ[K];
     const int tid = threadIdx.x, lane = tid & 63, wave = tid >> 6;
-    if (mode == 0 && mdl->halted != 0u) return;
-    if (tid == 0) mdl->dbg_t[0] = wall_clock64();
     __shared__ float s_var[K], s_logN[K];
-    const int P = mdl->P, D = mdl->D;
-    const unsigned long long epoch = mdl->epoch;
-    const hml_key key = mdl->key;
     float hyp0 = 0.0f, hyp1 = 0.0f, hyp2 = 0.0f, hyp3 = 0.0f;
-    if (wave == 0 && lane < P) { hyp0 = mdl->nig_post[lane][0]; hyp1 = mdl->nig_post[lane][1]; hyp2 = mdl->nig_post[lane][2]; hyp3 = mdl->nig_post[lane][3]; }
+    if (wave == 0 && lane < K) { hyp0 = mdl->nig_post[lane][0]; hyp1 = mdl->nig_post[lane][1]; hyp2 = mdl->nig_post[lane][2]; hyp3 = mdl->nig_post[lane][3]; }
     if (wave == 1 && lane < K) hyp0 = mdl->dirPi[lane];
     if (tid >= 128 && tid < 128 + K * K) hyp0 = mdl->dirA[tid - 128];
+    unsigned long long cnt_v[HML_CNT_SPLIT];
+#pragma unroll
+    for (int sp = 0; sp < HML_CNT_SPLIT; ++sp) cnt_v[sp] = 0ull;
+    const bool has_trans = tid >= 128 && tid < 128 + K * K, has_occ = tid >= 512 && tid < 512 + K;
+    if (has_trans || has_occ) {
+        const unsigned long long* const src = has_trans ? &mdl->trans[0][tid - 128] : &mdl->occ[0][tid - 512];
+        const int pitch = has_trans ? HML_MAX_K * HML_MAX_K : HML_MAX_K;
+#pragma unroll
+        for (int sp = 0; sp < HML_CNT_SPLIT; ++sp) cnt_v[sp] = src[sp * pitch];
+    }
+    uint32_t halted = mdl->halted;
+    int32_t P = mdl->P, D = mdl->D;
+    unsigned long long epoch = mdl->epoch;
+    hml_key key = mdl->key;
+    unsigned long long dbg_word = mdl->dbg_t[HML_PARAMS_DBG_FLAG];
+    uint32_t m_T = mdl->T;
+    int32_t m_dynamic = mdl->dynamic;
+    float nig_prior[4] = {mdl->nig_prior[0], mdl->nig_prior[1], mdl->nig_prior[2], mdl->nig_prior[3]};
+    float a_off = mdl->a_off, a_diag = mdl->a_diag, pi_alpha = mdl->pi_alpha;
+    hml_warmup_state ws;
+    ws.load(mdl);
+    hml_pin(halted); hml_pin(P); hml_pin(D); hml_pin(epoch); hml_pin(key.k0); hml_pin(key.k1); hml_pin(dbg_word);
+    hml_pin(m_T); hml_pin(m_dynamic); hml_pin(nig_prior); hml_pin(a_off); hml_pin(a_diag); hml_pin(pi_alpha);
+    ws.pin();
+    if (mode == 0 && halted != 0u) return;
+    const bool dbg = dbg_word != 0ull;
+    if (dbg && tid == 0) mdl->dbg_t[0] = wall_clock64();
     unsigned long long acc_total = 0ull;
     if (tid >= 128 && tid < 128 + K * K) {
         const int e = tid - 128;
-        unsigned long long v[HML_CNT_SPLIT];
-#pragma unroll
-        for (int sp = 0; sp < HML_CNT_SPLIT; ++sp) v[sp] = mdl->trans[sp][e];
         unsigned long long t = 0ull;
 #pragma unroll
-        for (int sp = 0; sp < HML_CNT_SPLIT; ++sp) { t += v[sp]; if (!SPREAD) mdl->trans[sp][e] = 0ull; }
+        for (int sp = 0; sp < HML_CNT_SPLIT; ++sp) { t += cnt_v[sp]; if (!SPREAD) mdl->trans[sp][e] = 0ull; }
         s_trans[e] = t;
         if (!SPREAD) mdl->last_trans[e] = t;
         acc_total = t;
     }
     if (tid >= 512 && tid < 512 + K) {
         const int k = tid - 512;
-        unsigned long long v[HML_CNT_SPLIT];
-#pragma unroll
-        for (int sp = 0; sp < HML_CNT_SPLIT; ++sp) v[sp] = mdl->occ[sp][k];
         unsigned long long t = 0ull;
 #pragma unroll
-        for (int sp = 0; sp < HML_CNT_SPLIT; ++sp) { t += v[sp]; if (!SPREAD) mdl->occ[sp][k] = 0ull; }
+        for (int sp = 0; sp < HML_CNT_SPLIT; ++sp) { t += cnt_v[sp]; if (!SPREAD) mdl->occ[sp][k] = 0ull; }
         s_occ[k] = t;
         if (!SPREAD) mdl->last_occ[k] = t;
         acc_total = t;
@@ -119,7 +167,7 @@
 
     if (SPREAD) __syncthreads();
     else asm volatile("s_waitcnt lgkmcnt(0)\n\ts_barrier" ::: "memory");
-    if (tid == 0) mdl->dbg_t[1] = wall_clock64();
+    if (dbg && tid == 0) mdl->dbg_t[1] = wall_clock64();
     if constexpr (SPREAD) {
         static_assert(NDRAW <= 8, "wavefronts 8 (occupancies) and 15 (ticket) draw nothing");
         if (wave == 15) {
@@ -158,7 +206,7 @@
         th_gcore = hml_gamma_core_f32<hml_devmath>(src, th_alpha);
         hml_normal_f32<hml_devmath> nd;
         th_z = nd.draw_std(src);
-        if (tid == 0) mdl->dbg_t[7] = wall_clock64();
+        if (dbg && tid == 0) mdl->dbg_t[7] = wall_clock64();
     }
     if (mode != 2) {
         if (wave == 1 && lane < K) {
@@ -176,7 +224,7 @@
             graw[e] = hml_gamma_f32<hml_devmath>(src, al, 1.0f);
         }
     }
-    if (tid == 128) mdl->dbg_t[4] = wall_clock64();
+    if (dbg && tid == 128) mdl->dbg_t[4] = wall_clock64();
 
     if constexpr (SPREAD) {
         __syncthreads();
@@ -209,7 +257,7 @@
                 if (lane == 0) { wp[mirror][s][0] = a; wp[mirror][s][1] = d; }
             }
         }
-        if (tid == 1023) mdl->dbg_t[8] = wall_clock64();
+        if (dbg && tid == 1023) mdl->dbg_t[8] = wall_clock64();
         __syncthreads();
         if (tid < 2 * K) {
             const int s = tid >> 1, c = tid & 1;
@@ -223,7 +271,7 @@
             fin[s][c] = (float)v[0];
         }
         __syncthreads();
-        if (tid == 0) mdl->dbg_t[2] = wall_clock64();
+        if (dbg && tid == 0) mdl->dbg_t[2] = wall_clock64();
     }
 
     if (wave == 0 && lane < P) {
@@ -266,11 +314,11 @@
             s_var[k] = v;
         }
 #pragma unroll
-        for (int i = 0; i < 4; ++i) mdl->nig_post[k][i] = mdl->nig_prior[i];
-        if (tid == 0) mdl->dbg_t[3] = wall_clock64();
+        for (int i = 0; i < 4; ++i) mdl->nig_post[k][i] = nig_prior[i];
+        if (dbg && tid == 0) mdl->dbg_t[3] = wall_clock64();
     }
     __syncthreads();
-    if (tid == 0) mdl->dbg_t[5] = wall_clock64();
+    if (dbg && tid == 0) mdl->dbg_t[5] = wall_clock64();
     if (mode != 2) {
         if (tid < K) {
             float sum = 0.0f;
@@ -289,11 +337,11 @@
             float mv = HML_INF_F;
 #pragma unroll
             for (int k = 0; k < P; ++k) { const float v = s_var[k]; mv = (v < mv) ? v : mv; }
-            const float l = hml_logf((float)mdl->T);
+            const float l = hml_logf((float)m_T);
             const float arg = 2 * l * mv;
             const float t = HML_SQRTF(arg);
             mdl->thr_theta = t;
-            if (mdl->dynamic) mdl->thr = t;
+            if (m_dynamic) mdl->thr = t;
         }
         if (tid == 64) {
             float sum = 0.0f;
@@ -304,11 +352,11 @@
         }
         if (tid >= 128 && tid < 128 + K * K) {
             const int e = tid - 128;
-            mdl->dirA[e] = (e / K == e % K) ? mdl->a_diag : mdl->a_off;
+            mdl->dirA[e] = (e / K == e % K) ? a_diag : a_off;
         }
         if (tid >= 512 && tid < 512 + K) {
             const int k = tid - 512;
-            mdl->dirPi[k] = mdl->pi_alpha;
+            mdl->dirPi[k] = pi_alpha;
         }
     }
     if (mode != 0) {
@@ -318,49 +366,50 @@
     }
     if (tid == 1023) {
         if (mode == 0) {
-            uint32_t W = mdl->fwd_W;
-            const unsigned long long refits = mdl->forward_refits - mdl->fwd_refits_seen;
-            const unsigned long long serial = mdl->forward_serial - mdl->fwd_serial_seen;
-            const unsigned long long handful = (mdl->B >> 22) ? (((unsigned long long)(mdl->B >> 16) > 16ull) ? (unsigned long long)(mdl->B >> 16) : 16ull) : 0ull;
-            if (mdl->tre_fused && (mdl->B >> 22)) {
-                const unsigned long long hi = (unsigned long long)(mdl->B >> mdl->tre_hi_shift) + 16ull, lo = (unsigned long long)(mdl->B >> mdl->tre_lo_shift) + 2ull;
+            uint32_t W = ws.fwd_W;
+            const unsigned long long refits = ws.forward_refits - ws.fwd_refits_seen;
+            const unsigned long long serial = ws.forward_serial - ws.fwd_serial_seen;
+            const unsigned long long handful = (ws.B >> 22) ? (((unsigned long long)(ws.B >> 16) > 16ull) ? (unsigned long long)(ws.B >> 16) : 16ull) : 0ull;
+            if (ws.tre_fused && (ws.B >> 22)) {
+                const unsigned long long hi = (unsigned long long)(ws.B >> ws.tre_hi_shift) + 16ull, lo = (unsigned long long)(ws.B >> ws.tre_lo_shift) + 2ull;
                 if (serial != 0ull || refits > hi) {
                     W = (W + 8u < (uint32_t)HML_TRE_HALO_MAX) ? W + 8u : (uint32_t)HML_TRE_HALO_MAX;
-                    mdl->tre_W_floor = W;
-                    mdl->tre_floor_age = 0u;
+                    ws.tre_W_floor = W;
+                    ws.tre_floor_age = 0u;
                 } else {
-                    if (++mdl->tre_floor_age >= 256u) { mdl->tre_floor_age = 0u; mdl->tre_W_floor = (mdl->tre_W_floor > 8u) ? mdl->tre_W_floor - 8u : 0u; }
-                    const uint32_t lowest = (mdl->tre_W_floor > 8u) ? mdl->tre_W_floor : 8u;
+                    if (++ws.tre_floor_age >= 256u) { ws.tre_floor_age = 0u; ws.tre_W_floor = (ws.tre_W_floor > 8u) ? ws.tre_W_floor - 8u : 0u; }
+                    const uint32_t lowest = (ws.tre_W_floor > 8u) ? ws.tre_W_floor : 8u;
                     if (refits < lo && W >= lowest + 8u) W -= 8u;
                 }
                 if (W > (uint32_t)HML_TRE_HALO_MAX) W = (uint32_t)HML_TRE_HALO_MAX;
             } else
             {
-            if (mdl->wl_W_need != 0u && ++mdl->wl_need_age > 128u) mdl->wl_W_need = 0u;
+            if (ws.wl_W_need != 0u && ++ws.wl_need_age > 128u) ws.wl_W_need = 0u;
             if (serial != 0ull || refits > handful) {
-                if (mdl->sweeps >= (unsigned long long)mdl->fwd_burnin_sweeps && (serial != 0ull || refits >= 16ull) && !MANY) { mdl->wl_W_need = W; mdl->wl_need_age = 0u; }
-                W = (2u * W < 1024u) ? 2u * W : 1024u; mdl->fwd_quiet = 0u;
+                if (ws.sweeps >= (unsigned long long)ws.fwd_burnin_sweeps && (serial != 0ull || refits >= 16ull) && !MANY) { ws.wl_W_need = W; ws.wl_need_age = 0u; }
+                W = (2u * W < 1024u) ? 2u * W : 1024u; ws.fwd_quiet = 0u;
             } else if (refits == 0ull) {
-                uint32_t floorW = (mdl->sweeps < (unsigned long long)mdl->fwd_burnin_sweeps) ? mdl->fwd_W_burnin : mdl->fwd_W0;
-                if (mdl->wl_W_need != 0u) { const uint32_t keep = ((mdl->wl_W_need + 8u) & ~7u) < 1024u ? ((mdl->wl_W_need + 8u) & ~7u) : 1024u; floorW = keep > floorW ? keep : floorW; }
-                if (++mdl->fwd_quiet >= mdl->fwd_quiet_need) {
+                uint32_t floorW = (ws.sweeps < (unsigned long long)ws.fwd_burnin_sweeps) ? ws.fwd_W_burnin : ws.fwd_W0;
+                if (ws.wl_W_need != 0u) { const uint32_t keep = ((ws.wl_W_need + 8u) & ~7u) < 1024u ? ((ws.wl_W_need + 8u) & ~7u) : 1024u; floorW = keep > floorW ? keep : floorW; }
+                if (++ws.fwd_quiet >= ws.fwd_quiet_need) {
                     const uint32_t w2 = W - W / 4u;
                     const uint32_t lower = (w2 > floorW) ? ((w2 & ~7u) > floorW ? (w2 & ~7u) : floorW) : floorW;
                     W = lower < W ? lower : W;
-                    mdl->fwd_quiet = 0u;
+                    ws.fwd_quiet = 0u;
                 }
-            } else mdl->fwd_quiet = 0u;
-            }
-            mdl->fwd_W = W;
-            mdl->fwd_refits_seen = mdl->forward_refits;
-            mdl->fwd_serial_seen = mdl->forward_serial;
+            } else ws.fwd_quiet = 0u;
+            }
+            ws.fwd_W = W;
+            ws.fwd_refits_seen = ws.forward_refits;
+            ws.fwd_serial_seen = ws.forward_serial;
             mdl->fwd_serial_ran = 0u;
-        }
-        mdl->dbg_t[6] = wall_clock64();
+            ws.store_adapted(mdl);
+        }
+        if (dbg) mdl->dbg_t[6] = wall_clock64();
         mdl->fwd_mismatch = 0u;
         mdl->fwd_mismatch2 = 0u;
         mdl->epoch = epoch + 1ull;
-        if (mode == 0) { mdl->sweeps += 1ull; mdl->block_updates += (unsigned long long)mdl->B; }
+        if (mode == 0) { mdl->sweeps = ws.sweeps + 1ull; mdl->block_updates = ws.block_updates + (unsigned long long)ws.B; }
     }
 }
 template <int K>
diff --git a/hammlet_amd/csrc/hml_state.h b/hammlet_amd/csrc/hml_state.h
--- a/hammlet_amd/csrc/hml_state.h
+++ b/hammlet_amd/csrc/hml_state.h
@@ -91,6 +91,7 @@
     uint32_t tre_W_floor, tre_floor_age;
     unsigned long long fwd_refits_seen, fwd_serial_seen;
     uint32_t params_ticket;
+#define HML_PARAMS_DBG_FLAG 11
     unsigned long long dbg_t[12];
     uint32_t wl_lshift, wl_cstride;
     uint32_t wl_bwd_W, wl_bwd_quiet;
diff --git a/hammlet_amd/csrc/hml_sweep.hip b/hammlet_amd/csrc/hml_sweep.hip
--- a/hammlet_amd/csrc/hml_sweep.hip
+++ b/hammlet_amd/csrc/hml_sweep.hip
@@ -170,17 +170,17 @@
         }
     } else if (!mix) {
         const uint64_t chunks = ((uint64_t)hint + L - 1) / L;
-        const int gF = grid_for(chunks, 256, 16, 1 << 20);
+        const int gF = grid_for(chunks, HML_FWD_THREADS, 16, 1 << 20);
         {
             ProfScope ps(c, "forward");
-            hipLaunchKernelGGL(HIP_KERNEL_NAME(hml_k_forward<KK>), dim3(gF), dim3(256), 0, s, c->d_em, gsc_plane, c->d_mdl, c->d_rows,
+            hipLaunchKernelGGL(HIP_KERNEL_NAME(hml_k_forward<KK>), dim3(gF), dim3(HML_FWD_THREADS), 0, s, c->d_em, gsc_plane, c->d_mdl, c->d_rows,
                                c->probes ? c->d_aprobe : nullptr, c->d_entry, c->d_exitA, c->d_fb, L, lay);
         }
         {
             const uint64_t bch = ((uint64_t)hint + HML_BWD_CHUNK - 1) / HML_BWD_CHUNK;
             {
                 ProfScope ps(c, "backward_maps");
-                hipLaunchKernelGGL(HIP_KERNEL_NAME(hml_k_backward_maps<KK>), dim3(grid_for(bch * 64, 256, 16, 1 << 18)), dim3(256), 0,
+                hipLaunchKernelGGL(HIP_KERNEL_NAME(hml_k_backward_maps<KK>), dim3(grid_for(bch * 64, HML_BWD_MAPS_THREADS, 16, 1 << 18)), dim3(HML_BWD_MAPS_THREADS), 0,
                                    s, c->d_rows, c->d_mdl, c->d_smap, c->d_cmap, lay, c->d_entry, c->d_exitA, c->d_redo, L, starts_for_maps, c->d_mdl);
             }
             ProfScope ps(c, "backward_chain");
@@ -391,8 +391,8 @@
                 memset(&ma, 0, sizeof ma);
                 for (int k = 0; k < nk; ++k) ma.c[k] = h[k0 + k];
                 const unsigned nyk = (unsigned)nk;
-                hipLaunchKernelGGL(HIP_KERNEL_NAME(hml_m_forward<KK>), dim3((unsigned)grid_for(chunks, 256, 16, 1 << 20), nyk), dim3(256), 0, s, ma, with_gsc, L);
-                hipLaunchKernelGGL(HIP_KERNEL_NAME(hml_m_backward_maps<KK>), dim3((unsigned)grid_for((bch + 1) / 2 * 64, 256, 16, 1 << 18), nyk), dim3(256), 0, s, ma, with_gsc, L);
+                hipLaunchKernelGGL(HIP_KERNEL_NAME(hml_m_forward<KK>), dim3((unsigned)grid_for(chunks, HML_FWD_THREADS, 16, 1 << 20), nyk), dim3(HML_FWD_THREADS), 0, s, ma, with_gsc, L);
+                hipLaunchKernelGGL(HIP_KERNEL_NAME(hml_m_backward_maps<KK>), dim3((unsigned)grid_for((bch + 1) / 2 * 64, HML_BWD_MAPS_THREADS, 16, 1 << 18), nyk), dim3(HML_BWD_MAPS_THREADS), 0, s, ma, with_gsc, L);
                 hipLaunchKernelGGL(HIP_KERNEL_NAME(hml_m_backward_chain<KK>), dim3(1, nyk), dim3(1024), 0, s, ma, with_gsc, L);
                 hipLaunchKernelGGL(HIP_KERNEL_NAME(hml_m_counts<KK>), dim3(HML_REDUCE_GROUPS, nyk), dim3(256), 0, s, ma);
                 if (record && (rec_mask >> k0)) hipLaunchKernelGGL(hml_m_record, dim3(gB, nyk), dim3(256), 0, s, ma, rec_mask >> k0);
```

Result: faster. 3.169 billion block-updates/s (median of 6 runs) (+2.4%).
